# retinal-information-processing-lab/gaussian_processes

Measured on AMD Instinct MI355X. Metric: GP fits/sec (kernel+chol+solve+grad loglik) at N=8192 d=256, higher is better.
Workload: dtype f64; 1 GPU; N=8192 d=256 single cell f64, one M-step closure evaluation with 6 gradients (BASELINE configs[2], headline); N=8192, d=256, parallelism=independent units over 1 GPU(s), one process per GPU, no data-path collective

## Files before the change

### gaussian_processes_amd/csrc/elementwise.hip

```cpp
#include "kernels.h"

namespace gpfit {

__device__ __forceinline__ double wave_sum(double v) {
#pragma unroll
  for (int o = 32; o > 0; o >>= 1) v += __shfl_down(v, o);
  return v;
}

__device__ __forceinline__ double block_sum(double v, double* sh) {
  const int lane = threadIdx.x & 63, wave = threadIdx.x >> 6;
  const int nw = (blockDim.x + 63) >> 6;
  v = wave_sum(v);
  __syncthreads();
  if (lane == 0) sh[wave] = v;
  __syncthreads();
  if (wave == 0) {
    double t = (lane < nw) ? sh[lane] : 0.0;
    t = wave_sum(t);
    if (lane == 0) sh[16] = t;
  }
  __syncthreads();
  return sh[16];
}

__device__ __forceinline__ double lin_pm1(int i, int n) {
  if (n <= 1) return -1.0;
  const double step = 2.0 / (double)(n - 1);
  return (i < n / 2) ? fma(step, (double)i, -1.0) : fma(-step, (double)(n - 1 - i), 1.0);
}

template <typename R>
__global__ void localker_kernel(Theta th, const int* __restrict__ pix, int d, int dp, int n_rows, int n_cols,
                                R* __restrict__ C, int64_t ldc, R* __restrict__ dC) {
  const int j = blockIdx.x * blockDim.x + threadIdx.x;
  const int i = blockIdx.y * blockDim.y + threadIdx.y;
  if (i >= dp || j >= dp) return;
  if (i >= d || j >= d) {
    C[(int64_t)i * ldc + j] = (R)0;
    return;
  }
  const int pi = pix[i], pj = pix[j];
  const double xi = lin_pm1(pi % n_cols, n_cols), yi = lin_pm1(pi / n_cols, n_rows);
  const double xj = lin_pm1(pj % n_cols, n_cols), yj = lin_pm1(pj / n_cols, n_rows);
  const double dxi = xi - th.eps0x, dyi = yi - th.eps0y, dxj = xj - th.eps0x, dyj = yj - th.eps0y;
  const double lai = -th.eb * (dxi * dxi + dyi * dyi);
  const double laj = -th.eb * (dxj * dxj + dyj * dyj);
  const double ai = exp(lai), aj = exp(laj);
  const double ex = xj - xi, ey = yj - yi;
  const double ls = -th.er * (ex * ex + ey * ey);
  const double es = exp(ls);
  const double cij = th.amp * ai * es * aj;
  const double cji = th.amp * aj * es * ai;
  const double c = (cij + cji) / 2.0;
  C[(int64_t)i * ldc + j] = (R)c;
  if (dC) {
    const int64_t dd = (int64_t)d * d, o = (int64_t)i * d + j;
    dC[o] = (R)(c / th.amp);
    dC[dd + o] = (R)(c * (lai + laj));
    dC[2 * dd + o] = (R)(c * ls);
    dC[3 * dd + o] = (R)(2.0 * th.eb * c * (xi + xj - 2.0 * th.eps0x));
    dC[4 * dd + o] = (R)(2.0 * th.eb * c * (yi + yj - 2.0 * th.eps0y));
  }
}

template <typename R>
int launch_localker(const Theta& th, const int* pix, int d, int dp, int n_rows, int n_cols, R* C, int64_t ldc,
                    R* dC, hipStream_t s) {
  dim3 block(32, 8), grid((dp + 31) / 32, (dp + 7) / 8);
  hipLaunchKernelGGL(localker_kernel<R>, grid, block, 0, s, th, pix, d, dp, n_rows, n_cols, C, ldc, dC);
  GP_HIP(hipGetLastError());
  return 0;
}

template <typename R>
__global__ void gather_kernel(const R* __restrict__ X, int64_t ldx, int n, const int* __restrict__ pix, int d,
                              R* __restrict__ Xt, int64_t ldt, R* __restrict__ Xm, int64_t ldm) {
  __shared__ R tile[32][33];
  const int k0 = blockIdx.x * 32, n0 = blockIdx.y * 32;
  const int tx = threadIdx.x, ty = threadIdx.y;
#pragma unroll
  for (int r = 0; r < 4; ++r) {
    const int nn = n0 + ty + 8 * r, k = k0 + tx;
    R v = 0;
    if (nn < n && k < d) v = X[(int64_t)nn * ldx + (pix ? pix[k] : k)];
    tile[ty + 8 * r][tx] = v;
    if (Xm) Xm[(int64_t)nn * ldm + k] = v;
  }
  __syncthreads();
#pragma unroll
  for (int r = 0; r < 4; ++r) {
    const int k = k0 + ty + 8 * r, nn = n0 + tx;
    Xt[(int64_t)k * ldt + nn] = tile[tx][ty + 8 * r];
  }
}

template <typename R>
int launch_gather(const R* X, int64_t ldx, int n, const int* pix, int d, int dp, int np, R* Xt, int64_t ldt, R* Xm,
                  int64_t ldm, hipStream_t s) {
  if (dp % 32 || np % 32) {
    set_error("launch_gather: padded extents must be multiples of 32");
    return -3;
  }
  hipLaunchKernelGGL(gather_kernel<R>, dim3(dp / 32, np / 32), dim3(32, 8), 0, s, X, ldx, n, pix, d, Xt, ldt, Xm,
                     ldm);
  GP_HIP(hipGetLastError());
  return 0;
}

template <typename R>
__global__ __launch_bounds__(256) void qvec_kernel(const R* __restrict__ Xt, const R* __restrict__ XCt, int64_t ld, int dp,
                                                   int n, int np, double s0sq, R* __restrict__ Kvec, R* __restrict__ q) {
  __shared__ double part[8][33];
  const int li = threadIdx.x & 31, sl = threadIdx.x >> 5;
  const int i = blockIdx.x * 32 + li;
  double h = 0.0;
  if (i < n) {
#pragma unroll 4
    for (int k = sl; k < dp; k += 8) h += (double)Xt[(int64_t)k * ld + i] * (double)XCt[(int64_t)k * ld + i];
  }
  part[sl][li] = h;
  __syncthreads();
  if (sl != 0 || i >= np) return;
  if (i >= n) {
    Kvec[i] = (R)1;
    q[i] = (R)1;
    return;
  }
  double t = part[0][li];
#pragma unroll
  for (int z = 1; z < 8; ++z) t += part[z][li];
  const double kv = t + s0sq;
  Kvec[i] = (R)kv;
  q[i] = (R)sqrt(kv);
}

template <typename R>
int launch_qvec(const R* Xt, const R* XCt, int64_t ld, int dp, int n, int np, double s0sq, R* Kvec, R* q,
                hipStream_t s) {
  hipLaunchKernelGGL(qvec_kernel<R>, dim3((np + 31) / 32), dim3(256), 0, s, Xt, XCt, ld, dp, n, np, s0sq, Kvec, q);
  GP_HIP(hipGetLastError());
  return 0;
}

template <typename R>
__global__ __launch_bounds__(256) void group_prepare_kernel(GroupPrepT<R> g) {
  const int u = blockIdx.y;
  const int i = blockIdx.x * 256 + threadIdx.x;
  if (i < g.np) g.mpad[u][i] = (i < g.n) ? g.m[u][i] : (R)0;
  if (blockIdx.x == 0) {
    for (int k = threadIdx.x; k < g.d[u]; k += 256) g.pix[u][k] = g.pix_host[u][k];
    if (threadIdx.x < 4) g.info[u][threadIdx.x] = 0;
  }
}

template <typename R>
int launch_group_prepare(const GroupPrepT<R>& g, hipStream_t s) {
  hipLaunchKernelGGL(group_prepare_kernel<R>, dim3((g.np + 255) / 256, g.n_units), dim3(256), 0, s, g);
  GP_HIP(hipGetLastError());
  return 0;
}

__global__ void group_collect_kernel(GroupCollectT g) {
  const int u = blockIdx.x, t = threadIdx.x;
  if (t < 64) g.scal_host[u][t] = g.scal[u][t];
  else if (t < 68) g.info_host[u][t - 64] = g.info[u][t - 64];
  __threadfence_system();
}

int launch_group_collect(const GroupCollectT& g, hipStream_t s) {
  hipLaunchKernelGGL(group_collect_kernel, dim3(g.n_units), dim3(128), 0, s, g);
  GP_HIP(hipGetLastError());
  return 0;
}

template <typename R>
__global__ __launch_bounds__(256) void pack_lower_kernel(const R* __restrict__ src, int64_t lds, int n, R* __restrict__ dst,
                                                         int64_t ldd) {
  const int tj = blockIdx.x, ti = blockIdx.y;
  if (tj > ti) return;
  const int r0 = ti * TILE + 16 * blockIdx.z, c0 = tj * TILE;
#pragma unroll
  for (int it = 0; it < 8; ++it) {
    const int e = threadIdx.x + 256 * it;
    const int i = r0 + (e >> 7), j = c0 + (e & 127);
    R v;
    if (i < n && j < n) v = src[(int64_t)i * lds + j];
    else v = (i == j) ? (R)1 : (R)0;
    dst[(int64_t)i * ldd + j] = v;
  }
}

template <typename R>
int launch_pack_lower(const R* src, int64_t lds, int n, R* dst, int64_t ldd, int np, hipStream_t s) {
  hipLaunchKernelGGL(pack_lower_kernel<R>, dim3(np / TILE, np / TILE, TILE / 16), dim3(256), 0, s, src, lds, n, dst, ldd);
  GP_HIP(hipGetLastError());
  return 0;
}

template <typename R>
__global__ void symmetrize_kernel(R* __restrict__ A, int64_t lda, int n) {
  __shared__ R tile[32][33];
  const int tj = blockIdx.x, ti = blockIdx.y;
  if (tj > ti) return;
  const int tx = threadIdx.x, ty = threadIdx.y;
#pragma unroll
  for (int r = 0; r < 4; ++r) {
    const int i = ti * 32 + ty + 8 * r, j = tj * 32 + tx;
    tile[ty + 8 * r][tx] = (i < n && j < n) ? A[(int64_t)i * lda + j] : (R)0;
  }
  __syncthreads();
#pragma unroll
  for (int r = 0; r < 4; ++r) {
    const int jj = tj * 32 + ty + 8 * r, ii = ti * 32 + tx;
    if (ii < n && jj < n && ii > jj) A[(int64_t)jj * lda + ii] = tile[tx][ty + 8 * r];
  }
}

template <typename R>
int launch_symmetrize(R* A, int64_t lda, int n, hipStream_t s) {
  const int t = (n + 31) / 32;
  hipLaunchKernelGGL(symmetrize_kernel<R>, dim3(t, t), dim3(32, 8), 0, s, A, lda, n);
  GP_HIP(hipGetLastError());
  return 0;
}

template <typename R>
__global__ void logdet_kernel(const R* __restrict__ L0, double* __restrict__ out0, const R* __restrict__ L1,
                              double* __restrict__ out1, int64_t ldl, int n) {
  __shared__ double sh[17];
  const R* __restrict__ L = blockIdx.x == 0 ? L0 : L1;
  double v = 0.0;
  for (int i = threadIdx.x; i < n; i += blockDim.x) v += log((double)L[(int64_t)i * ldl + i]);
  v = block_sum(v, sh);
  if (threadIdx.x == 0) (blockIdx.x == 0 ? out0 : out1)[0] = 2.0 * v;
}

template <typename R>
int launch_logdet(const R* L, int64_t ldl, int n, double* out, hipStream_t s) {
  hipLaunchKernelGGL(logdet_kernel<R>, dim3(1), dim3(1024), 0, s, L, out, L, out, ldl, n);
  GP_HIP(hipGetLastError());
  return 0;
}

template <typename R>
int launch_logdet_pair(const R* L0, double* out0, const R* L1, double* out1, int64_t ldl, int n, hipStream_t s) {
  hipLaunchKernelGGL(logdet_kernel<R>, dim3(2), dim3(1024), 0, s, L0, out0, L1, out1, ldl, n);
  GP_HIP(hipGetLastError());
  return 0;
}

template <typename R>
__global__ void sum_kernel(const R* __restrict__ x, int n, double scale, double* __restrict__ out) {
  __shared__ double sh[17];
  double v = 0.0;
  for (int i = threadIdx.x; i < n; i += blockDim.x) v += (double)x[i];
  v = block_sum(v, sh);
  if (threadIdx.x == 0) out[0] = scale * v;
}

template <typename R>
__global__ void frob_tile_kernel(const R* __restrict__ T, int64_t ldt, double* __restrict__ partial) {
  __shared__ double sh[17];
  int ti, tj;
  {
    const int t = blockIdx.x;
    int i = (int)((sqrt(8.0 * (double)t + 1.0) - 1.0) * 0.5);
    while ((i + 1) * (i + 2) / 2 <= t) ++i;
    while (i * (i + 1) / 2 > t) --i;
    ti = i;
    tj = t - i * (i + 1) / 2;
  }
  const R* base = T + (int64_t)ti * TILE * ldt + tj * TILE;
  double v = 0.0;
#pragma unroll 8
  for (int e = threadIdx.x; e < TILE * TILE; e += 256) {
    const double x = (double)base[(int64_t)(e >> 7) * ldt + (e & 127)];
    v += x * x;
  }
  v = block_sum(v, sh);
  if (threadIdx.x == 0) partial[blockIdx.x] = v;
}

template <typename R>
int launch_frob_lower(const R* T, int64_t ldt, int np, double* out, double* partial, hipStream_t s) {
  const int t = np / TILE, nt = t * (t + 1) / 2;
  hipLaunchKernelGGL(frob_tile_kernel<R>, dim3(nt), dim3(256), 0, s, T, ldt, partial);
  hipLaunchKernelGGL(sum_kernel<double>, dim3(1), dim3(1024), 0, s, partial, nt, 1.0, out);
  GP_HIP(hipGetLastError());
  return 0;
}

int launch_frob_finish(const double* partial, int nt, double* out, hipStream_t s) {
  hipLaunchKernelGGL(sum_kernel<double>, dim3(1), dim3(1024), 0, s, partial, nt, 1.0, out);
  GP_HIP(hipGetLastError());
  return 0;
}

template <typename R>
__global__ void trmv_lower_kernel(const R* __restrict__ L, int64_t ldl, int np, const R* __restrict__ x,
                                  R* __restrict__ y) {
  const int lane = threadIdx.x & 63;
  const int i = blockIdx.x * (blockDim.x >> 6) + (threadIdx.x >> 6);
  if (i >= np) return;
  const R* row = L + (int64_t)i * ldl;
  double v = 0.0;
#pragma unroll 8
  for (int j = lane; j <= i; j += 64) v += (double)row[j] * (double)x[j];
  v = wave_sum(v);
  if (lane == 0) y[i] = (R)v;
}

template <typename R>
int launch_trmv_lower(const R* L, int64_t ldl, int np, const R* x, R* y, hipStream_t s) {
  hipLaunchKernelGGL(trmv_lower_kernel<R>, dim3((np + 3) / 4), dim3(256), 0, s, L, ldl, np, x, y);
  GP_HIP(hipGetLastError());
  return 0;
}

template <typename R>
__global__ void trmv_lower_t_kernel(const R* __restrict__ L, int64_t ldl, int np, const R* __restrict__ x,
                                    double* __restrict__ partial) {
  __shared__ double sh[4][64];
  const int c = threadIdx.x & 63, rl = threadIdx.x >> 6;
  const int j = blockIdx.x * 64 + c;
  const int i0 = blockIdx.y * TRMV_ROWS, i1 = min(np, i0 + TRMV_ROWS);
  double v = 0.0;
  if (i1 > blockIdx.x * 64) {
#pragma unroll 8
    for (int i = i0 + rl; i < i1; i += 4)
      if (i >= j) v += (double)L[(int64_t)i * ldl + j] * (double)x[i];
  }
  sh[rl][c] = v;
  __syncthreads();
  if (rl == 0) partial[(int64_t)blockIdx.y * np + j] = sh[0][c] + sh[1][c] + sh[2][c] + sh[3][c];
}

template <typename RI, typename RO>
__global__ void reduce_slices_kernel(const RI* __restrict__ src, int64_t stride, int nslice, RO* __restrict__ dst,
                                     int64_t count) {
  const int64_t i = (int64_t)blockIdx.x * blockDim.x + threadIdx.x;
  if (i >= count) return;
  double v = 0.0;
  for (int z = 0; z < nslice; ++z) v += (double)src[(int64_t)z * stride + i];
  dst[i] = (RO)v;
}

template <typename RI, typename RO>
int launch_reduce_slices(const RI* src, int64_t slice_stride, int nslice, RO* dst, int64_t count, hipStream_t s) {
  hipLaunchKernelGGL((reduce_slices_kernel<RI, RO>), dim3((unsigned)((count + 255) / 256)), dim3(256), 0, s, src,
                     slice_stride, nslice, dst, count);
  GP_HIP(hipGetLastError());
  return 0;
}

template <typename R>
int launch_trmv_lower_t(const R* L, int64_t ldl, int np, const R* x, R* z, double* partial, hipStream_t s) {
  const int chunks = (np + TRMV_ROWS - 1) / TRMV_ROWS;
  hipLaunchKernelGGL(trmv_lower_t_kernel<R>, dim3(np / 64, chunks), dim3(256), 0, s, L, ldl, np, x, partial);
  GP_HIP(hipGetLastError());
  return launch_reduce_slices(partial, np, chunks, z, np, s);
}

template <typename R>
__global__ void dot_kernel(const R* __restrict__ x, const R* __restrict__ y, int n, double* __restrict__ out) {
  __shared__ double sh[17];
  double v = 0.0;
  for (int i = threadIdx.x; i < n; i += blockDim.x) v += (double)x[i] * (double)y[i];
  v = block_sum(v, sh);
  if (threadIdx.x == 0) out[0] = v;
}

template <typename R>
int launch_dot(const R* x, const R* y, int n, double* out, hipStream_t s) {
  hipLaunchKernelGGL(dot_kernel<R>, dim3(1), dim3(1024), 0, s, x, y, n, out);
  GP_HIP(hipGetLastError());
  return 0;
}

template <typename R>
__global__ __launch_bounds__(256) void moments_kernel(const R* __restrict__ Kvec, const R* __restrict__ q,
                                                      const R* __restrict__ Cos, int64_t ldc, const R* __restrict__ V,
                                                      int64_t ldv, const R* __restrict__ m, const R* __restrict__ r, int n,
                                                      double A, double lambda0, R* __restrict__ lam_m,
                                                      R* __restrict__ lam_var, R* __restrict__ f, R* __restrict__ wl,
                                                      double* __restrict__ scal, double* __restrict__ part,
                                                      int* __restrict__ ticket) {
  __shared__ double sh[17];
  __shared__ bool last;
  double s_rm = 0.0, s_r = 0.0, s_f = 0.0;
  const int i = blockIdx.x * 256 + threadIdx.x;
  if (i < n) {
    const double c = (double)Cos[(int64_t)i * ldc + i];
    const double delta = acos(c);
    const double J = (sqrt(1.0 - c * c) + PI32 * c - delta * c) / PI32;
    const double qi = (double)q[i];
    const double kii = qi * qi * J;
    const double lv = (double)Kvec[i] - kii + (double)V[(int64_t)i * ldv + i];
    const double lm = (double)m[i];
    const double fi = exp(A * lm + 0.5 * A * A * lv + lambda0);
    const double g = 1.0 - J - (PI32 - delta) * (1.0 - c) / PI32;
    lam_m[i] = (R)lm;
    lam_var[i] = (R)lv;
    f[i] = (R)fi;
    wl[i] = (R)(-0.5 * A * A * fi * g);
    s_rm = (double)r[i] * lm;
    s_r = (double)r[i];
    s_f = fi;
  }
  s_rm = block_sum(s_rm, sh);
  s_r = block_sum(s_r, sh);
  s_f = block_sum(s_f, sh);
  if (threadIdx.x == 0) {
    part[blockIdx.x * 3 + 0] = s_rm;
    part[blockIdx.x * 3 + 1] = s_r;
    part[blockIdx.x * 3 + 2] = s_f;
    __threadfence();
    last = (atomicAdd(ticket, 1) == (int)gridDim.x - 1);
  }
  __syncthreads();
  if (!last) return;
  __threadfence();
  if (threadIdx.x < 3) {
    double v = 0.0;
    for (int b = 0; b < (int)gridDim.x; ++b)
      v += __hip_atomic_load(&part[b * 3 + threadIdx.x], __ATOMIC_RELAXED, __HIP_MEMORY_SCOPE_AGENT);
    scal[threadIdx.x] = v;
  }
  if (threadIdx.x == 0) *ticket = 0;
}

template <typename R>
int launch_moments(const R* Kvec, const R* q, const R* Cos, int64_t ldc, const R* V, int64_t ldv, const R* m,
                   const R* r, int n, double A, double lambda0, R* lam_m, R* lam_var, R* f, R* wl, double* scal,
                   double* part, int* ticket, hipStream_t s) {
  hipLaunchKernelGGL(moments_kernel<R>, dim3((n + 255) / 256), dim3(256), 0, s, Kvec, q, Cos, ldc, V, ldv, m, r, n, A,
                     lambda0, lam_m, lam_var, f, wl, scal, part, ticket);
  GP_HIP(hipGetLastError());
  return 0;
}

template <typename R>
__global__ __launch_bounds__(256) void adjoint_kernel(const R* __restrict__ W, const R* __restrict__ Cos, int64_t ld,
                                                      const R* __restrict__ b, const R* __restrict__ q, int n,
                                                      int np, R* __restrict__ Aout, double* __restrict__ upart,
                                                      double* __restrict__ vpart, double* __restrict__ sumA_part) {
  __shared__ R tA[64][65];
  __shared__ double colsum[4][64];
  __shared__ double sh[17];
  int ti, tj;
  {
    const int t = blockIdx.x;
    int i = (int)((sqrt(8.0 * (double)t + 1.0) - 1.0) * 0.5);
    while ((i + 1) * (i + 2) / 2 <= t) ++i;
    while (i * (i + 1) / 2 > t) --i;
    ti = i;
    tj = t - i * (i + 1) / 2;
  }
  const bool diag = (ti == tj);
  const int tx = threadIdx.x & 63, ty = threadIdx.x >> 6;
  const int j = tj * 64 + tx;
  const double qj = (double)q[j], bj = (double)b[j];
  double csum = 0.0, asum = 0.0;
  for (int rr = ty; rr < 64; rr += 4) {
    const int i = ti * 64 + rr;
    double aw = 0.0, bm = 0.0;
    if (i < n && j < n) {
      const int64_t o = (diag && i < j) ? ((int64_t)j * ld + i) : ((int64_t)i * ld + j);
      const double w = (double)W[o] - 0.5 * (double)b[i] * bj;
      const double c = (double)Cos[o];
      aw = w * (PI32 - acos(c)) / PI32;
      bm = w * sqrt(1.0 - c * c) / PI32;
    }
    tA[rr][tx] = (R)aw;
    Aout[(int64_t)i * ld + j] = (R)aw;
    asum += aw;
    const double rs = wave_sum(bm * qj);
    if (tx == 0) upart[(int64_t)tj * np + i] = rs;
    csum += bm * (double)q[i];
  }
  colsum[ty][tx] = csum;
  __syncthreads();
  if (!diag) {
    if (ty == 0) vpart[(int64_t)ti * np + j] = colsum[0][tx] + colsum[1][tx] + colsum[2][tx] + colsum[3][tx];
    for (int rr = ty; rr < 64; rr += 4) {
      const int jj = tj * 64 + rr, ii = ti * 64 + tx;
      Aout[(int64_t)jj * ld + ii] = tA[tx][rr];
    }
  }
  asum = block_sum(asum, sh);
  if (threadIdx.x == 0) sumA_part[blockIdx.x] = diag ? asum : 2.0 * asum;
}

template <typename R>
__global__ __launch_bounds__(256) void adjoint_u_kernel(const double* __restrict__ upart, const double* __restrict__ vpart,
                                                        int nt64, const R* __restrict__ q, const R* __restrict__ wl, int n,
                                                        int np, R* __restrict__ tvec, double* __restrict__ uq) {
  __shared__ double sl[8][33];
  const int li = threadIdx.x & 31, z = threadIdx.x >> 5;
  const int i = blockIdx.x * 32 + li;
  double u = 0.0;
  if (i < n) {
    const int T = i >> 6;
#pragma unroll 4
    for (int t = z; t < nt64; t += 8) u += (t <= T ? upart : vpart)[(int64_t)t * np + i];
  }
  sl[z][li] = u;
  __syncthreads();
  if (z != 0 || i >= np) return;
  if (i >= n) {
    tvec[i] = (R)0;
    uq[i] = 0.0;
    return;
  }
  u = sl[0][li];
#pragma unroll
  for (int k = 1; k < 8; ++k) u += sl[k][li];
  const double v = u / (double)q[i];
  uq[i] = v;
  tvec[i] = (R)(v - (double)wl[i]);
}

template <typename R>
__global__ void adjoint_sums_kernel(const double* __restrict__ uq, const R* __restrict__ wl, int n,
                                    const double* __restrict__ sumA_part, int ntile_tri, double* __restrict__ out) {
  __shared__ double sh[17];
  const int b = blockIdx.x;
  double v = 0.0;
  if (b == 0) for (int i = threadIdx.x; i < n; i += blockDim.x) v += uq[i];
  else if (b == 1) for (int i = threadIdx.x; i < n; i += blockDim.x) v += (double)wl[i];
  else for (int i = threadIdx.x; i < ntile_tri; i += blockDim.x) v += sumA_part[i];
  v = block_sum(v, sh);
  if (threadIdx.x == 0) out[b] = v;
}

__global__ __launch_bounds__(256) void adjoint_rect_kernel(const double* __restrict__ W, int64_t ldw,
                                                           const double* __restrict__ Cos, int64_t ldc,
                                                           const double* __restrict__ q1,
                                                           const double* __restrict__ q2, int n1, int n2, int np1,
                                                           int np2, double* __restrict__ Aout, int64_t lda,
                                                           double* __restrict__ upart, double* __restrict__ vpart,
                                                           double* __restrict__ tile_sum) {
  __shared__ double colsum[4][64];
  __shared__ double sh[17];
  const int tj = blockIdx.x, ti = blockIdx.y;
  const int tx = threadIdx.x & 63, ty = threadIdx.x >> 6;
  const int j = tj * 64 + tx;
  const double qj = (j < n2) ? q2[j] : 0.0;
  double csum = 0.0, asum = 0.0;
  for (int rr = ty; rr < 64; rr += 4) {
    const int i = ti * 64 + rr;
    double aw = 0.0, bm = 0.0;
    if (i < n1 && j < n2) {
      const double w = W[(int64_t)i * ldw + j];
      const double c = Cos[(int64_t)i * ldc + j];
      aw = w * (PI32 - acos(c)) / PI32;
      bm = w * sqrt(1.0 - c * c) / PI32;
    }
    Aout[(int64_t)i * lda + j] = aw;
    asum += aw;
    const double rs = wave_sum(bm * qj);
    if (tx == 0) upart[(int64_t)tj * np1 + i] = rs;
    csum += (i < n1) ? bm * q1[i] : 0.0;
  }
  colsum[ty][tx] = csum;
  __syncthreads();
  if (ty == 0) vpart[(int64_t)ti * np2 + j] = colsum[0][tx] + colsum[1][tx] + colsum[2][tx] + colsum[3][tx];
  asum = block_sum(asum, sh);
  if (threadIdx.x == 0) tile_sum[ti * gridDim.x + tj] = asum;
}

__global__ __launch_bounds__(256) void adjoint_rect_reduce_kernel(const double* __restrict__ part, int nt,
                                                                  const double* __restrict__ q,
                                                                  const double* __restrict__ extra, int n, int np,
                                                                  double* __restrict__ tvec, double* __restrict__ uq) {
  __shared__ double sl[8][33];
  const int li = threadIdx.x & 31, z = threadIdx.x >> 5;
  const int i = blockIdx.x * 32 + li;
  double u = 0.0;
  if (i < n) {
#pragma unroll 4
    for (int t = z; t < nt; t += 8) u += part[(int64_t)t * np + i];
  }
  sl[z][li] = u;
  __syncthreads();
  if (z != 0 || i >= np) return;
  if (i >= n) {
    tvec[i] = 0.0;
    uq[i] = 0.0;
    return;
  }
  u = sl[0][li];
#pragma unroll
  for (int k = 1; k < 8; ++k) u += sl[k][li];
  const double v = u / q[i];
  uq[i] = v;
  tvec[i] = 0.5 * v + (extra ? extra[i] : 0.0);
}

struct SumList {
  const double* x[4];
  int n[4];
  double scale[4];
  double* out[4];
};
__global__ void sum_list_kernel(SumList l) {
  __shared__ double sh[17];
  const int b = blockIdx.x;
  double v = 0.0;
  for (int i = threadIdx.x; i < l.n[b]; i += blockDim.x) v += l.x[b][i];
  v = block_sum(v, sh);
  if (threadIdx.x == 0) l.out[b][0] = l.scale[b] * v;
}

int launch_adjoint_rect(const double* W, int64_t ldw, const double* Cos, int64_t ldc, const double* q1,
                        const double* q2, int n1, int n2, int np1, int np2, double* Aout, int64_t lda, double* upart,
                        double* vpart, double* tile_sum, const double* extra1, double* t1, double* t2, double* uq1,
                        double* uq2, double* scal3, hipStream_t s) {
  const int g1 = np1 / 64, g2 = np2 / 64;
  hipLaunchKernelGGL(adjoint_rect_kernel, dim3(g2, g1), dim3(256), 0, s, W, ldw, Cos, ldc, q1, q2, n1, n2, np1, np2,
                     Aout, lda, upart, vpart, tile_sum);
  hipLaunchKernelGGL(adjoint_rect_reduce_kernel, dim3((np1 + 31) / 32), dim3(256), 0, s, upart, g2, q1, extra1, n1,
                     np1, t1, uq1);
  hipLaunchKernelGGL(adjoint_rect_reduce_kernel, dim3((np2 + 31) / 32), dim3(256), 0, s, vpart, g1, q2,
                     (const double*)nullptr, n2, np2, t2, uq2);
  SumList l{};
  l.x[0] = tile_sum; l.n[0] = g1 * g2; l.scale[0] = 1.0; l.out[0] = scal3 + 0;
  l.x[1] = uq1; l.n[1] = n1; l.scale[1] = 1.0; l.out[1] = scal3 + 1;
  l.x[2] = uq2; l.n[2] = n2; l.scale[2] = 1.0; l.out[2] = scal3 + 2;
  hipLaunchKernelGGL(sum_list_kernel, dim3(3), dim3(1024), 0, s, l);
  GP_HIP(hipGetLastError());
  return 0;
}

template <typename R>
int launch_adjoint(const R* W, const R* Cos, int64_t ld, const R* b, const R* q, int n, int np, R* Aout,
                   double* upart, double* vpart, double* sumA_part, hipStream_t s) {
  const int t = np / 64, nt = t * (t + 1) / 2;
  hipLaunchKernelGGL(adjoint_kernel<R>, dim3(nt), dim3(256), 0, s, W, Cos, ld, b, q, n, np, Aout, upart, vpart,
                     sumA_part);
  GP_HIP(hipGetLastError());
  return 0;
}

template <typename R>
int launch_adjoint_reduce(const double* upart, const double* vpart, const double* sumA_part, int ntile,
                          int ntile_tri, const R* q, const R* wl, int n, int np, R* tvec, double* uq,
                          double* scal_out, hipStream_t s) {
  hipLaunchKernelGGL(adjoint_u_kernel<R>, dim3((np + 31) / 32), dim3(256), 0, s, upart, vpart, ntile, q, wl, n,
                     np, tvec, uq);
  hipLaunchKernelGGL(adjoint_sums_kernel<R>, dim3(3), dim3(1024), 0, s, uq, wl, n, sumA_part, ntile_tri, scal_out);
  GP_HIP(hipGetLastError());
  return 0;
}

template <typename R>
__global__ void rowscale_add_kernel(R* __restrict__ Y, int64_t ldy, const R* __restrict__ Xm, int64_t ldm,
                                    const R* __restrict__ t, int dp) {
  const int i = blockIdx.y;
  const R ti = t[i];
  for (int k = blockIdx.x * blockDim.x + threadIdx.x; k < dp; k += gridDim.x * blockDim.x)
    Y[(int64_t)i * ldy + k] += ti * Xm[(int64_t)i * ldm + k];
}

template <typename R>
int launch_rowscale_add(R* Y, int64_t ldy, const R* Xm, int64_t ldm, const R* t, int np, int dp, hipStream_t s) {
  hipLaunchKernelGGL(rowscale_add_kernel<R>, dim3((dp + 255) / 256, np), dim3(256), 0, s, Y, ldy, Xm, ldm, t, dp);
  GP_HIP(hipGetLastError());
  return 0;
}

constexpr int METRIC_BLOCKS = 32;
template <typename R>
__global__ __launch_bounds__(256) void metric_contract_kernel(Theta th, const int* __restrict__ pix, int d, int n_rows,
                                                              int n_cols, const R* __restrict__ C, int64_t ldc,
                                                              const R* __restrict__ M, int64_t ldm,
                                                              double* __restrict__ grad5, double* __restrict__ part,
                                                              int* __restrict__ ticket) {
  __shared__ double sh[17];
  __shared__ int last;
  double g[5] = {0, 0, 0, 0, 0};
  for (int i = blockIdx.x; i < d; i += gridDim.x) {
    const int pi = pix[i];
    const double xi = lin_pm1(pi % n_cols, n_cols), yi = lin_pm1(pi / n_cols, n_rows);
    const double dxi = xi - th.eps0x, dyi = yi - th.eps0y;
    const double lai = -th.eb * (dxi * dxi + dyi * dyi);
    for (int j = threadIdx.x; j < d; j += blockDim.x) {
      const int pj = pix[j];
      const double xj = lin_pm1(pj % n_cols, n_cols), yj = lin_pm1(pj / n_cols, n_rows);
      const double dxj = xj - th.eps0x, dyj = yj - th.eps0y;
      const double laj = -th.eb * (dxj * dxj + dyj * dyj);
      const double ex = xj - xi, ey = yj - yi;
      const double ls = -th.er * (ex * ex + ey * ey);
      const double c = (double)C[(int64_t)i * ldc + j];
      const double mm = (double)M[(int64_t)i * ldm + j];
      g[0] += (c / th.amp) * mm;
      g[1] += (c * (lai + laj)) * mm;
      g[2] += (c * ls) * mm;
      g[3] += (2.0 * th.eb * c * (xi + xj - 2.0 * th.eps0x)) * mm;
      g[4] += (2.0 * th.eb * c * (yi + yj - 2.0 * th.eps0y)) * mm;
    }
  }
#pragma unroll
  for (int p = 0; p < 5; ++p) {
    const double v = block_sum(g[p], sh);
    if (threadIdx.x == 0) part[blockIdx.x * 5 + p] = v;
  }
  if (threadIdx.x == 0) {
    __threadfence();
    last = (atomicAdd(ticket, 1) == (int)gridDim.x - 1);
  }
  __syncthreads();
  if (!last) return;
  __threadfence();
  if (threadIdx.x < 5) {
    double v = 0.0;
    for (int b = 0; b < (int)gridDim.x; ++b) v += __hip_atomic_load(&part[b * 5 + threadIdx.x], __ATOMIC_RELAXED, __HIP_MEMORY_SCOPE_AGENT);
    grad5[threadIdx.x] = v;
  }
  if (threadIdx.x == 0) *ticket = 0;
}

template <typename R>
int launch_metric_contract(const Theta& th, const int* pix, int d, int n_rows, int n_cols, const R* C, int64_t ldc,
                           const R* M, int64_t ldm, double* grad5, double* part, int* ticket, hipStream_t s) {
  hipLaunchKernelGGL(metric_contract_kernel<R>, dim3(METRIC_BLOCKS), dim3(256), 0, s, th, pix, d, n_rows, n_cols, C,
                     ldc, M, ldm, grad5, part, ticket);
  GP_HIP(hipGetLastError());
  return 0;
}

__global__ void pad_copy_kernel(const double* __restrict__ src, int64_t lds, int rows, int cols,
                                double* __restrict__ dst, int64_t ldd, int prow, int pcol) {
  const int j = blockIdx.x * blockDim.x + threadIdx.x, i = blockIdx.y;
  if (j >= pcol || i >= prow) return;
  dst[(int64_t)i * ldd + j] = (i < rows && j < cols) ? src[(int64_t)i * lds + j] : 0.0;
}

int launch_pad_copy(const double* src, int64_t lds, int rows, int cols, double* dst, int64_t ldd, int prow,
                    int pcol, hipStream_t s) {
  hipLaunchKernelGGL(pad_copy_kernel, dim3((pcol + 255) / 256, prow), dim3(256), 0, s, src, lds, rows, cols, dst,
                     ldd, prow, pcol);
  GP_HIP(hipGetLastError());
  return 0;
}

__global__ void symmetrize_avg_kernel(double* __restrict__ A, int64_t lda, int n) {
  const int j = blockIdx.x * blockDim.x + threadIdx.x, i = blockIdx.y;
  if (i >= n || j >= i) return;
  const double a = A[(int64_t)i * lda + j], b = A[(int64_t)j * lda + i];
  const double v = (a + b) / 2.0;
  A[(int64_t)i * lda + j] = v;
  A[(int64_t)j * lda + i] = v;
}

int launch_symmetrize_avg(double* A, int64_t lda, int n, hipStream_t s) {
  hipLaunchKernelGGL(symmetrize_avg_kernel, dim3((n + 255) / 256, n), dim3(256), 0, s, A, lda, n);
  GP_HIP(hipGetLastError());
  return 0;
}

__global__ void dk_sigma0_kernel(const double* __restrict__ Cos, int64_t ldc, const double* __restrict__ q1,
                                 const double* __restrict__ q2, int n1, int n2, double s0,
                                 double* __restrict__ dK, int64_t ldk) {
  const int j = blockIdx.x * blockDim.x + threadIdx.x, i = blockIdx.y;
  if (i >= n1 || j >= n2) return;
  const double c = Cos[(int64_t)i * ldc + j];
  const double a = q1[i], b = q2[j], qq = a * b;
  const double delta = acos(c);
  const double J = (sqrt(1.0 - c * c) + PI32 * c - delta * c) / PI32;
  const double dqq = s0 * s0 * (b / a + a / b);
  const double dcos = (2.0 * s0 * s0 - c * dqq) / qq;
  const double dJ = -(delta - PI32) * dcos / PI32;
  dK[(int64_t)i * ldk + j] = (qq * dJ + dqq * J) / s0;
}

int launch_dk_sigma0(const double* Cos, int64_t ldc, const double* q1, const double* q2, int n1, int n2,
                     double s0, double* dK, int64_t ldk, hipStream_t s) {
  hipLaunchKernelGGL(dk_sigma0_kernel, dim3((n2 + 255) / 256, n1), dim3(256), 0, s, Cos, ldc, q1, q2, n1, n2, s0,
                     dK, ldk);
  GP_HIP(hipGetLastError());
  return 0;
}

__global__ void dq_kernel(const double* __restrict__ Xt, const double* __restrict__ XDt, int64_t ld, int dp,
                          int n, const double* __restrict__ q, double* __restrict__ dq, double* __restrict__ h) {
  const int i = blockIdx.x * blockDim.x + threadIdx.x;
  if (i >= n) return;
  double v = 0.0;
  for (int k = 0; k < dp; ++k) v += Xt[(int64_t)k * ld + i] * XDt[(int64_t)k * ld + i];
  if (h) h[i] = v;
  if (dq) dq[i] = 0.5 * v / q[i];
}

int launch_dq(const double* Xt, const double* XDt, int64_t ld, int dp, int n, const double* q, double* dq,
              double* h, hipStream_t s) {
  hipLaunchKernelGGL(dq_kernel, dim3((n + 255) / 256), dim3(256), 0, s, Xt, XDt, ld, dp, n, q, dq, h);
  GP_HIP(hipGetLastError());
  return 0;
}

__global__ void dk_metric_kernel(double* __restrict__ H, int64_t ldh, const double* __restrict__ Cos, int64_t ldc,
                                 const double* __restrict__ q1, const double* __restrict__ q2,
                                 const double* __restrict__ dq1, const double* __restrict__ dq2, int n1, int n2) {
  const int j = blockIdx.x * blockDim.x + threadIdx.x, i = blockIdx.y;
  if (i >= n1 || j >= n2) return;
  const double c = Cos[(int64_t)i * ldc + j];
  const double a = q1[i], b = q2[j], qq = a * b;
  const double delta = acos(c);
  const double J = (sqrt(1.0 - c * c) + PI32 * c - delta * c) / PI32;
  const double dqq = dq1[i] * b + a * dq2[j];
  const double dcos = (H[(int64_t)i * ldh + j] - c * dqq) / qq;
  const double dJ = -(delta - PI32) * dcos / PI32;
  H[(int64_t)i * ldh + j] = qq * dJ + dqq * J;
}

int launch_dk_metric(double* H, int64_t ldh, const double* Cos, int64_t ldc, const double* q1, const double* q2,
                     const double* dq1, const double* dq2, int n1, int n2, hipStream_t s) {
  hipLaunchKernelGGL(dk_metric_kernel, dim3((n2 + 255) / 256, n1), dim3(256), 0, s, H, ldh, Cos, ldc, q1, q2, dq1,
                     dq2, n1, n2);
  GP_HIP(hipGetLastError());
  return 0;
}

template <typename R>
__global__ void add_diag_kernel(R* __restrict__ A, int64_t lda, int n, double v) {
  const int i = blockIdx.x * blockDim.x + threadIdx.x;
  if (i < n) A[(int64_t)i * lda + i] += (R)v;
}

template <typename R>
int launch_add_diag(R* A, int64_t lda, int n, double v, hipStream_t s) {
  hipLaunchKernelGGL(add_diag_kernel<R>, dim3((n + 255) / 256), dim3(256), 0, s, A, lda, n, v);
  GP_HIP(hipGetLastError());
  return 0;
}

template <typename R>
__global__ void scale_copy_kernel(R* __restrict__ dst, const R* __restrict__ src, int n, R alpha) {
  const int i = blockIdx.x * blockDim.x + threadIdx.x;
  if (i < n) dst[i] = alpha * src[i];
}

template <typename R>
int launch_scale_copy(R* dst, const R* src, int n, double alpha, hipStream_t s) {
  hipLaunchKernelGGL(scale_copy_kernel<R>, dim3((n + 255) / 256), dim3(256), 0, s, dst, src, n, (R)alpha);
  GP_HIP(hipGetLastError());
  return 0;
}

template <typename R>
__global__ void axpby_block_kernel(R* __restrict__ dst, int64_t ldd, const R* __restrict__ src, int64_t lds, int rows,
                                   int cols, R a, R b) {
  const int c = (blockIdx.x * blockDim.x + threadIdx.x) * 2;
  const int r = blockIdx.y;
  if (c >= cols || r >= rows) return;
  R* d = dst + (int64_t)r * ldd + c;
  const R* q = src + (int64_t)r * lds + c;
  d[0] = a * d[0] + b * q[0];
  d[1] = a * d[1] + b * q[1];
}

template <typename R>
int launch_axpby_block(R* dst, int64_t ldd, const R* src, int64_t lds, int rows, int cols, double a, double b,
                       hipStream_t s) {
  hipLaunchKernelGGL(axpby_block_kernel<R>, dim3((cols / 2 + 255) / 256, rows), dim3(256), 0, s, dst, ldd, src, lds,
                     rows, cols, (R)a, (R)b);
  GP_HIP(hipGetLastError());
  return 0;
}

__global__ void fill_kernel(double* __restrict__ x, int64_t n, double v) {
  const int64_t i = (int64_t)blockIdx.x * blockDim.x + threadIdx.x;
  if (i < n) x[i] = v;
}

int launch_fill(double* x, int64_t n, double v, hipStream_t s) {
  hipLaunchKernelGGL(fill_kernel, dim3((unsigned)((n + 255) / 256)), dim3(256), 0, s, x, n, v);
  GP_HIP(hipGetLastError());
  return 0;
}

__global__ void estep_prep_kernel(const double* __restrict__ f, const double* __restrict__ r,
                                  const double* __restrict__ m, int n, int np, double A, double* __restrict__ sv,
                                  double* __restrict__ rhs) {
  const int i = blockIdx.x * blockDim.x + threadIdx.x;
  if (i >= np) return;
  if (i >= n) {
    sv[i] = 0.0;
    rhs[i] = 0.0;
    return;
  }
  sv[i] = A * sqrt(f[i]);
  rhs[i] = A * A * f[i] * m[i] + A * (r[i] - f[i]);
}

int launch_estep_prep(const double* f, const double* r, const double* m, int n, int np, double A, double* sv,
                      double* rhs, hipStream_t s) {
  hipLaunchKernelGGL(estep_prep_kernel, dim3((np + 255) / 256), dim3(256), 0, s, f, r, m, n, np, A, sv, rhs);
  GP_HIP(hipGetLastError());
  return 0;
}

__global__ void estep_build_kernel(const double* __restrict__ K, int64_t ldk, int n, const double* __restrict__ sv,
                                   double* __restrict__ Mb, double* __restrict__ SK, double* __restrict__ Kl,
                                   int64_t ld) {
  const int tj = blockIdx.x, ti = blockIdx.y;
  const int r0 = ti * TILE, c0 = tj * TILE;
  for (int e = threadIdx.x; e < TILE * TILE; e += blockDim.x) {
    const int i = r0 + (e >> 7), j = c0 + (e & 127);
    const bool in = (i < n && j < n);
    const double k = in ? K[(int64_t)i * ldk + j] : 0.0;
    const double si = sv[i];
    SK[(int64_t)i * ld + j] = si * k;
    if (tj <= ti) {
      Mb[(int64_t)i * ld + j] = si * k * sv[j] + ((i == j) ? 1.0 : 0.0);
      Kl[(int64_t)i * ld + j] = k;
    }
  }
}

int launch_estep_build(const double* K, int64_t ldk, int n, int np, const double* sv, double* Mb, double* SK,
                       double* Kl, int64_t ld, hipStream_t s) {
  hipLaunchKernelGGL(estep_build_kernel, dim3(np / TILE, np / TILE), dim3(256), 0, s, K, ldk, n, sv, Mb, SK, Kl, ld);
  GP_HIP(hipGetLastError());
  return 0;
}

__global__ void symv_lower_kernel(const double* __restrict__ A, int64_t lda, int n, const double* __restrict__ x,
                                  double* __restrict__ y) {
  const int lane = threadIdx.x & 63;
  const int i = blockIdx.x * (blockDim.x >> 6) + (threadIdx.x >> 6);
  if (i >= n) return;
  double v = 0.0;
  for (int j = lane; j <= i; j += 64) v += A[(int64_t)i * lda + j] * x[j];
  for (int j = i + 1 + lane; j < n; j += 64) v += A[(int64_t)j * lda + i] * x[j];
  v = wave_sum(v);
  if (lane == 0) y[i] = v;
}

int launch_symv_lower(const double* A, int64_t lda, int n, const double* x, double* y, hipStream_t s) {
  hipLaunchKernelGGL(symv_lower_kernel, dim3((n + 3) / 4), dim3(256), 0, s, A, lda, n, x, y);
  GP_HIP(hipGetLastError());
  return 0;
}

__global__ void unpack_sym_kernel(const double* __restrict__ src, int64_t lds, int n, double* __restrict__ dst,
                                  int64_t ldd) {
  const int j = blockIdx.x * blockDim.x + threadIdx.x, i = blockIdx.y;
  if (i >= n || j >= n) return;
  dst[(int64_t)i * ldd + j] = (j <= i) ? src[(int64_t)i * lds + j] : src[(int64_t)j * lds + i];
}

int launch_unpack_sym(const double* src, int64_t lds, int n, double* dst, int64_t ldd, hipStream_t s) {
  hipLaunchKernelGGL(unpack_sym_kernel, dim3((n + 255) / 256, n), dim3(256), 0, s, src, lds, n, dst, ldd);
  GP_HIP(hipGetLastError());
  return 0;
}

__global__ void unpack_tri_kernel(const double* __restrict__ src, int64_t lds, int n, double* __restrict__ dst,
                                  int64_t ldd) {
  const int j = blockIdx.x * blockDim.x + threadIdx.x, i = blockIdx.y;
  if (i >= n || j >= n) return;
  dst[(int64_t)i * ldd + j] = (j <= i) ? src[(int64_t)i * lds + j] : 0.0;
}

int launch_unpack_tri(const double* src, int64_t lds, int n, double* dst, int64_t ldd, hipStream_t s) {
  hipLaunchKernelGGL(unpack_tri_kernel, dim3((n + 255) / 256, n), dim3(256), 0, s, src, lds, n, dst, ldd);
  GP_HIP(hipGetLastError());
  return 0;
}


__device__ __forceinline__ void fparam_sums_A(const double* __restrict__ lam_m, const double* __restrict__ lam_var,
                                              int n, double A, double* sh, double& se, double& sg) {
  double e_sum = 0.0, g_sum = 0.0;
  for (int i = threadIdx.x; i < n; i += blockDim.x) {
    const double e = exp(A * lam_m[i] + 0.5 * A * A * lam_var[i]);
    e_sum += e;
    g_sum += (lam_m[i] + A * lam_var[i]) * e;
  }
  se = block_sum(e_sum, sh);
  sg = block_sum(g_sum, sh);
}

__device__ __forceinline__ void fparam_sums_r(const double* __restrict__ lam_m, const double* __restrict__ r, int n,
                                              double* sh, double& sr, double& srm) {
  double r_sum = 0.0, rm_sum = 0.0;
  for (int i = threadIdx.x; i < n; i += blockDim.x) {
    r_sum += r[i];
    rm_sum += r[i] * lam_m[i];
  }
  sr = block_sum(r_sum, sh);
  srm = block_sum(rm_sum, sh);
}

__device__ __forceinline__ void fparam_rate(const double* __restrict__ lam_m, const double* __restrict__ lam_var, int n,
                                            double A, double lambda0, double* __restrict__ f) {
  for (int i = threadIdx.x; i < n; i += blockDim.x) f[i] = exp(A * lam_m[i] + 0.5 * A * A * lam_var[i] + lambda0);
}

struct FparamScalars {
  double lambda0, loglik, dloglik, sum_f, lambda0_closed;
};
__device__ __forceinline__ FparamScalars fparam_scalars(double A, double se, double sg, double sr, double srm,
                                                        int closed_form, double lambda0_in) {
  FparamScalars v;
  v.lambda0 = closed_form ? (log(sr) - log(se)) : lambda0_in;
  const double el0 = exp(v.lambda0);
  v.sum_f = se * el0;
  v.loglik = A * srm + v.lambda0 * sr - v.sum_f;
  v.dloglik = A * (srm - sg * el0);
  v.lambda0_closed = log(sr) - log(se);
  return v;
}

__global__ void fparam_kernel(const double* __restrict__ lam_m, const double* __restrict__ lam_var,
                              const double* __restrict__ r, int n, double A, int closed_form, double lambda0_in,
                              double* __restrict__ f, double* __restrict__ out) {
  __shared__ double sh[17];
  double se, sg, sr, srm;
  fparam_sums_A(lam_m, lam_var, n, A, sh, se, sg);
  fparam_sums_r(lam_m, r, n, sh, sr, srm);
  const FparamScalars v = fparam_scalars(A, se, sg, sr, srm, closed_form, lambda0_in);
  if (f) fparam_rate(lam_m, lam_var, n, A, v.lambda0, f);
  if (threadIdx.x == 0) {
    out[0] = v.lambda0;
    out[1] = v.loglik;
    out[2] = v.dloglik;
    out[3] = v.sum_f;
    out[4] = sr;
    out[5] = srm;
    out[6] = v.lambda0_closed;
  }
}

int launch_fparam(const double* lam_m, const double* lam_var, const double* r, int n, double A, int closed_form,
                  double lambda0_in, double* f, double* out, hipStream_t s) {
  hipLaunchKernelGGL(fparam_kernel, dim3(1), dim3(1024), 0, s, lam_m, lam_var, r, n, A, closed_form, lambda0_in, f,
                     out);
  GP_HIP(hipGetLastError());
  return 0;
}

struct FparamDevicePass {
  const double* lam_m;
  const double* lam_var;
  int n;
  double* sh;
  double sr, srm;
  double A, se, sg;
  __device__ void pass(double logA) {
    const double A_new = exp(logA);
    if (!(A_new == A)) {
      fparam_sums_A(lam_m, lam_var, n, A_new, sh, se, sg);
      A = A_new;
    }
  }
  __device__ double lambda0_closed() const { return log(sr) - log(se); }
  __device__ FparamValues values(double lambda0_used) const {
    const FparamScalars v = fparam_scalars(A, se, sg, sr, srm, 0, lambda0_used);
    return FparamValues{v.loglik, v.dloglik, v.sum_f};
  }
};

struct Lbfgs1dLdsSlots {
  __device__ static void put(double* p, int i, double v) {
    if (threadIdx.x == 0) p[i] = v;
  }
  __device__ static void publish() { __syncthreads(); }
};

__global__ __launch_bounds__(1024) void fparam_lbfgs_kernel(const double* __restrict__ lam_m,
                                                            const double* __restrict__ lam_var,
                                                            const double* __restrict__ r, int n, double logA0,
                                                            int lambda0_mode, double lambda0_fixed, Lbfgs1dConfig cfg,
                                                            double* __restrict__ f, double* __restrict__ out) {
  __shared__ double sh[17];
  extern __shared__ double hist[];
  const int hs = cfg.history_size;
  FparamClosure<FparamDevicePass> obj;
  obj.ev.lam_m = lam_m;
  obj.ev.lam_var = lam_var;
  obj.ev.n = n;
  obj.ev.sh = sh;
  obj.ev.A = __builtin_nan("");
  obj.ev.se = obj.ev.sg = 0.0;
  fparam_sums_r(lam_m, r, n, sh, obj.ev.sr, obj.ev.srm);
  obj.fixed = lambda0_mode;
  obj.lambda0_fixed = lambda0_fixed;
  obj.lambda0 = 0.0;
  obj.calls = 0;
  obj.fail_x = obj.fail_lambda0 = 0.0;
  const Lbfgs1dResult res =
      lbfgs1d_step<Lbfgs1dLdsSlots>(obj, logA0, cfg, Lbfgs1dStorage{hist, hist + hs, hist + 2 * hs, hist + 3 * hs});
  double lambda0 = __builtin_nan("");
  if (res.status == 0) {
    obj.ev.pass(res.x);
    lambda0 = obj.ev.lambda0_closed();
    if (f) fparam_rate(lam_m, lam_var, n, obj.ev.A, lambda0, f);
  }
  if (threadIdx.x == 0) {
    out[0] = res.x;
    out[1] = lambda0;
    out[2] = res.first_loss;
    out[3] = res.last_loss;
    out[4] = res.n_evals;
    out[5] = res.n_iter;
    out[6] = res.status;
    out[7] = res.status ? obj.fail_x : 0.0;
    out[8] = res.status ? obj.fail_lambda0 : 0.0;
  }
}

int launch_fparam_lbfgs(const double* lam_m, const double* lam_var, const double* r, int n, double logA0,
                        int lambda0_mode, double lambda0_fixed, const Lbfgs1dConfig& cfg, double* f, double* out,
                        hipStream_t s) {
  const size_t lds = 4 * (size_t)cfg.history_size * sizeof(double);
  hipLaunchKernelGGL(fparam_lbfgs_kernel, dim3(1), dim3(1024), lds, s, lam_m, lam_var, r, n, logA0, lambda0_mode,
                     lambda0_fixed, cfg, f, out);
  GP_HIP(hipGetLastError());
  return 0;
}

#define GP_INST(R)                                                                                                  \
  template int launch_localker<R>(const Theta&, const int*, int, int, int, int, R*, int64_t, R*, hipStream_t);      \
  template int launch_gather<R>(const R*, int64_t, int, const int*, int, int, int, R*, int64_t, R*, int64_t,        \
                                hipStream_t);                                                                       \
  template int launch_qvec<R>(const R*, const R*, int64_t, int, int, int, double, R*, R*, hipStream_t);             \
  template int launch_pack_lower<R>(const R*, int64_t, int, R*, int64_t, int, hipStream_t);                         \
  template int launch_symmetrize<R>(R*, int64_t, int, hipStream_t);                                                 \
  template int launch_logdet<R>(const R*, int64_t, int, double*, hipStream_t);                                      \
  template int launch_logdet_pair<R>(const R*, double*, const R*, double*, int64_t, int, hipStream_t);              \
  template int launch_frob_lower<R>(const R*, int64_t, int, double*, double*, hipStream_t);                         \
  template int launch_trmv_lower<R>(const R*, int64_t, int, const R*, R*, hipStream_t);                             \
  template int launch_trmv_lower_t<R>(const R*, int64_t, int, const R*, R*, double*, hipStream_t);                  \
  template int launch_group_prepare<R>(const GroupPrepT<R>&, hipStream_t);                                          \
  template int launch_dot<R>(const R*, const R*, int, double*, hipStream_t);                                        \
  template int launch_moments<R>(const R*, const R*, const R*, int64_t, const R*, int64_t, const R*, const R*, int, \
                                 double, double, R*, R*, R*, R*, double*, double*, int*, hipStream_t);              \
  template int launch_adjoint<R>(const R*, const R*, int64_t, const R*, const R*, int, int, R*, double*, double*,   \
                                 double*, hipStream_t);                                                             \
  template int launch_adjoint_reduce<R>(const double*, const double*, const double*, int, int, const R*, const R*,  \
                                        int, int, R*, double*, double*, hipStream_t);                               \
  template int launch_rowscale_add<R>(R*, int64_t, const R*, int64_t, const R*, int, int, hipStream_t);             \
  template int launch_reduce_slices<R, R>(const R*, int64_t, int, R*, int64_t, hipStream_t);                        \
  template int launch_metric_contract<R>(const Theta&, const int*, int, int, int, const R*, int64_t, const R*,      \
                                         int64_t, double*, double*, int*, hipStream_t);                             \
  template int launch_add_diag<R>(R*, int64_t, int, double, hipStream_t);                                           \
  template int launch_axpby_block<R>(R*, int64_t, const R*, int64_t, int, int, double, double, hipStream_t);          \
  template int launch_scale_copy<R>(R*, const R*, int, double, hipStream_t);
GP_INST(double)
GP_INST(float)
#undef GP_INST
template int launch_reduce_slices<double, float>(const double*, int64_t, int, float*, int64_t, hipStream_t);

}
```

### gaussian_processes_amd/csrc/fit.hip

```cpp
#include "context.h"
#include "gpfit_mi355x.h"

#include <algorithm>
#include <chrono>
#include <cmath>
#include <cstdlib>
#include <cstring>
#include <limits>

namespace gpfit {

static thread_local gpfit_ctx* g_prof = nullptr;
static thread_local void* g_main_sk_ws = nullptr;

static const int* walks() {
  static int w[7] = {3, 2, 1, 9, 9, 2, 2};
  static bool init = false;
  if (!init) {
    init = true;
    if (const char* e = getenv("GPFIT_WALKS")) {
      int v[7];
      if (sscanf(e, "%d,%d,%d,%d,%d,%d,%d", &v[0], &v[1], &v[2], &v[3], &v[4], &v[5], &v[6]) == 7)
        for (int i = 0; i < 7; ++i) w[i] = v[i];
    }
  }
  return w;
}

static hipEvent_t prof_event(gpfit_ctx* c) {
  hipEvent_t e;
  if (!c->ev_pool.empty()) {
    e = c->ev_pool.back();
    c->ev_pool.pop_back();
    return e;
  }
  (void)hipEventCreate(&e);
  return e;
}

void prof_begin(gpfit_ctx* c) {
  if (c->profile == 1) {
    g_prof = c;
    c->prof.clear();
  }
}

void prof_end(gpfit_ctx* c) {
  if (g_prof != c) return;
  g_prof = nullptr;
  (void)hipDeviceSynchronize();
  double ms[4] = {0, 0, 0, 0}, fl[4] = {0, 0, 0, 0}, cnt[4] = {0, 0, 0, 0};
  double big_ms = 0, big_fl = 0;
  for (auto& r : c->prof) {
    float t = 0.f;
    (void)hipEventElapsedTime(&t, r.a, r.b);
    if (r.kind == 0 && r.flops > big_fl) { big_fl = r.flops; big_ms = t; }
    ms[r.kind] += t;
    fl[r.kind] += r.flops;
    cnt[r.kind] += 1;
    c->ev_pool.push_back(r.a);
    c->ev_pool.push_back(r.b);
  }
  c->prof.clear();
  c->prof_out[0] = ms[0]; c->prof_out[1] = fl[0]; c->prof_out[2] = cnt[0];
  c->prof_out[3] = ms[1]; c->prof_out[4] = cnt[1];
  c->prof_out[5] = ms[2]; c->prof_out[6] = fl[2]; c->prof_out[7] = cnt[2];
  c->prof_out[8] = ms[3]; c->prof_out[9] = fl[3]; c->prof_out[10] = cnt[3];
  c->prof_out[11] = big_ms; c->prof_out[12] = big_fl;
}

ProfScope::ProfScope(hipStream_t s_, double flops_, int kind_) : s(s_), flops(flops_), kind(kind_) {
  if (g_prof) {
    a = prof_event(g_prof);
    (void)hipEventRecord(a, s);
  }
}
ProfScope::~ProfScope() {
  if (g_prof && a) {
    hipEvent_t b = prof_event(g_prof);
    (void)hipEventRecord(b, s);
    g_prof->prof.push_back({a, b, flops, kind});
  }
}

template <typename R>
double gemm_flops(const GemmArgsT<R>& g) {
  const int T = gemm_pick_tile(g);
  const int tm = (g.M + T - 1) / T, tn = (g.N + T - 1) / T, r = TILE / T;
  double steps = 0;
  for (int ti = 0; ti < tm; ++ti)
    for (int tj = 0; tj < tn; ++tj) {
      if (g.out_lower && tj / r > ti / r) continue;
      int kb = 0, ke = g.K;
      if (g.a_tri == 1) ke = std::min(ke, ti * T + T);
      if (g.a_tri == 2) kb = std::max(kb, ti * T);
      if (g.b_tri == 1) kb = std::max(kb, tj * T);
      if (g.b_tri == 2) ke = std::min(ke, tj * T + T);
      if (ke > kb) steps += (ke - kb);
    }
  return 2.0 * T * T * steps * (g.nptr > 0 ? g.nptr : (g.batch > 0 ? g.batch : 1));
}

template <typename R>
static GemmArgsT<R> gemm_args(int a_kmajor, int b_kmajor, int M, int N, int K, double alpha, const R* A, int64_t lda,
                              const R* B, int64_t ldb, double beta, R* C, int64_t ldc, int out_lower, int a_tri,
                              int b_tri, int reverse = 0, int ws = 0, void* sk_ws = nullptr) {
  GemmArgsT<R> g{};
  g.A = A; g.B = B; g.C = C;
  g.lda = lda; g.ldb = ldb; g.ldc = ldc;
  g.M = M; g.N = N; g.K = K;
  g.alpha = alpha; g.beta = beta;
  g.a_kmajor = a_kmajor; g.b_kmajor = b_kmajor;
  g.out_lower = out_lower; g.a_tri = a_tri; g.b_tri = b_tri;
  g.batch = 1; g.split_k = 1; g.reverse = reverse; g.workspace = ws; g.sk_ws = sk_ws ? sk_ws : g_main_sk_ws;
  return g;
}

static int g_eval_count = 0;
static int gemm_log_eval() {
  static const int v = getenv("GPFIT_GEMM_LOG") ? atoi(getenv("GPFIT_GEMM_LOG")) : -1;
  return v;
}

template <typename R>
static int run_gemm(hipStream_t s, const GemmArgsT<R>& g) {
  if (gemm_log_eval() >= 0 && g_eval_count == gemm_log_eval())
    fprintf(stderr, "[gpfit gemm] M %d N %d K %d atri %d btri %d lower %d nb %d tile %d ak %d bk %d epi %d flops %.6e\n", g.M, g.N, g.K,
            g.a_tri, g.b_tri, g.out_lower, g.nptr > 0 ? g.nptr : 1, gemm_pick_tile(g), g.a_kmajor, g.b_kmajor, g.epi, gemm_flops(g));
  ProfScope ps(s, g_prof ? gemm_flops(g) : 0.0, (g_prof && gemm_pick_tile(g) != TILE) ? 3 : 0);
  return launch_gemm(g, s);
}

template <typename R>
static int gemm(hipStream_t s, int a_kmajor, int b_kmajor, int M, int N, int K, double alpha, const R* A,
                int64_t lda, const R* B, int64_t ldb, double beta, R* C, int64_t ldc, int out_lower, int a_tri,
                int b_tri, int reverse = 0, int ws = 0, void* sk_ws = nullptr) {
  return run_gemm(s, gemm_args<R>(a_kmajor, b_kmajor, M, N, K, alpha, A, lda, B, ldb, beta, C, ldc, out_lower, a_tri, b_tri,
                                  reverse, ws, sk_ws));
}

template <typename R>
static int gemm_splitk(hipStream_t s, int a_kmajor, int b_kmajor, int M, int N, int K, double alpha, const R* A, int64_t lda,
                       const R* B, int64_t ldb, R* C, int64_t ldc, int splits, R* partial, int64_t partial_elems) {
  static const bool off = getenv("GPFIT_NO_SPLITK") != nullptr;
  splits = (int)std::min<int64_t>(splits, partial_elems / std::max<int64_t>(1, (int64_t)M * ldc));
  if (splits <= 1 || off || partial == nullptr)
    return gemm<R>(s, a_kmajor, b_kmajor, M, N, K, alpha, A, lda, B, ldb, 0.0, C, ldc, 0, 0, 0);
  GemmArgsT<R> g = gemm_args<R>(a_kmajor, b_kmajor, M, N, K, alpha, A, lda, B, ldb, 0.0, partial, ldc, 0, 0, 0);
  g.split_k = splits;
  g.sC = (int64_t)M * ldc;
  g.tile = TILE;
  GP_TRY(run_gemm(s, g));
  return launch_reduce_slices(partial, (int64_t)M * ldc, splits, C, (int64_t)M * ldc, s);
}
static int splitk_for(int M, int N, int K) {
  const long tiles = (long)((M + TILE - 1) / TILE) * ((N + TILE - 1) / TILE);
  if (tiles >= 384) return 1;
  long sp = (768 + tiles - 1) / tiles;
  sp = std::min<long>(sp, std::max(1, K / 256));
  return (int)std::max<long>(1, sp);
}

static int fused_epilogues() {
  static const int v = getenv("GPFIT_FUSED_EPI") ? atoi(getenv("GPFIT_FUSED_EPI")) : 7;
  return v;
}


template <typename R>
static int gemm_list(hipStream_t s, int cnt, const R* const* Ap, const R* const* Bp, R* const* Cp, int a_kmajor,
                     int b_kmajor, int M, int N, int K, double alpha, int64_t lda, int64_t ldb, double beta, int64_t ldc,
                     int out_lower, int a_tri, int b_tri, int reverse = 0, int ws_id = 0, void* sk_ws = nullptr,
                     int epi = 0, R* const* auxp = nullptr, double* const* sumsqp = nullptr, bool* epi_done = nullptr,
                     int* sumsq_entries = nullptr) {
  if (epi_done) *epi_done = false;
  if (sumsq_entries) *sumsq_entries = 0;
  if (cnt <= 0) return 0;
  if (cnt > GEMM_MAXB) {
    set_error("gemm_list: more problems than a pointer batch holds");
    return -3;
  }
  GemmArgsT<R> g = gemm_args<R>(a_kmajor, b_kmajor, M, N, K, alpha, Ap[0], lda, Bp[0], ldb, beta, Cp[0], ldc, out_lower,
                                a_tri, b_tri, reverse, ws_id, sk_ws);
  static const bool no_batch = getenv("GPFIT_NO_BATCH") != nullptr;
  static const int list_t128 = getenv("GPFIT_LIST_T128") ? atoi(getenv("GPFIT_LIST_T128")) : 0;
  static const int list_t128_dim = getenv("GPFIT_LIST_T128_DIM") ? atoi(getenv("GPFIT_LIST_T128_DIM")) : 4096;
  const bool share_t128 = epi != 0 && list_t128 > 0 && cnt >= list_t128 && M <= list_t128_dim && N <= list_t128_dim;
  if (cnt == 1 || (gemm_pick_tile(g) == TILE && !share_t128) || no_batch) {
    bool fused = epi != 0;
    for (int i = 0; i < cnt && fused; ++i) {
      g.A = Ap[i]; g.B = Bp[i]; g.C = Cp[i];
      g.epi = epi; g.aux = auxp ? auxp[i] : nullptr; g.sumsq = sumsqp ? sumsqp[i] : nullptr;
      fused = gemm_epilogue_ok(g);
    }
    for (int i = 0; i < cnt; ++i) {
      g.A = Ap[i]; g.B = Bp[i]; g.C = Cp[i];
      g.epi = fused ? epi : 0; g.aux = (fused && auxp) ? auxp[i] : nullptr; g.sumsq = (fused && sumsqp) ? sumsqp[i] : nullptr;
      GP_TRY(run_gemm(s, g));
    }
    if (epi_done) *epi_done = fused;
    if (fused && sumsq_entries) {
      g.A = Ap[0]; g.B = Bp[0]; g.C = Cp[0];
      g.epi = epi; g.aux = auxp ? auxp[0] : nullptr; g.sumsq = sumsqp ? sumsqp[0] : nullptr;
      *sumsq_entries = gemm_sumsq_entries(g);
    }
    return 0;
  }
  g.nptr = cnt;
  g.batch = cnt;
  for (int i = 0; i < cnt; ++i) {
    g.Ap[i] = Ap[i]; g.Bp[i] = Bp[i]; g.Cp[i] = Cp[i];
    g.auxp[i] = auxp ? auxp[i] : nullptr; g.sumsqp[i] = sumsqp ? sumsqp[i] : nullptr;
  }
  g.epi = epi;
  if (epi && !gemm_epilogue_ok(g)) g.epi = 0;
  if (epi_done) *epi_done = g.epi != 0;
  if (g.epi && sumsq_entries) *sumsq_entries = gemm_sumsq_entries(g);
  return run_gemm(s, g);
}

template <typename R>
static int bgemm(const CholBatchT<R>& B, hipStream_t s, uint32_t mask, int a_kmajor, int b_kmajor, int M, int N, int K,
                 double alpha, R* const* Ab, int64_t offA, R* const* Bb, int64_t offB, double beta, R* const* Cb,
                 int64_t offC, int out_lower, int a_tri, int b_tri, int reverse, int ws_id, void* sk_ws) {
  const R* Ap[GEMM_MAXB];
  const R* Bp[GEMM_MAXB];
  R* Cp[GEMM_MAXB];
  int cnt = 0;
  for (int b = 0; b < B.nb; ++b)
    if (mask & (1u << b)) {
      Ap[cnt] = Ab[b] + offA; Bp[cnt] = Bb[b] + offB; Cp[cnt] = Cb[b] + offC;
      ++cnt;
    }
  return gemm_list<R>(s, cnt, Ap, Bp, Cp, a_kmajor, b_kmajor, M, N, K, alpha, B.ld, B.ld, beta, B.ld, out_lower, a_tri,
                      b_tri, reverse, ws_id, sk_ws);
}

template <typename R>
static GemmArgsT<R> batch_args(const CholBatchT<R>& B, uint32_t mask, int a_kmajor, int b_kmajor, int M, int N, int K, double alpha,
                               R* const* Ab, int64_t offA, R* const* Bb, int64_t offB, double beta, R* const* Cb, int64_t offC,
                               int out_lower, int a_tri, int b_tri, int reverse) {
  GemmArgsT<R> g = gemm_args<R>(a_kmajor, b_kmajor, M, N, K, alpha, (const R*)nullptr, B.ld, (const R*)nullptr, B.ld, beta,
                                (R*)nullptr, B.ld, out_lower, a_tri, b_tri, reverse, B.ws, B.sk_ws);
  int cnt = 0;
  for (int b = 0; b < B.nb; ++b)
    if (mask & (1u << b)) {
      g.Ap[cnt] = Ab[b] + offA; g.Bp[cnt] = Bb[b] + offB; g.Cp[cnt] = Cb[b] + offC;
      ++cnt;
    }
  g.nptr = cnt;
  g.batch = cnt;
  if (cnt > 0) { g.A = g.Ap[0]; g.B = g.Bp[0]; g.C = g.Cp[0]; }
  return g;
}

template <typename R>
int potrf_lockstep(const CholBatchT<R>& B, int r0, int n, uint32_t need, hipStream_t s, uint32_t halves) {
  const int64_t ld = B.ld;
  const uint32_t all = (B.nb >= 32) ? 0xffffffffu : ((1u << B.nb) - 1u);
  auto off = [&](int r, int c) { return (int64_t)r * ld + c; };
  if (n == TILE) {
    ProfScope ps(s, 0.0, 1);
    LeafBatchT<R> bt{};
    bt.n = B.nb;
    for (int b = 0; b < B.nb; ++b) {
      bt.A[b] = B.A[b] + off(r0, r0); bt.L[b] = B.L[b] + off(r0, r0); bt.Li[b] = B.Li[b] + off(r0, r0);
      bt.info[b] = B.info[b];
    }
    bt.lda = bt.ldl = bt.ldi = ld;
    bt.info_base = r0;
    return launch_chol_leaf_batch(bt, s);
  }
  const int k = n / TILE;
  const int n1 = ((k + 1) / 2) * TILE, n2 = n - n1;
  const int r1 = r0 + n1;
  GP_TRY(potrf_lockstep<R>(B, r0, n1, all, s));
  GP_TRY(bgemm<R>(B, s, all, 0, 0, n2, n1, n1, 1.0, B.A, off(r1, r0), B.Li, off(r0, r0), 0.0, B.L, off(r1, r0), 0, 0, 2,
                  walks()[0], B.ws, B.sk_ws));
  hipEvent_t joined = nullptr;
  if (need && B.ctx && B.side_min > 0 && n >= B.side_min && B.ctx->side) {
    gpfit_ctx* c = B.ctx;
    auto next_event = [&]() {
      if (c->side_ev_next == (int)c->side_ev.size()) {
        hipEvent_t e = nullptr;
        (void)hipEventCreateWithFlags(&e, hipEventDisableTiming);
        c->side_ev.push_back(e);
      }
      return c->side_ev[c->side_ev_next++];
    };
    hipEvent_t fork = next_event();
    joined = next_event();
    GP_HIP(hipEventRecord(fork, s));
    GP_HIP(hipStreamWaitEvent(c->side, fork, 0));
    GP_TRY(bgemm<R>(B, c->side, need, 0, 1, n2, n1, n1, 1.0, B.L, off(r1, r0), B.Li, off(r0, r0), 0.0, B.Tmp, off(r1, r0), 0, 0,
                    1, walks()[1], 1, c->sk_ws[1]));
    GP_HIP(hipEventRecord(joined, c->side));
  }
  bool merged = false;
  if (need && !joined) {
    static const bool no_batch = getenv("GPFIT_NO_BATCH") != nullptr;
    const GemmArgsT<R> g2 = batch_args<R>(B, all, 0, 0, n2, n2, n1, -1.0, B.L, off(r1, r0), B.L, off(r1, r0), 1.0, B.A, off(r1, r1),
                                          1, 0, 0, 0);
    const GemmArgsT<R> g3 = batch_args<R>(B, need, 0, 1, n2, n1, n1, 1.0, B.L, off(r1, r0), B.Li, off(r0, r0), 0.0, B.Tmp,
                                          off(r1, r0), 0, 0, 1, walks()[1]);
    if (!no_batch && gemm_pair_ok(g2, g3)) {
      if (gemm_log_eval() >= 0 && g_eval_count == gemm_log_eval())
        fprintf(stderr, "[gpfit gemm] pair: M %d N %d K %d lower 1 nb %d + M %d N %d K %d btri 1 nb %d tile %d flops %.6e\n", g2.M, g2.N,
                g2.K, g2.nptr, g3.M, g3.N, g3.K, g3.nptr, gemm_pick_tile(g3), gemm_flops(g2) + gemm_flops(g3));
      ProfScope ps(s, g_prof ? gemm_flops(g2) + gemm_flops(g3) : 0.0, 3);
      GP_TRY(launch_gemm_pair(g2, g3, s));
      merged = true;
    }
  }
  if (!merged)
    GP_TRY(bgemm<R>(B, s, all, 0, 0, n2, n2, n1, -1.0, B.L, off(r1, r0), B.L, off(r1, r0), 1.0, B.A, off(r1, r1), 1, 0, 0, 0,
                    B.ws, B.sk_ws));
  GP_TRY(potrf_lockstep<R>(B, r1, n2, need | halves, s));
  if (need) {
    if (joined) GP_HIP(hipStreamWaitEvent(s, joined, 0));
    else if (!merged)
      GP_TRY(bgemm<R>(B, s, need, 0, 1, n2, n1, n1, 1.0, B.L, off(r1, r0), B.Li, off(r0, r0), 0.0, B.Tmp, off(r1, r0), 0, 0,
                      1, walks()[1], B.ws, B.sk_ws));
    GP_TRY(bgemm<R>(B, s, need, 0, 1, n2, n1, n2, -1.0, B.Li, off(r1, r1), B.Tmp, off(r1, r0), 0.0, B.Li, off(r1, r0), 0, 1, 0,
                    walks()[2], B.ws, B.sk_ws));
  }
  return 0;
}

template int potrf_lockstep<double>(const CholBatchT<double>&, int, int, uint32_t, hipStream_t, uint32_t);
template int potrf_lockstep<float>(const CholBatchT<float>&, int, int, uint32_t, hipStream_t, uint32_t);

template <typename R>
struct TwoSidedBufs {
  const R* Q; const R* Li; R* W; R* Z; R* H; int64_t ld; int min_split;
  void* sk_ws = nullptr;
};
template <typename R>
static int two_sided_list(int cnt, const TwoSidedBufs<R>* b, const int* r0, int n, hipStream_t s) {
  if (cnt <= 0) return 0;
  const int64_t ld = b[0].ld;
  auto at = [&](const R* base, int r, int c) { return const_cast<R*>(base) + (int64_t)r * ld + c; };
  const R* Ap[GEMM_MAXB];
  const R* Bp[GEMM_MAXB];
  R* Cp[GEMM_MAXB];
  const int k = n / TILE;
  if (n < b[0].min_split || k < 2) {
    static const int wbase_walk = getenv("GPFIT_WBASE_WALK") ? atoi(getenv("GPFIT_WBASE_WALK")) : 0;
    for (int i = 0; i < cnt; ++i) { Ap[i] = at(b[i].Q, r0[i], r0[i]); Bp[i] = at(b[i].Li, r0[i], r0[i]); Cp[i] = at(b[i].Z, r0[i], r0[i]); }
    GP_TRY(gemm_list<R>(s, cnt, Ap, Bp, Cp, 1, 1, n, n, n, 1.0, ld, ld, 0.0, ld, 0, 0, 1, walks()[5], 0, b[0].sk_ws));
    for (int i = 0; i < cnt; ++i) { Ap[i] = at(b[i].Li, r0[i], r0[i]); Bp[i] = at(b[i].Z, r0[i], r0[i]); Cp[i] = at(b[i].W, r0[i], r0[i]); }
    GP_TRY(gemm_list<R>(s, cnt, Ap, Bp, Cp, 1, 1, n, n, n, 0.5, ld, ld, 0.0, ld, 1, 2, 0, wbase_walk, 0, b[0].sk_ws));
    return 0;
  }
  const int n1 = ((k + 1) / 2) * TILE, n2 = n - n1;
  auto diagonal_blocks = [&]() -> int {
    TwoSidedBufs<R> bb[GEMM_MAXB];
    int rr[GEMM_MAXB];
    if (n1 == n2 && 2 * cnt <= GEMM_MAXB) {
      for (int i = 0; i < cnt; ++i) {
        bb[2 * i] = b[i]; rr[2 * i] = r0[i];
        bb[2 * i + 1] = b[i]; rr[2 * i + 1] = r0[i] + n1;
      }
      return two_sided_list<R>(2 * cnt, bb, rr, n1, s);
    }
    for (int i = 0; i < cnt; ++i) rr[i] = r0[i] + n1;
    GP_TRY(two_sided_list<R>(cnt, b, r0, n1, s));
    return two_sided_list<R>(cnt, b, rr, n2, s);
  };
  for (int i = 0; i < cnt; ++i) {
    const int r1 = r0[i] + n1;
    Ap[i] = at(b[i].Q, r1, r1); Bp[i] = at(b[i].Li, r1, r0[i]); Cp[i] = at(b[i].Z, r1, r0[i]);
  }
  GP_TRY(gemm_list<R>(s, cnt, Ap, Bp, Cp, 1, 1, n2, n1, n2, 0.5, ld, ld, 0.0, ld, 0, 0, 0, 0, 0, b[0].sk_ws));
  {
    R* Zp[GEMM_MAXB];
    for (int i = 0; i < cnt; ++i) {
      const int r1 = r0[i] + n1;
      Ap[i] = at(b[i].Q, r1, r0[i]); Bp[i] = at(b[i].Li, r0[i], r0[i]); Cp[i] = at(b[i].H, r1, r0[i]); Zp[i] = at(b[i].Z, r1, r0[i]);
    }
    bool fused = false;
    if (fused_epilogues() & 4) {
      GemmArgsT<R> g = gemm_args<R>(0, 1, n2, n1, n1, 1.0, Ap[0], ld, Bp[0], ld, 0.0, Cp[0], ld, 0, 0, 1, walks()[6], 0, b[0].sk_ws);
      g.epi = 4; g.aux = Zp[0];
      static const bool no_batch = getenv("GPFIT_NO_BATCH") != nullptr;
      if (cnt > 1 && gemm_pick_tile(g) != TILE && !no_batch) { g.nptr = cnt; g.batch = cnt; }
      fused = gemm_epilogue_ok(g);
    }
    if (fused) {
      bool done = false;
      GP_TRY(gemm_list<R>(s, cnt, Ap, Bp, Cp, 0, 1, n2, n1, n1, 1.0, ld, ld, 0.0, ld, 0, 0, 1, walks()[6], 0, b[0].sk_ws, 4, Zp, nullptr,
                          &done));
      if (!done) {
        set_error("two_sided: the dual-update epilogue was announced but not carried");
        return -100;
      }
    } else {
      for (int i = 0; i < cnt; ++i)
        GP_HIP(hipMemcpy2DAsync(Cp[i], (size_t)ld * sizeof(R), Zp[i], (size_t)ld * sizeof(R), (size_t)n1 * sizeof(R), (size_t)n2,
                                hipMemcpyDeviceToDevice, s));
      GP_TRY(gemm_list<R>(s, cnt, Ap, Bp, Cp, 0, 1, n2, n1, n1, 1.0, ld, ld, 1.0, ld, 0, 0, 1, walks()[6], 0, b[0].sk_ws));
      for (int i = 0; i < cnt; ++i) GP_TRY(launch_axpby_block<R>(Zp[i], ld, Cp[i], ld, n2, n1, 1.0, 1.0, s));
    }
  }
  static const int w21_walk = getenv("GPFIT_W21_WALK") ? atoi(getenv("GPFIT_W21_WALK")) : 0;
  for (int i = 0; i < cnt; ++i) {
    const int r1 = r0[i] + n1;
    Ap[i] = at(b[i].Li, r1, r1); Bp[i] = at(b[i].Z, r1, r0[i]); Cp[i] = at(b[i].W, r1, r0[i]);
  }
  GP_TRY(gemm_list<R>(s, cnt, Ap, Bp, Cp, 1, 1, n2, n1, n2, 0.5, ld, ld, 0.0, ld, 0, 2, 0, w21_walk, 0, b[0].sk_ws));
  GP_TRY(diagonal_blocks());
  for (int i = 0; i < cnt; ++i) {
    const int r1 = r0[i] + n1;
    Ap[i] = at(b[i].Li, r1, r0[i]); Bp[i] = at(b[i].H, r1, r0[i]); Cp[i] = at(b[i].W, r0[i], r0[i]);
  }
  GP_TRY(gemm_list<R>(s, cnt, Ap, Bp, Cp, 1, 1, n1, n1, n2, 0.5, ld, ld, 1.0, ld, 1, 0, 0, 0, 0, b[0].sk_ws));
  for (int i = 0; i < cnt; ++i) {
    const int r1 = r0[i] + n1;
    Ap[i] = at(b[i].H, r1, r0[i]); Bp[i] = at(b[i].Li, r1, r0[i]);
  }
  GP_TRY(gemm_list<R>(s, cnt, Ap, Bp, Cp, 1, 1, n1, n1, n2, 0.5, ld, ld, 1.0, ld, 1, 0, 0, 0, 0, b[0].sk_ws));
  return 0;
}

static double lin_pm1_host(int i, int n) {
  if (n <= 1) return -1.0;
  const double step = 2.0 / (double)(n - 1);
  return (i < n / 2) ? std::fma(step, (double)i, -1.0) : std::fma(-step, (double)(n - 1 - i), 1.0);
}

static int compute_mask(const double* theta, int n_rows, int n_cols, uint8_t* mask, int* pix) {
  const double eb = std::exp(theta[3]);
  int d = 0;
  for (int p = 0; p < n_rows * n_cols; ++p) {
    const double x = lin_pm1_host(p % n_cols, n_cols), y = lin_pm1_host(p / n_cols, n_rows);
    const double dx = x - theta[1], dy = y - theta[2];
    const double alpha = std::exp(-eb * (dx * dx + dy * dy));
    const bool keep = alpha >= 0.001;
    if (mask) mask[p] = keep ? 1 : 0;
    if (keep) {
      if (pix) pix[d] = p;
      ++d;
    }
  }
  return d;
}

static Theta make_theta(const double* t) {
  Theta th;
  th.sigma0 = t[0]; th.eps0x = t[1]; th.eps0y = t[2]; th.logbeta = t[3]; th.logrho = t[4]; th.amp = t[5];
  th.eb = std::exp(t[3]);
  th.er = std::exp(t[4]);
  return th;
}

static int check_limits(const double* theta, const double* lower, const double* upper) {
  static const char* names[6] = {"sigma_0", "eps_0x", "eps_0y", "-2log2beta", "-log2rho2", "Amp"};
  for (int i = 0; i < 6; ++i) {
    if (!(lower[i] <= theta[i] && theta[i] <= upper[i])) {
      char buf[256];
      snprintf(buf, sizeof buf, "%s = %.4f is not within the limits of %g and %g", names[i], theta[i], lower[i],
               upper[i]);
      set_error(buf);
      return -2;
    }
  }
  return 0;
}

static int ensure_side_stream(gpfit_ctx* c) {
  if (c->side) return 0;
  int least = 0, greatest = 0;
  GP_HIP(hipDeviceGetStreamPriorityRange(&least, &greatest));
  GP_HIP(hipStreamCreateWithPriority(&c->side, hipStreamNonBlocking, least));
  return 0;
}

template <typename T>
static int dev_alloc(gpfit_ctx* c, T** p, size_t count) {
  void* q = nullptr;
  GP_HIP(hipMalloc(&q, count * sizeof(T)));
  c->allocs.push_back(q);
  *p = (T*)q;
  return 0;
}

template <typename R>
static R* ws_as(double* b) { return reinterpret_cast<R*>(b); }

static void fill_out_of_box(double* out) {
  const double inf = std::numeric_limits<double>::infinity();
  out[0] = inf;
  out[1] = out[2] = std::numeric_limits<double>::quiet_NaN();
  for (int i = 0; i < 6; ++i) out[3 + i] = inf;
}

struct Admitted { int d, dp; Theta th; };
static int admit(gpfit_ctx* c, const char* name, const char* whose, const double* theta, const double* lower,
                 const double* upper, int n_rows, int n_cols, int np, double* out, Admitted* a) {
  if (lower && upper && check_limits(theta, lower, upper) != 0) {
    fill_out_of_box(out);
    return -2;
  }
  if (np > c->np_cap || n_rows * n_cols > c->dfull_cap) {
    set_error(std::string(name) + ": problem larger than " + whose + " capacity");
    return -3;
  }
  a->d = compute_mask(theta, n_rows, n_cols, nullptr, c->pix_host);
  a->dp = (int)round_up(a->d, 32);
  if (a->d <= 0 || a->dp > c->dp_cap) {
    set_error(std::string(name) + ": masked pixel count is zero or exceeds " + whose + " capacity");
    return -3;
  }
  a->th = make_theta(theta);
  return 0;
}

template <typename R>
static int build_metric(gpfit_ctx* c, hipStream_t s, const Theta& th, int d, int dp, int n_rows, int n_cols) {
  return launch_localker<R>(th, c->pix, d, dp, n_rows, n_cols, ws_as<R>(c->Cmat), dp, nullptr, s);
}
template <typename R>
static int kernel_side(gpfit_ctx* c, hipStream_t s, const R* X, int64_t ldx, int n, int np, int d, int dp, double s0sq,
                       R* Xt, R* XCt, R* Xm, R* Kvec, R* q) {
  const int64_t ld = np;
  GP_TRY(launch_gather(X, ldx, n, c->pix, d, dp, np, Xt, ld, Xm, dp, s));
  GP_TRY(gemm<R>(s, 1, 1, dp, np, dp, 1.0, ws_as<R>(c->Cmat), dp, Xt, ld, 0.0, XCt, ld, 0, 0, 0));
  return launch_qvec(Xt, XCt, ld, dp, n, np, s0sq, Kvec, q, s);
}
template <typename R>
static int gram_square(hipStream_t s, const R* XCt, const R* Xt, const R* q, R* Kout, R* Cos, int n, int np, int dp,
                       double s0sq, int mirror) {
  GramArgsT<R> g{};
  g.XCt = XCt; g.Xt = Xt; g.q1 = q; g.q2 = q; g.Kout = Kout; g.Cos = Cos;
  g.ld1 = np; g.ld2 = np; g.ldk = np; g.np1 = np; g.np2 = np; g.nv1 = n; g.nv2 = n; g.Kd = dp;
  g.s0sq = s0sq; g.lower = 1; g.pad_identity = 1;
  g.mirror = mirror;
  ProfScope ps(s, (double)np * (np + TILE) * dp, 2);
  return launch_gram(g, s);
}
template <typename R>
static int build_kernel(gpfit_ctx* c, hipStream_t s, const Theta& th, int d, int dp, int n_rows, int n_cols, const R* X,
                        int64_t ldx, int n, int np, int mirror) {
  const double s0sq = th.sigma0 * th.sigma0;
  GP_TRY(build_metric<R>(c, s, th, d, dp, n_rows, n_cols));
  GP_TRY(kernel_side<R>(c, s, X, ldx, n, np, d, dp, s0sq, ws_as<R>(c->Xt), ws_as<R>(c->XCt), ws_as<R>(c->Xm),
                        ws_as<R>(c->Kvec), ws_as<R>(c->q)));
  return gram_square<R>(s, ws_as<R>(c->XCt), ws_as<R>(c->Xt), ws_as<R>(c->q), ws_as<R>(c->Kbuf), ws_as<R>(c->Cos), n, np,
                        dp, s0sq, mirror);
}

template <typename R>
static int solve_mean(gpfit_ctx* c, int np, hipStream_t s) {
  const int64_t ld = np;
  GP_TRY(launch_trmv_lower(ws_as<R>(c->Libuf), ld, np, ws_as<R>(c->mpad), ws_as<R>(c->yv), s));
  GP_TRY(launch_dot(ws_as<R>(c->yv), ws_as<R>(c->yv), np, c->scal + 6, s));
  return launch_trmv_lower_t(ws_as<R>(c->Libuf), ld, np, ws_as<R>(c->yv), ws_as<R>(c->bv), c->trmv_part, s);
}

template <typename R>
static int adjoint_pass(gpfit_ctx* c, hipStream_t s, const R* W, const R* Cos, const R* bv, const R* q, const R* wl, int n,
                        int np, R* A, R* tvec) {
  GP_TRY(launch_adjoint(W, Cos, (int64_t)np, bv, q, n, np, A, c->upart, c->vpart, c->sumA_part, s));
  const int t64 = np / 64;
  return launch_adjoint_reduce(c->upart, c->vpart, c->sumA_part, t64, t64 * (t64 + 1) / 2, q, wl, n, np, tvec, c->rpad,
                               c->scal + 7, s);
}
template <typename R>
static int xty(gpfit_ctx* c, hipStream_t s, const R* Xa, const R* Yb, int np, int dp, R* out, bool prof) {
  GemmArgsT<R> g{};
  g.A = Xa; g.B = Yb; g.C = ws_as<R>(c->Mpart);
  g.lda = dp; g.ldb = dp; g.ldc = dp;
  g.M = dp; g.N = dp; g.K = np;
  g.alpha = 1.0; g.beta = 0.0; g.a_kmajor = 1; g.b_kmajor = 1;
  g.batch = 1; g.split_k = c->split_k_M; g.sC = (int64_t)dp * dp;
  if (prof) {
    ProfScope ps(s, g_prof ? gemm_flops(g) : 0.0, (g_prof && gemm_pick_tile(g) != TILE) ? 3 : 0);
    GP_TRY(launch_gemm(g, s));
  } else {
    GP_TRY(launch_gemm(g, s));
  }
  return launch_reduce_slices(ws_as<R>(c->Mpart), (int64_t)dp * dp, c->split_k_M, out, (int64_t)dp * dp, s);
}
static int pullback_to_metric(gpfit_ctx* c, hipStream_t s, const double* W, const double* Cos, const double* q, int n,
                              int np, int dp, double* A, const double* Xm) {
  GP_TRY(adjoint_pass<double>(c, s, W, Cos, c->bv, q, c->wl, n, np, A, c->tvec));
  GP_TRY(gemm<double>(s, 1, 1, np, dp, np, 1.0, A, np, Xm, dp, 0.0, c->Ybuf, dp, 0, 0, 0));
  GP_TRY(launch_rowscale_add(c->Ybuf, dp, Xm, dp, c->tvec, np, dp, s));
  return xty<double>(c, s, Xm, c->Ybuf, np, dp, c->Mmat, false);
}

static int projected_factor(gpfit_ctx* c, hipStream_t s, const double* V_b, int64_t ldvb, int nk, int nb, double* Va,
                            double* Vl, double* Vli, double* Vt) {
  double *S1 = c->Vbuf, *S2 = c->LVbuf, *S3 = c->LiVbuf, *S4 = c->TmpV;
  const int64_t lb = nb;
  CholBatchT<double> cb;
  cb.nb = 2;
  cb.A[0] = S1; cb.L[0] = S2; cb.Li[0] = S3; cb.Tmp[0] = S4; cb.info[0] = c->info + 0;
  cb.A[1] = Va; cb.L[1] = Vl; cb.Li[1] = Vli; cb.Tmp[1] = Vt; cb.info[1] = c->info + 1;
  cb.ld = lb; cb.ws = 0; cb.sk_ws = c->sk_ws[0]; cb.ctx = nullptr; cb.side_min = 0;
  GP_TRY(potrf_lockstep<double>(cb, 0, nb, 1u, s));
  GP_TRY(launch_logdet(Vl, lb, nk, c->scal + 40, s));
  GP_TRY(launch_logdet(S2, lb, nk, c->scal + 3, s));
  GP_TRY(gemm<double>(s, 1, 1, nb, nb, nb, 1.0, S3, lb, S3, lb, 0.0, S1, lb, 1, 2, 1));
  GP_TRY(launch_symmetrize(S1, lb, nb, s));
  GP_TRY(launch_pack_lower(V_b, ldvb, nk, S2, lb, nb, s));
  return launch_symmetrize(S2, lb, nb, s);
}
static int projected_kl_products(gpfit_ctx* c, hipStream_t s, int nk, int nb) {
  double *Ki = c->Vbuf, *S2 = c->LVbuf, *S3 = c->LiVbuf, *S4 = c->TmpV;
  const int64_t lb = nb;
  GP_TRY(gemm<double>(s, 0, 1, nb, nb, nb, 1.0, Ki, lb, S2, lb, 0.0, S3, lb, 0, 0, 0));
  GP_TRY(launch_proj_trace(S3, lb, nk, c->scal + 5, s));
  return gemm<double>(s, 0, 1, nb, nb, nb, 1.0, S3, lb, Ki, lb, 0.0, S4, lb, 0, 0, 0);
}

static double sigma0_row_metric(const double* sc, double sigma0) { return sigma0 * (2.0 * sc[9] + 2.0 * sc[7]); }
static void grad_rows(const double* sc, double sigma0_row, double* g6) {
  g6[0] = sigma0_row;
  g6[1] = sc[13];
  g6[2] = sc[14];
  g6[3] = sc[11];
  g6[4] = sc[12];
  g6[5] = sc[10];
}
static int assemble_out(gpfit_ctx* c, double A, double lambda0, double sigma0_row, int pad, int d, int want_grad,
                        const char* err_K, const char* err_V, double* out_host) {
  const double* sc = c->scal_host;
  const double loglik = A * sc[0] + lambda0 * sc[1] - sc[2];
  const double trKinvV = sc[5] - (double)pad;
  const double logdetV = sc[40];
  const double KL = -0.5 * logdetV + 0.5 * sc[3] + 0.5 * sc[6] + 0.5 * trKinvV;
  out_host[0] = -(loglik - KL);
  out_host[1] = loglik;
  out_host[2] = KL;
  if (want_grad) grad_rows(sc, sigma0_row, out_host + 3);
  else
    for (int i = 0; i < 6; ++i) out_host[3 + i] = 0.0;
  out_host[9] = sc[3];
  out_host[10] = logdetV;
  out_host[11] = trKinvV;
  out_host[12] = sc[6];
  out_host[13] = (double)d;
  out_host[14] = (double)c->info_host[0];
  out_host[15] = (double)c->info_host[1];
  if (c->info_host[0] != 0) {
    set_error(err_K);
    return c->info_host[0];
  }
  if (c->info_host[1] != 0) {
    set_error(err_V);
    return c->info_host[1];
  }
  return 0;
}

template <typename R>
struct PostJoin {
  const R *Li, *LV, *Cos, *bv, *q, *wl, *Xm, *Cmat;
  R *T, *W, *Z, *H, *A, *Y, *tvec, *Mpart, *Mmat;
};
template <typename R>
static PostJoin<R> post_join_args(gpfit_ctx* c) {
  auto RP = ws_as<R>;
  return PostJoin<R>{RP(c->Libuf), RP(c->LVbuf), RP(c->Cos), RP(c->bv), RP(c->q), RP(c->wl), RP(c->Xm), RP(c->Cmat),
                     RP(c->Tbuf), RP(c->Wbuf), RP(c->Zbuf), RP(c->Tmp), RP(c->Abuf), RP(c->Ybuf), RP(c->tvec),
                     RP(c->Mpart), RP(c->Mmat)};
}
static int demote_for_mixed(gpfit_ctx* c, bool reuse_V, int np, int dp, hipStream_t s, PostJoin<float>* pf) {
  auto F = ws_as<float>;
  const int64_t nn = (int64_t)np * np;
  GP_TRY((launch_reduce_slices<double, float>(c->Libuf, nn, 1, F(c->Kbuf), nn, s)));
  if (!(reuse_V && c->lv32_valid)) GP_TRY((launch_reduce_slices<double, float>(c->LVbuf, nn, 1, F(c->Vbuf), nn, s)));
  c->lv32_valid = true;
  GP_TRY((launch_reduce_slices<double, float>(c->Cos, nn, 1, F(c->TmpV), nn, s)));
  GP_TRY((launch_reduce_slices<double, float>(c->bv, np, 1, F(c->q2), np, s)));
  GP_TRY((launch_reduce_slices<double, float>(c->q, np, 1, F(c->dq1), np, s)));
  GP_TRY((launch_reduce_slices<double, float>(c->wl, np, 1, F(c->dq2), np, s)));
  GP_TRY((launch_reduce_slices<double, float>(c->Xm, (int64_t)np * dp, 1, F(c->Xt2), (int64_t)np * dp, s)));
  GP_TRY((launch_reduce_slices<double, float>(c->Cmat, (int64_t)dp * dp, 1, F(c->dCpad), (int64_t)dp * dp, s)));
  *pf = PostJoin<float>{F(c->Kbuf), F(c->Vbuf), F(c->TmpV), F(c->q2), F(c->dq1), F(c->dq2), F(c->Xt2), F(c->dCpad),
                        F(c->Tbuf), F(c->Wbuf), F(c->Zbuf), F(c->Tmp), F(c->Abuf), F(c->Ybuf), F(c->tvec),
                        F(c->Mpart), F(c->Mmat)};
  return 0;
}
template <typename R, typename PhaseFn>
static int post_join_list(int cnt, gpfit_ctx* const* cs, const PostJoin<R>* a, const Theta* th, int n, int np, const int* d,
                          const int* dp, int n_rows, int n_cols, int want_grad, hipStream_t s, PhaseFn&& phase) {
  const int64_t ld = np;
  const R* Ap[GEMM_MAXB];
  const R* Bp[GEMM_MAXB];
  R* Cp[GEMM_MAXB];
  double* Sp[GEMM_MAXB];
  if (cnt <= 0 || cnt > GEMM_MAXB) return cnt == 0 ? 0 : -3;
  {
    for (int i = 0; i < cnt; ++i) { Ap[i] = a[i].Li; Bp[i] = a[i].LV; Cp[i] = a[i].T; Sp[i] = cs[i]->frob_part; }
    bool normed = false;
    int norm_entries = 0;
    GP_TRY(gemm_list<R>(s, cnt, Ap, Bp, Cp, 0, 1, np, np, np, 1.0, ld, ld, 0.0, ld, 1, 1, 1, walks()[3], 0, cs[0]->sk_ws[0],
                        (fused_epilogues() & 2) ? 2 : 0, nullptr, Sp, &normed, &norm_entries));
    for (int i = 0; i < cnt; ++i) {
      if (normed) GP_TRY(launch_frob_finish(cs[i]->frob_part, norm_entries, cs[i]->scal + 5, s));
      else GP_TRY(launch_frob_lower(a[i].T, ld, np, cs[i]->scal + 5, cs[i]->frob_part, s));
    }
  }
  phase(4, s);
  if (!want_grad) return 0;
  {
    for (int i = 0; i < cnt; ++i) { Ap[i] = a[i].T; Bp[i] = a[i].T; Cp[i] = a[i].W; }
    bool mirrored = false;
    GP_TRY(gemm_list<R>(s, cnt, Ap, Bp, Cp, 0, 0, np, np, np, -1.0, ld, ld, 0.0, ld, 1, 1, 2, walks()[4], 0, cs[0]->sk_ws[0],
                        (fused_epilogues() & 1) ? 1 : 0, nullptr, nullptr, &mirrored));
    for (int i = 0; i < cnt; ++i) {
      GP_TRY(launch_add_diag(a[i].W, ld, np, 1.0, s));
      if (!mirrored) GP_TRY(launch_symmetrize(a[i].W, ld, np, s));
    }
  }
  phase(5, s);
  {
    static const int ts_min = getenv("GPFIT_TS_MIN") ? atoi(getenv("GPFIT_TS_MIN")) : 4096;
    TwoSidedBufs<R> tb[GEMM_MAXB];
    int r0[GEMM_MAXB];
    for (int i = 0; i < cnt; ++i) {
      tb[i] = TwoSidedBufs<R>{a[i].W, a[i].Li, a[i].T, a[i].Z, a[i].H, ld, ts_min > 0 ? ts_min : (1 << 30)};
      tb[i].sk_ws = cs[0]->sk_ws[0];
      r0[i] = 0;
    }
    GP_TRY(two_sided_list<R>(cnt, tb, r0, np, s));
  }
  phase(6, s);
  for (int i = 0; i < cnt; ++i)
    GP_TRY(adjoint_pass<R>(cs[i], s, a[i].T, a[i].Cos, a[i].bv, a[i].q, a[i].wl, n, np, a[i].A, a[i].tvec));
  {
    bool same_dp = true;
    for (int i = 1; i < cnt; ++i) same_dp = same_dp && dp[i] == dp[0];
    for (int i = 0; i < cnt; ++i) { Ap[i] = a[i].A; Bp[i] = a[i].Xm; Cp[i] = a[i].Y; }
    if (same_dp) GP_TRY(gemm_list<R>(s, cnt, Ap, Bp, Cp, 1, 1, np, dp[0], np, 1.0, ld, dp[0], 0.0, dp[0], 0, 0, 0, 0, 0, cs[0]->sk_ws[0]));
    else
      for (int i = 0; i < cnt; ++i) GP_TRY(gemm<R>(s, 1, 1, np, dp[i], np, 1.0, a[i].A, ld, a[i].Xm, dp[i], 0.0, a[i].Y, dp[i], 0, 0, 0));
  }
  for (int i = 0; i < cnt; ++i) {
    gpfit_ctx* c = cs[i];
    GP_TRY(launch_rowscale_add(a[i].Y, dp[i], a[i].Xm, dp[i], a[i].tvec, np, dp[i], s));
    GP_TRY(xty<R>(c, s, a[i].Xm, a[i].Y, np, dp[i], a[i].Mmat, true));
    GP_TRY(launch_metric_contract(th[i], c->pix, d[i], n_rows, n_cols, a[i].Cmat, dp[i], a[i].Mmat, dp[i], c->scal + 10, c->upart,
                                  c->info + 3, s));
  }
  return 0;
}

static void set_pending(gpfit_ctx* c, hipStream_t s, double A, double lambda0, double sigma0, int n, int np, int d,
                        int want_grad, int elem_bytes, bool use_done) {
  c->pend.active = true; c->pend.stream = s; c->pend.A = A; c->pend.lambda0 = lambda0; c->pend.sigma0 = sigma0;
  c->pend.n = n; c->pend.np = np; c->pend.d = d; c->pend.want_grad = want_grad; c->pend.elem_bytes = elem_bytes;
  c->pend.use_done = use_done;
}

int fit_eval_finish(gpfit_ctx* c, double* out_host);

template <typename R>
static int fit_eval_impl(gpfit_ctx* c, void* stream, const double* theta, const double* lower, const double* upper,
                         int n_rows, int n_cols, const R* X, int64_t ldx, int64_t N, const R* r, const R* m,
                         const R* V, int64_t ldv, double logA, double lambda0, int want_grad, double* out_host,
                         R* lam_m_out, R* lam_var_out, R* f_out) {
  auto RP = ws_as<R>;
  if (!c || !theta || !X || !r || !m || !V || !out_host || N <= 0) {
    set_error("gpfit_fit_eval: bad argument");
    return -3;
  }
  GP_CTX_ENTER(c, "gpfit_fit_eval");
  hipStream_t s = (hipStream_t)stream;
  const int n = (int)N, np = (int)round_up(N, TILE);
  Admitted ad;
  GP_TRY(admit(c, "gpfit_fit_eval", "the context", theta, lower, upper, n_rows, n_cols, np, out_host, &ad));
  const int d = ad.d, dp = ad.dp;
  const Theta th = ad.th;
  const double A = std::exp(logA);
  const int64_t ld = np;
  c->cur_n = n; c->cur_np = np; c->cur_d = d; c->cur_dp = dp;

  ++g_eval_count;
  const auto t_host0 = std::chrono::steady_clock::now();
  auto phase = [&](int i, hipStream_t st) {
    if (c->profile != 2) return;
    if (!c->phase_ev[i]) (void)hipEventCreate(&c->phase_ev[i]);
    (void)hipEventRecord(c->phase_ev[i], st);
  };
  c->phase_valid = false;
  phase(0, s);
  g_main_sk_ws = c->sk_ws[0];
  prof_begin(c);
  struct ProfGuard { gpfit_ctx* c; ~ProfGuard() { prof_end(c); } } prof_guard{c};
  GP_HIP(hipMemsetAsync(c->info, 0, 4 * sizeof(int), s));
  GP_HIP(hipMemcpyAsync(c->pix, c->pix_host, (size_t)d * sizeof(int), hipMemcpyHostToDevice, s));
  GP_HIP(hipMemsetAsync(RP(c->mpad), 0, (size_t)np * sizeof(R), s));
  GP_HIP(hipMemcpyAsync(RP(c->mpad), m, (size_t)n * sizeof(R), hipMemcpyDeviceToDevice, s));

  const bool reuse_V = (want_grad & 2) && c->lv_valid && c->lv_n == n && c->lv_bytes == (int)sizeof(R);
  const bool async_call = (want_grad & 4) != 0;
  const bool mixed_grad = (want_grad & 8) != 0 && sizeof(R) == 8 && (want_grad & 1);
  want_grad &= 1;
  static const int side_min_env = getenv("GPFIT_SIDE_MIN") ? atoi(getenv("GPFIT_SIDE_MIN")) : 1024;
  const int side_min = async_call ? 0 : side_min_env;
  if (!async_call) GP_TRY(ensure_side_stream(c));
  c->side_ev_next = 0;
  if (!reuse_V) {
    c->lv_valid = false; c->lv32_valid = false;
    GP_HIP(hipEventRecord(c->ev_fork, s));
    GP_HIP(hipStreamWaitEvent(c->aux, c->ev_fork, 0));
    GP_TRY(launch_pack_lower(V, ldv, n, RP(c->Vbuf), ld, np, c->aux));
    GP_HIP(hipEventRecord(c->ev_join, c->aux));
  }

  GP_TRY(build_kernel<R>(c, s, th, d, dp, n_rows, n_cols, X, ldx, n, np, 0));
  GP_TRY(launch_moments(RP(c->Kvec), RP(c->q), RP(c->Cos), ld, V, ldv, m, r, n, A, lambda0, RP(c->lam_m), RP(c->lam_var), RP(c->fvec),
                        RP(c->wl), c->scal, c->sumA_part, c->info + 2, s));
  phase(1, s);
  {
    CholBatchT<R> cb;
    cb.nb = reuse_V ? 1 : 2;
    cb.A[0] = RP(c->Kbuf); cb.L[0] = RP(c->Lbuf); cb.Li[0] = RP(c->Libuf); cb.Tmp[0] = RP(c->Tmp); cb.info[0] = c->info + 0;
    cb.A[1] = RP(c->Vbuf); cb.L[1] = RP(c->LVbuf); cb.Li[1] = RP(c->LiVbuf); cb.Tmp[1] = RP(c->TmpV); cb.info[1] = c->info + 1;
    cb.ld = ld; cb.ws = 0; cb.sk_ws = c->sk_ws[0]; cb.ctx = c; cb.side_min = side_min;
    if (!reuse_V) GP_HIP(hipStreamWaitEvent(s, c->ev_join, 0));
    GP_TRY(potrf_lockstep<R>(cb, 0, np, 1u, s));
    if (!reuse_V) GP_TRY(launch_logdet(RP(c->LVbuf), ld, n, c->scal + 40, s));
    phase(3, s);
  }
  GP_TRY(launch_logdet(RP(c->Lbuf), ld, n, c->scal + 3, s));
  GP_TRY(solve_mean<R>(c, np, s));

  phase(2, s);
  if (mixed_grad) {
    PostJoin<float> pf;
    GP_TRY(demote_for_mixed(c, reuse_V, np, dp, s, &pf));
    GP_TRY(post_join_list<float>(1, &c, &pf, &th, n, np, &d, &dp, n_rows, n_cols, want_grad, s, phase));
  } else {
    const PostJoin<R> pj = post_join_args<R>(c);
    GP_TRY(post_join_list<R>(1, &c, &pj, &th, n, np, &d, &dp, n_rows, n_cols, want_grad, s, phase));
  }

  if (lam_m_out) GP_HIP(hipMemcpyAsync(lam_m_out, RP(c->lam_m), (size_t)n * sizeof(R), hipMemcpyDeviceToDevice, s));
  if (lam_var_out) GP_HIP(hipMemcpyAsync(lam_var_out, RP(c->lam_var), (size_t)n * sizeof(R), hipMemcpyDeviceToDevice, s));
  if (f_out) GP_HIP(hipMemcpyAsync(f_out, RP(c->fvec), (size_t)n * sizeof(R), hipMemcpyDeviceToDevice, s));
  GP_HIP(hipMemcpyAsync(c->scal_host, c->scal, 64 * sizeof(double), hipMemcpyDeviceToHost, s));
  GP_HIP(hipMemcpyAsync(c->info_host, c->info, 4 * sizeof(int), hipMemcpyDeviceToHost, s));
  phase(7, s);
  c->phase_valid = (c->profile == 2 && want_grad && !reuse_V);
  c->last_enqueue_ms = std::chrono::duration<double, std::milli>(std::chrono::steady_clock::now() - t_host0).count();
  set_pending(c, s, A, lambda0, th.sigma0, n, np, d, want_grad, (int)sizeof(R), false);
  if (async_call) return 0;
  return fit_eval_finish(c, out_host);
}

template <typename R>
static int fit_eval_batch_impl(gpfit_ctx* const* cs, int nu, void* stream, const double* theta6, const double* lower,
                               const double* upper, int n_rows, int n_cols, const R* const* X, int64_t ldx, int64_t N,
                               const R* const* r, const R* const* m, const R* const* V, int64_t ldv, const double* logA,
                               const double* lambda0, int want_grad, double* out_host, int* rc_out) {
  auto RP = ws_as<R>;
  if (!cs || nu <= 0 || 2 * nu > GEMM_MAXB || !theta6 || !X || !r || !m || !V || !logA || !lambda0 || !out_host || !rc_out ||
      N <= 0) {
    set_error("gpfit_fit_eval_batch: bad argument (1 .. 16 units per call)");
    return -3;
  }
  for (int u = 0; u < nu; ++u) {
    if (!cs[u] || !X[u] || !r[u] || !m[u] || !V[u]) {
      set_error("gpfit_fit_eval_batch: null context or operand");
      return -3;
    }
    if (cs[u]->device != cs[0]->device) {
      set_error("gpfit_fit_eval_batch: the contexts of one call must live on one device");
      return -3;
    }
    for (int v = 0; v < u; ++v)
      if (cs[v] == cs[u]) {
        set_error("gpfit_fit_eval_batch: every unit needs a context of its own");
        return -3;
      }
    if (cs[u]->pend.active) {
      set_error("gpfit_fit_eval_batch: an asynchronous evaluation is pending on one of the contexts");
      return -3;
    }
  }
  DeviceGuard device_guard(cs[0]->device);
  hipStream_t s = (hipStream_t)stream;
  const int n = (int)N, np = (int)round_up(N, TILE);
  const int64_t ld = np;
  const bool mixed_grad = (want_grad & 8) != 0 && sizeof(R) == 8 && (want_grad & 1);
  const bool want_reuse = (want_grad & 2) != 0;
  want_grad &= 1;
  const auto t_host0 = std::chrono::steady_clock::now();

  struct Unit { gpfit_ctx* c; int u, d, dp; Theta th; double A; bool reuse_V; };
  Unit un[GEMM_MAXB];
  int na = 0;
  for (int u = 0; u < nu; ++u) {
    gpfit_ctx* c = cs[u];
    Admitted ad;
    const int rc = admit(c, "gpfit_fit_eval_batch", "a context's", theta6 + 6 * u, lower, upper, n_rows, n_cols, np,
                         out_host + 16 * u, &ad);
    rc_out[u] = rc == -2 ? -2 : 0;
    if (rc == -2) continue;
    if (rc != 0) return rc;
    Unit& q = un[na++];
    q.c = c; q.u = u; q.d = ad.d; q.dp = ad.dp; q.th = ad.th; q.A = std::exp(logA[u]);
    q.reuse_V = want_reuse && c->lv_valid && c->lv_n == n && c->lv_bytes == (int)sizeof(R);
    c->cur_n = n; c->cur_np = np; c->cur_d = q.d; c->cur_dp = q.dp;
    c->phase_valid = false;
    c->side_ev_next = 0;
  }
  if (na == 0) return 0;
  gpfit_ctx* c0 = un[0].c;
  static const bool batch_times = getenv("GPFIT_BATCH_TIMES") != nullptr;
  hipEvent_t tev[4] = {nullptr, nullptr, nullptr, nullptr};
  if (batch_times) {
    for (auto& e : tev) (void)hipEventCreate(&e);
    (void)hipEventRecord(tev[0], s);
  }
  {
    GroupPrepT<R> gp{};
    gp.n_units = na; gp.n = n; gp.np = np;
    for (int i = 0; i < na; ++i) {
      gpfit_ctx* c = un[i].c;
      gp.pix_host[i] = c->pix_host; gp.pix[i] = c->pix; gp.d[i] = un[i].d; gp.info[i] = c->info;
      gp.m[i] = m[un[i].u]; gp.mpad[i] = RP(c->mpad);
    }
    GP_TRY(launch_group_prepare(gp, s));
  }
  for (int i = 0; i < na; ++i) {
    Unit& q = un[i];
    gpfit_ctx* c = q.c;
    g_main_sk_ws = c0->sk_ws[0];
    GP_TRY(build_kernel<R>(c, s, q.th, q.d, q.dp, n_rows, n_cols, X[q.u], ldx, n, np, 0));
    GP_TRY(launch_moments(RP(c->Kvec), RP(c->q), RP(c->Cos), ld, V[q.u], ldv, m[q.u], r[q.u], n, q.A, lambda0[q.u], RP(c->lam_m),
                          RP(c->lam_var), RP(c->fvec), RP(c->wl), c->scal, c->sumA_part, c->info + 2, s));
    if (!q.reuse_V) {
      c->lv_valid = false; c->lv32_valid = false;
      GP_TRY(launch_pack_lower(V[q.u], ldv, n, RP(c->Vbuf), ld, np, s));
    }
  }
  if (batch_times) (void)hipEventRecord(tev[1], s);
  {
    CholBatchT<R> cb;
    uint32_t need = 0;
    for (int i = 0; i < na; ++i) {
      gpfit_ctx* c = un[i].c;
      int b = cb.nb++;
      cb.A[b] = RP(c->Kbuf); cb.L[b] = RP(c->Lbuf); cb.Li[b] = RP(c->Libuf); cb.Tmp[b] = RP(c->Tmp); cb.info[b] = c->info + 0;
      need |= 1u << b;
      if (un[i].reuse_V) continue;
      b = cb.nb++;
      cb.A[b] = RP(c->Vbuf); cb.L[b] = RP(c->LVbuf); cb.Li[b] = RP(c->LiVbuf); cb.Tmp[b] = RP(c->TmpV); cb.info[b] = c->info + 1;
    }
    cb.ld = ld; cb.ws = 0; cb.sk_ws = c0->sk_ws[0]; cb.ctx = nullptr; cb.side_min = 0;
    GP_TRY(potrf_lockstep<R>(cb, 0, np, need, s));
  }
  if (batch_times) (void)hipEventRecord(tev[2], s);
  auto no_phase = [](int, hipStream_t) {};
  gpfit_ctx* cl[GEMM_MAXB];
  Theta thl[GEMM_MAXB];
  int dl[GEMM_MAXB], dpl[GEMM_MAXB];
  PostJoin<R> pjl[GEMM_MAXB];
  PostJoin<float> pfl[GEMM_MAXB];
  for (int i = 0; i < na; ++i) {
    Unit& q = un[i];
    gpfit_ctx* c = q.c;
    cl[i] = c; thl[i] = q.th; dl[i] = q.d; dpl[i] = q.dp;
    if (!q.reuse_V) GP_TRY(launch_logdet_pair(RP(c->Lbuf), c->scal + 3, RP(c->LVbuf), c->scal + 40, ld, n, s));
    else GP_TRY(launch_logdet(RP(c->Lbuf), ld, n, c->scal + 3, s));
    GP_TRY(solve_mean<R>(c, np, s));
    if (mixed_grad) GP_TRY(demote_for_mixed(c, q.reuse_V, np, q.dp, s, &pfl[i]));
    else pjl[i] = post_join_args<R>(c);
  }
  if (mixed_grad) GP_TRY(post_join_list<float>(na, cl, pfl, thl, n, np, dl, dpl, n_rows, n_cols, want_grad, s, no_phase));
  else GP_TRY(post_join_list<R>(na, cl, pjl, thl, n, np, dl, dpl, n_rows, n_cols, want_grad, s, no_phase));
  {
    GroupCollectT gc{};
    gc.n_units = na;
    for (int i = 0; i < na; ++i) {
      gpfit_ctx* c = un[i].c;
      gc.scal[i] = c->scal; gc.info[i] = c->info; gc.scal_host[i] = c->scal_host; gc.info_host[i] = c->info_host;
    }
    GP_TRY(launch_group_collect(gc, s));
  }
  if (!c0->pend.done) GP_HIP(hipEventCreateWithFlags(&c0->pend.done, hipEventDisableTiming));
  GP_HIP(hipEventRecord(c0->pend.done, s));
  for (int i = 0; i < na; ++i) {
    Unit& q = un[i];
    gpfit_ctx* c = q.c;
    if (c != c0) {
      if (!c->pend.done) GP_HIP(hipEventCreateWithFlags(&c->pend.done, hipEventDisableTiming));
      GP_HIP(hipEventRecord(c->pend.done, s));
    }
    set_pending(c, s, q.A, lambda0[q.u], q.th.sigma0, n, np, q.d, want_grad, (int)sizeof(R), true);
  }
  c0->last_enqueue_ms = std::chrono::duration<double, std::milli>(std::chrono::steady_clock::now() - t_host0).count();
  if (batch_times) {
    (void)hipEventRecord(tev[3], s);
    (void)hipEventSynchronize(tev[3]);
    float a = 0, b = 0, d3 = 0;
    (void)hipEventElapsedTime(&a, tev[0], tev[1]);
    (void)hipEventElapsedTime(&b, tev[1], tev[2]);
    (void)hipEventElapsedTime(&d3, tev[2], tev[3]);
    fprintf(stderr, "[gpfit batch] %d units: build %.3f ms, lock-step factorisations %.3f ms, post %.3f ms (enqueue %.2f ms)\n", na, a,
            b, d3, c0->last_enqueue_ms);
    for (auto& e : tev) (void)hipEventDestroy(e);
  }
  return 0;
}

static int grad_pullback_impl(gpfit_ctx* c, void* stream, const double* theta, int n_rows, int n_cols, const double* X,
                              int64_t ldx, int64_t N, const double* W, int64_t ldw, const double* gvec,
                              double* out6) {
  using R = double;
  if (!c || !theta || !X || !W || !gvec || !out6 || N <= 0) {
    set_error("gpfit_grad_pullback: bad argument");
    return -3;
  }
  GP_CTX_ENTER(c, "gpfit_grad_pullback");
  hipStream_t s = (hipStream_t)stream;
  const int n = (int)N, np = (int)round_up(N, TILE);
  Admitted ad;
  GP_TRY(admit(c, "gpfit_grad_pullback", "the context", theta, nullptr, nullptr, n_rows, n_cols, np, nullptr, &ad));
  const int d = ad.d, dp = ad.dp;
  const Theta th = ad.th;
  c->lv_valid = false; c->lv32_valid = false;
  g_main_sk_ws = c->sk_ws[0];
  GP_HIP(hipMemcpyAsync(c->pix, c->pix_host, (size_t)d * sizeof(int), hipMemcpyHostToDevice, s));
  GP_TRY(build_kernel<R>(c, s, th, d, dp, n_rows, n_cols, X, ldx, n, np, 0));
  GP_TRY(launch_pack_lower(W, ldw, n, c->Wbuf, (int64_t)np, np, s));
  GP_HIP(hipMemsetAsync(c->bv, 0, (size_t)np * sizeof(R), s));
  GP_HIP(hipMemsetAsync(c->wl, 0, (size_t)np * sizeof(R), s));
  GP_TRY(launch_scale_copy<R>(c->wl, gvec, n, -1.0, s));
  GP_TRY(pullback_to_metric(c, s, c->Wbuf, c->Cos, c->q, n, np, dp, c->Abuf, c->Xm));
  GP_TRY(launch_metric_contract(th, c->pix, d, n_rows, n_cols, c->Cmat, dp, c->Mmat, dp, c->scal + 10, c->upart, c->info + 3, s));
  GP_HIP(hipMemcpyAsync(c->scal_host, c->scal, 64 * sizeof(double), hipMemcpyDeviceToHost, s));
  GP_HIP(hipStreamSynchronize(s));
  const double* sc = c->scal_host;
  grad_rows(sc, sigma0_row_metric(sc, th.sigma0) - 2.0 * th.sigma0 * sc[8], out6);
  return 0;
}

static int fit_eval_projected_impl(gpfit_ctx* c, void* stream, const double* theta, const double* lower,
                                   const double* upper, int n_rows, int n_cols, const double* X, int64_t ldx, int64_t N,
                                   const double* r, const double* B, int64_t ldb, int64_t n_kept, const double* m_b,
                                   const double* V_b, int64_t ldvb, double logA, double lambda0, double* out_host) {
  using R = double;
  if (!c || !theta || !X || !r || !B || !m_b || !V_b || !out_host || N <= 0 || n_kept <= 0 || n_kept > N) {
    set_error("gpfit_fit_eval_projected: bad argument");
    return -3;
  }
  GP_CTX_ENTER(c, "gpfit_fit_eval_projected");
  hipStream_t s = (hipStream_t)stream;
  const int n = (int)N, np = (int)round_up(N, TILE), nk = (int)n_kept, nb = (int)round_up(n_kept, TILE);
  Admitted ad;
  GP_TRY(admit(c, "gpfit_fit_eval_projected", "the context", theta, lower, upper, n_rows, n_cols, np, out_host, &ad));
  const int d = ad.d, dp = ad.dp;
  const Theta th = ad.th;
  const double A = std::exp(logA);
  const int64_t ld = np, lb = nb;
  c->lv_valid = false; c->lv32_valid = false;
  c->side_ev_next = 0;
  g_main_sk_ws = c->sk_ws[0];
  ++g_eval_count;
  prof_begin(c);
  struct ProfGuard { gpfit_ctx* c; ~ProfGuard() { prof_end(c); } } prof_guard{c};
  double *Kt = c->Kbuf, *Bp = c->Lbuf, *Kb = c->Libuf, *aV = c->Tbuf, *Ga = c->Zbuf, *GaKi = c->Tmp, *W = c->Wbuf;
  double *S1 = c->Vbuf, *S2 = c->LVbuf, *S3 = c->LiVbuf, *S4 = c->TmpV;
  double *mbp = c->mpad, *bvec = c->yv, *gm = c->dq1, *gv = c->dq2;
  GP_HIP(hipMemsetAsync(c->info, 0, 4 * sizeof(int), s));
  GP_HIP(hipMemcpyAsync(c->pix, c->pix_host, (size_t)d * sizeof(int), hipMemcpyHostToDevice, s));
  GP_TRY(build_kernel<R>(c, s, th, d, dp, n_rows, n_cols, X, ldx, n, np, 1));
  GP_TRY(launch_pad_copy(B, ldb, n, nk, Bp, lb, np, nb, s));
  GP_HIP(hipMemsetAsync(mbp, 0, (size_t)np * sizeof(double), s));
  GP_HIP(hipMemcpyAsync(mbp, m_b, (size_t)nk * sizeof(double), hipMemcpyDeviceToDevice, s));
  GP_TRY(gemm_splitk<R>(s, 0, 1, np, nb, np, 1.0, Kt, ld, Bp, lb, Kb, lb, splitk_for(np, nb, np), c->Wbuf, (int64_t)c->np_cap * c->np_cap));
  GP_TRY(gemm_splitk<R>(s, 1, 1, nb, nb, np, 1.0, Bp, lb, Kb, lb, S4, lb, splitk_for(nb, nb, np), c->Wbuf, (int64_t)c->np_cap * c->np_cap));
  GP_TRY(launch_symmetrize_avg(S4, lb, nk, s));
  GP_TRY(launch_pack_lower(S4, lb, nk, S1, lb, nb, s));
  GP_TRY(launch_pack_lower(V_b, ldvb, nk, c->Abuf, lb, nb, s));
  GP_TRY(projected_factor(c, s, V_b, ldvb, nk, nb, c->Abuf, c->Wbuf, c->Zbuf, c->Tmp));
  double* Ki = S1;
  GP_TRY(gemm<R>(s, 0, 1, np, nb, nb, 1.0, Bp, lb, S2, lb, 0.0, aV, lb, 0, 0, 0));
  GP_TRY(projected_kl_products(c, s, nk, nb));
  GP_TRY(launch_symv_lower(Ki, lb, nb, mbp, bvec, s));
  GP_TRY(launch_dot(mbp, bvec, nb, c->scal + 6, s));
  GP_TRY(launch_proj_moments(Bp, Kb, aV, lb, nb, mbp, c->Kvec, r, n, A, lambda0, c->lam_m, c->lam_var, c->fvec, gm, gv,
                             c->upart, c->scal + 0, s));
  GP_TRY(launch_proj_ga(Kb, aV, lb, nb, n, np, gm, gv, mbp, Ga, s));
  GP_TRY(gemm<R>(s, 0, 1, np, nb, nb, 1.0, Ga, lb, Ki, lb, 0.0, GaKi, lb, 0, 0, 0));
  GP_TRY(gemm_splitk<R>(s, 1, 1, nb, nb, np, 1.0, Bp, lb, GaKi, lb, c->Abuf, lb, splitk_for(nb, nb, np), c->Wbuf, (int64_t)c->np_cap * c->np_cap));
  GP_TRY(launch_proj_gktb(Ki, S4, c->Abuf, lb, nb, bvec, S3, s));
  GP_TRY(launch_proj_gkb(Bp, lb, nb, n, np, gv, GaKi, s));
  GP_TRY(gemm<R>(s, 0, 1, np, nb, nb, 1.0, Bp, lb, S3, lb, 1.0, GaKi, lb, 0, 0, 0));
  if (2 * (int64_t)nb * np <= (int64_t)c->np_cap * c->np_cap) {
    double *Cat1 = Ga, *Cat2 = aV;
    const int64_t l2b = 2 * lb;
    GP_TRY(launch_pad_copy(GaKi, lb, np, nb, Cat1, l2b, np, nb, s));
    GP_TRY(launch_pad_copy(Bp, lb, np, nb, Cat1 + nb, l2b, np, nb, s));
    GP_TRY(launch_pad_copy(Bp, lb, np, nb, Cat2, l2b, np, nb, s));
    GP_TRY(launch_pad_copy(GaKi, lb, np, nb, Cat2 + nb, l2b, np, nb, s));
    GP_TRY(gemm<R>(s, 0, 0, np, np, 2 * nb, 0.5, Cat1, l2b, Cat2, l2b, 0.0, W, ld, 1, 0, 0));
  } else {
    GP_TRY(gemm<R>(s, 0, 0, np, np, nb, 1.0, GaKi, lb, Bp, lb, 0.0, W, ld, 0, 0, 0));
    GP_TRY(launch_symmetrize_avg(W, ld, np, s));
  }
  GP_HIP(hipMemsetAsync(c->bv, 0, (size_t)np * sizeof(R), s));
  GP_HIP(hipMemsetAsync(c->wl, 0, (size_t)np * sizeof(R), s));
  GP_TRY(launch_scale_copy<R>(c->wl, gv, n, 1.0, s));
  GP_TRY(pullback_to_metric(c, s, W, c->Cos, c->q, n, np, dp, c->Abuf, c->Xm));
  GP_TRY(launch_metric_contract(th, c->pix, d, n_rows, n_cols, c->Cmat, dp, c->Mmat, dp, c->scal + 10, c->upart, c->info + 3, s));
  GP_HIP(hipMemcpyAsync(c->scal_host, c->scal, 64 * sizeof(double), hipMemcpyDeviceToHost, s));
  GP_HIP(hipMemcpyAsync(c->info_host, c->info, 4 * sizeof(int), hipMemcpyDeviceToHost, s));
  GP_HIP(hipStreamSynchronize(s));
  const double* sc = c->scal_host;
  return assemble_out(c, A, lambda0, sigma0_row_metric(sc, th.sigma0) - 2.0 * th.sigma0 * sc[8], 0, d, 1,
                      "gpfit_fit_eval_projected: Cholesky of the projected K_tilde failed (non-positive pivot)",
                      "gpfit_fit_eval_projected: Cholesky of V_b failed (non-positive pivot)", out_host);
}

static int fit_eval_sparse_impl(gpfit_ctx* c, void* stream, const double* theta, const double* lower,
                                const double* upper, int n_rows, int n_cols, const double* X, int64_t ldx, int64_t N,
                                const double* Xtilde, int64_t ldxt, int64_t Ntilde, const double* r, const double* B,
                                int64_t ldb, int64_t n_kept, const double* m_b, const double* V_b, int64_t ldvb,
                                double logA, double lambda0, double* out_host) {
  using R = double;
  if (!c || !theta || !X || !Xtilde || !r || !B || !m_b || !V_b || !out_host || N <= 0 || Ntilde <= 0 || n_kept <= 0 ||
      n_kept > Ntilde) {
    set_error("gpfit_fit_eval_sparse: bad argument");
    return -3;
  }
  GP_CTX_ENTER(c, "gpfit_fit_eval_sparse");
  hipStream_t s = (hipStream_t)stream;
  const int n1 = (int)N, n2 = (int)Ntilde, nk = (int)n_kept;
  const int np1 = (int)round_up(N, TILE), np2 = (int)round_up(Ntilde, TILE), nb = (int)round_up(n_kept, TILE);
  Admitted ad;
  GP_TRY(admit(c, "gpfit_fit_eval_sparse", "the context", theta, lower, upper, n_rows, n_cols, std::max(np1, np2),
               out_host, &ad));
  const int d = ad.d, dp = ad.dp;
  const Theta th = ad.th;
  const double s0sq = th.sigma0 * th.sigma0, A = std::exp(logA);
  const int64_t l2 = np2, lb = nb;
  c->lv_valid = false; c->lv32_valid = false;
  c->side_ev_next = 0;
  g_main_sk_ws = c->sk_ws[0];
  ++g_eval_count;
  prof_begin(c);
  struct ProfGuard { gpfit_ctx* c; ~ProfGuard() { prof_end(c); } } prof_guard{c};
  double *X1m = c->Xm, *X2m = c->XDt, *Zm = c->XDt2;
  double *Kt = c->Kbuf, *CosT = c->Cos, *Kr = c->Lbuf, *CosR = c->Libuf, *Bp = c->Tbuf, *Kb = c->Zbuf, *am = c->Tmp,
         *aV = c->Abuf;
  double *S1 = c->Vbuf, *S2 = c->LVbuf, *S3 = c->LiVbuf, *S4 = c->TmpV;
  double *mbp = c->mpad, *bvec = c->yv, *gm = c->dq1, *gv = c->dq2, *gvec = c->hvec;
  GP_HIP(hipMemsetAsync(c->info, 0, 4 * sizeof(int), s));
  GP_HIP(hipMemcpyAsync(c->pix, c->pix_host, (size_t)d * sizeof(int), hipMemcpyHostToDevice, s));
  GP_TRY(build_metric<R>(c, s, th, d, dp, n_rows, n_cols));
  GP_TRY(kernel_side<R>(c, s, X, ldx, n1, np1, d, dp, s0sq, c->Xt, c->XCt, X1m, c->Kvec, c->q));
  GP_TRY(kernel_side<R>(c, s, Xtilde, ldxt, n2, np2, d, dp, s0sq, c->Xt2, c->XCt2, X2m, c->hvec, c->q2));
  GP_TRY(gram_square<R>(s, c->XCt2, c->Xt2, c->q2, Kt, CosT, n2, np2, dp, s0sq, 1));
  {
    GramArgsT<R> g{};
    g.XCt = c->XCt; g.Xt = c->Xt2; g.q1 = c->q; g.q2 = c->q2; g.Kout = Kr; g.Cos = CosR;
    g.ld1 = np1; g.ld2 = l2; g.ldk = l2; g.np1 = np1; g.np2 = np2; g.nv1 = n1; g.nv2 = n2; g.Kd = dp;
    g.s0sq = s0sq; g.lower = 0; g.pad_identity = 0;
    g.ldcos = l2;
    ProfScope ps(s, 2.0 * np1 * np2 * dp, 2);
    GP_TRY(launch_gram(g, s));
  }
  GP_TRY(launch_pad_copy(B, ldb, n2, nk, Bp, lb, np2, nb, s));
  GP_HIP(hipMemsetAsync(mbp, 0, (size_t)c->np_cap * sizeof(double), s));
  GP_HIP(hipMemcpyAsync(mbp, m_b, (size_t)nk * sizeof(double), hipMemcpyDeviceToDevice, s));
  GP_TRY(gemm_splitk<R>(s, 0, 1, np1, nb, np2, 1.0, Kr, l2, Bp, lb, Kb, lb, splitk_for(np1, nb, np2), c->Wbuf, (int64_t)c->np_cap * c->np_cap));
  GP_TRY(gemm_splitk<R>(s, 0, 1, np2, nb, np2, 1.0, Kt, l2, Bp, lb, am, lb, splitk_for(np2, nb, np2), c->Wbuf, (int64_t)c->np_cap * c->np_cap));
  GP_TRY(gemm_splitk<R>(s, 1, 1, nb, nb, np2, 1.0, Bp, lb, am, lb, S4, lb, splitk_for(nb, nb, np2), c->Wbuf, (int64_t)c->np_cap * c->np_cap));
  GP_TRY(launch_symmetrize_avg(S4, lb, nk, s));
  GP_TRY(launch_pack_lower(S4, lb, nk, S1, lb, nb, s));
  {
    double *Va = c->Wbuf, *Vl = c->Kbuf, *Vli = c->Lbuf, *Vt = c->Abuf;
    GP_TRY(launch_pack_lower(V_b, ldvb, nk, Va, lb, nb, s));
    for (double* p : {Vl, Vli, Vt})
      GP_HIP(hipMemsetAsync(p, 0, (size_t)nb * nb * sizeof(double), s));
    GP_TRY(projected_factor(c, s, V_b, ldvb, nk, nb, Va, Vl, Vli, Vt));
  }
  double* Ki = S1;
  GP_TRY(projected_kl_products(c, s, nk, nb));
  GP_TRY(gemm<R>(s, 0, 1, np1, nb, nb, 1.0, Kb, lb, Ki, lb, 0.0, am, lb, 0, 0, 0));
  GP_TRY(gemm<R>(s, 0, 1, np1, nb, nb, 1.0, am, lb, S2, lb, 0.0, aV, lb, 0, 0, 0));
  GP_TRY(launch_symv_lower(Ki, lb, nb, mbp, bvec, s));
  GP_TRY(launch_dot(mbp, bvec, nb, c->scal + 6, s));
  GP_TRY(launch_proj_moments(am, Kb, aV, lb, nb, mbp, c->Kvec, r, n1, A, lambda0, c->lam_m, c->lam_var, c->fvec, gm, gv,
                             c->upart, c->scal + 0, s));
  double* Ga = Kt;
  double* GaKi = Kr;
  GP_TRY(launch_proj_ga(Kb, aV, lb, nb, n1, np1, gm, gv, mbp, Ga, s));
  GP_TRY(gemm<R>(s, 0, 1, np1, nb, nb, 1.0, Ga, lb, Ki, lb, 0.0, GaKi, lb, 0, 0, 0));
  GP_TRY(gemm_splitk<R>(s, 1, 1, nb, nb, np1, 1.0, am, lb, GaKi, lb, c->Wbuf, lb, splitk_for(nb, nb, np1), c->TmpV + (int64_t)nb * nb,
                        (int64_t)c->np_cap * c->np_cap - (int64_t)nb * nb));
  GP_TRY(launch_proj_gktb(Ki, S4, c->Wbuf, lb, nb, bvec, S3, s));
  GP_TRY(launch_proj_gkb(am, lb, nb, n1, np1, gv, GaKi, s));
  GP_TRY(gemm<R>(s, 0, 1, np2, nb, nb, 1.0, Bp, lb, S3, lb, 0.0, Kt, lb, 0, 0, 0));
  GP_TRY(gemm<R>(s, 0, 0, np2, np2, nb, 1.0, Kt, lb, Bp, lb, 0.0, c->Wbuf, l2, 0, 0, 0));
  GP_TRY(launch_symmetrize_avg(c->Wbuf, l2, np2, s));
  GP_TRY(gemm<R>(s, 0, 0, np1, np2, nb, 1.0, GaKi, lb, Bp, lb, 0.0, aV, l2, 0, 0, 0));
  double* WK = aV;
  GP_HIP(hipMemsetAsync(c->bv, 0, (size_t)c->np_cap * sizeof(R), s));
  GP_HIP(hipMemsetAsync(c->wl, 0, (size_t)c->np_cap * sizeof(R), s));
  GP_TRY(pullback_to_metric(c, s, c->Wbuf, CosT, c->q2, n2, np2, dp, Kb, X2m));
  GP_TRY(launch_scale_copy<R>(gvec, gv, n1, -1.0, s));
  double* t1 = c->tvec;
  double* t2 = c->tvec + c->np_cap;
  GP_TRY(launch_adjoint_rect(WK, l2, CosR, l2, c->q, c->q2, n1, n2, np1, np2, Kt, l2, c->upart, c->vpart, c->rect_part,
                             gvec, t1, t2, c->rpad, c->mpad, c->scal + 20, s));
  GP_TRY(gemm<R>(s, 0, 1, np1, dp, np2, 1.0, Kt, l2, X2m, dp, 0.0, c->Ybuf, dp, 0, 0, 0));
  GP_TRY(launch_rowscale_add(c->Ybuf, dp, X1m, dp, t1, np1, dp, s));
  GP_HIP(hipMemsetAsync(Zm, 0, (size_t)np2 * dp * sizeof(double), s));
  GP_TRY(launch_rowscale_add(Zm, dp, X2m, dp, t2, np2, dp, s));
  GP_TRY(xty<R>(c, s, X1m, c->Ybuf, np1, dp, c->dCpad, false));
  GP_TRY(launch_axpby_block<double>(c->Mmat, dp, c->dCpad, dp, dp, dp, 1.0, 1.0, s));
  GP_TRY(xty<R>(c, s, X2m, Zm, np2, dp, c->dCpad, false));
  GP_TRY(launch_axpby_block<double>(c->Mmat, dp, c->dCpad, dp, dp, dp, 1.0, 1.0, s));
  GP_TRY(launch_symmetrize_avg(c->Mmat, dp, dp, s));
  GP_TRY(launch_metric_contract(th, c->pix, d, n_rows, n_cols, c->Cmat, dp, c->Mmat, dp, c->scal + 10, c->upart, c->info + 3, s));
  GP_HIP(hipMemcpyAsync(c->scal_host, c->scal, 64 * sizeof(double), hipMemcpyDeviceToHost, s));
  GP_HIP(hipMemcpyAsync(c->info_host, c->info, 4 * sizeof(int), hipMemcpyDeviceToHost, s));
  GP_HIP(hipStreamSynchronize(s));
  const double* sc = c->scal_host;
  const double sum_gvec = 0.5 * A * A * sc[2];
  return assemble_out(c, A, lambda0,
                      sigma0_row_metric(sc, th.sigma0) + th.sigma0 * (2.0 * sc[20] + sc[21] + sc[22]) +
                          2.0 * th.sigma0 * sum_gvec,
                      0, d, 1, "gpfit_fit_eval_sparse: Cholesky of the projected K_tilde failed (non-positive pivot)",
                      "gpfit_fit_eval_sparse: Cholesky of V_b failed (non-positive pivot)", out_host);
}

int fit_eval_finish(gpfit_ctx* c, double* out_host) {
  if (!c || !out_host || !c->pend.active) {
    set_error("gpfit_fit_eval_finish: nothing pending on this context");
    return -3;
  }
  c->pend.active = false;
  DeviceGuard device_guard(c->device);
  if (c->pend.use_done && c->pend.done) GP_HIP(hipEventSynchronize(c->pend.done));
  else GP_HIP(hipStreamSynchronize(c->pend.stream));
  const double* sc = c->scal_host;
  const double sigma0 = c->pend.sigma0;
  GP_TRY(assemble_out(c, c->pend.A, c->pend.lambda0, sigma0_row_metric(sc, sigma0) - 2.0 * sigma0 * sc[8],
                      c->pend.np - c->pend.n, c->pend.d, c->pend.want_grad, "Cholesky of K_tilde failed: non-positive pivot",
                      "Cholesky of V failed: non-positive pivot", out_host));
  c->lv_valid = true;
  c->lv_n = c->pend.n;
  c->lv_bytes = c->pend.elem_bytes;
  return 0;
}

}

using namespace gpfit;

extern "C" {

int gpfit_fit_eval(gpfit_ctx* c, void* stream, const double* theta, const double* lower, const double* upper,
                   int n_rows, int n_cols, const double* X, int64_t ldx, int64_t N, const double* r,
                   const double* m, const double* V, int64_t ldv, double logA, double lambda0, int want_grad,
                   double* out_host, double* lam_m_out, double* lam_var_out, double* f_out) {
  return fit_eval_impl<double>(c, stream, theta, lower, upper, n_rows, n_cols, X, ldx, N, r, m, V, ldv, logA, lambda0,
                               want_grad, out_host, lam_m_out, lam_var_out, f_out);
}

int gpfit_fit_eval_f32(gpfit_ctx* c, void* stream, const double* theta, const double* lower, const double* upper,
                       int n_rows, int n_cols, const float* X, int64_t ldx, int64_t N, const float* r,
                       const float* m, const float* V, int64_t ldv, double logA, double lambda0, int want_grad,
                       double* out_host, float* lam_m_out, float* lam_var_out, float* f_out) {
  return fit_eval_impl<float>(c, stream, theta, lower, upper, n_rows, n_cols, X, ldx, N, r, m, V, ldv, logA, lambda0,
                              want_grad, out_host, lam_m_out, lam_var_out, f_out);
}

int gpfit_fit_eval_finish(gpfit_ctx* c, double* out_host) { return fit_eval_finish(c, out_host); }

int gpfit_fit_eval_batch(gpfit_ctx* const* ctxs, int n_units, void* stream, const double* theta, const double* lower,
                         const double* upper, int n_rows, int n_cols, const double* const* X, int64_t ldx, int64_t N,
                         const double* const* r, const double* const* m, const double* const* V, int64_t ldv,
                         const double* logA, const double* lambda0, int want_grad, double* out_host, int* rc_out) {
  return fit_eval_batch_impl<double>(ctxs, n_units, stream, theta, lower, upper, n_rows, n_cols, X, ldx, N, r, m, V, ldv,
                                     logA, lambda0, want_grad, out_host, rc_out);
}

int gpfit_fit_eval_batch_f32(gpfit_ctx* const* ctxs, int n_units, void* stream, const double* theta, const double* lower,
                             const double* upper, int n_rows, int n_cols, const float* const* X, int64_t ldx, int64_t N,
                             const float* const* r, const float* const* m, const float* const* V, int64_t ldv,
                             const double* logA, const double* lambda0, int want_grad, double* out_host, int* rc_out) {
  return fit_eval_batch_impl<float>(ctxs, n_units, stream, theta, lower, upper, n_rows, n_cols, X, ldx, N, r, m, V, ldv,
                                    logA, lambda0, want_grad, out_host, rc_out);
}

int gpfit_fit_eval_projected(gpfit_ctx* c, void* stream, const double* theta, const double* lower, const double* upper,
                             int n_rows, int n_cols, const double* X, int64_t ldx, int64_t N, const double* r,
                             const double* B, int64_t ldb, int64_t n_kept, const double* m_b, const double* V_b,
                             int64_t ldvb, double logA, double lambda0, double* out_host) {
  return fit_eval_projected_impl(c, stream, theta, lower, upper, n_rows, n_cols, X, ldx, N, r, B, ldb, n_kept, m_b, V_b,
                                 ldvb, logA, lambda0, out_host);
}

int gpfit_fit_eval_sparse(gpfit_ctx* c, void* stream, const double* theta, const double* lower, const double* upper,
                          int n_rows, int n_cols, const double* X, int64_t ldx, int64_t N, const double* Xtilde,
                          int64_t ldxt, int64_t Ntilde, const double* r, const double* B, int64_t ldb, int64_t n_kept,
                          const double* m_b, const double* V_b, int64_t ldvb, double logA, double lambda0,
                          double* out_host) {
  return fit_eval_sparse_impl(c, stream, theta, lower, upper, n_rows, n_cols, X, ldx, N, Xtilde, ldxt, Ntilde, r, B, ldb,
                              n_kept, m_b, V_b, ldvb, logA, lambda0, out_host);
}

int gpfit_grad_pullback(gpfit_ctx* c, void* stream, const double* theta, int n_rows, int n_cols, const double* X,
                        int64_t ldx, int64_t N, const double* W, int64_t ldw, const double* gvec, double* out6) {
  return grad_pullback_impl(c, stream, theta, n_rows, n_cols, X, ldx, N, W, ldw, gvec, out6);
}

int gpfit_ctx_create(int device, int64_t n_max, int64_t d_max, int64_t d_full_max, gpfit_ctx** out) {
  if (!out || n_max <= 0 || d_max <= 0) {
    set_error("gpfit_ctx_create: bad argument");
    return -3;
  }
  DeviceGuard device_guard(device);
  {
    int cur = -1;
    GP_HIP(hipGetDevice(&cur));
    if (cur != device) {
      set_error("gpfit_ctx_create: cannot select the requested device");
      return -3;
    }
  }
  gpfit_ctx* c = new gpfit_ctx();
  c->device = device;
  c->np_cap = (int)round_up(n_max, TILE);
  c->dp_cap = (int)round_up(d_max, 32);
  c->dfull_cap = (int)std::max<int64_t>(d_full_max, d_max);
  const size_t np = c->np_cap, dp = c->dp_cap, nn = np * np;
  int rc = 0;
  auto A = [&](double** p, size_t cnt) { if (!rc) rc = dev_alloc(c, p, cnt); };
  A(&c->Kbuf, nn); A(&c->Cos, nn); A(&c->Lbuf, nn); A(&c->Libuf, nn); A(&c->Vbuf, nn); A(&c->LVbuf, nn);
  A(&c->LiVbuf, nn); A(&c->Tbuf, nn); A(&c->Zbuf, nn); A(&c->Wbuf, nn); A(&c->Abuf, nn); A(&c->Tmp, nn);
  A(&c->TmpV, nn);
  A(&c->Xt, dp * np); A(&c->Xm, np * dp); A(&c->XCt, dp * np); A(&c->Cmat, dp * dp); A(&c->Ybuf, np * dp);
  A(&c->Mpart, (size_t)c->split_k_M * dp * dp); A(&c->Mmat, dp * dp);
  A(&c->Xt2, dp * np); A(&c->XCt2, dp * np); A(&c->XDt, dp * np); A(&c->XDt2, dp * np); A(&c->dCpad, dp * dp);
  A(&c->q2, np); A(&c->dq1, np); A(&c->dq2, np); A(&c->hvec, np);
  A(&c->Kvec, np); A(&c->q, np); A(&c->lam_m, np); A(&c->lam_var, np); A(&c->fvec, np); A(&c->wl, np);
  A(&c->yv, np); A(&c->bv, np); A(&c->tvec, 2 * np); A(&c->mpad, np); A(&c->rpad, np);
  const size_t t64 = np / 64;
  A(&c->upart, t64 * np); A(&c->vpart, t64 * np); A(&c->sumA_part, t64 * (t64 + 1) / 2);
  A(&c->rect_part, t64 * t64);
  A(&c->frob_part, 33 * (np / TILE) * (np / TILE + 1) / 2); A(&c->trmv_part, (np / TRMV_ROWS + 1) * np);
  A(&c->scal, 64);
  for (int i = 0; i < 2 && !rc; ++i) {
    double* w = nullptr;
    rc = dev_alloc(c, &w, SK_WS_BYTES / sizeof(double));
    c->sk_ws[i] = w;
  }
  if (!rc) rc = dev_alloc(c, &c->pix, (size_t)c->dfull_cap);
  if (!rc) rc = dev_alloc(c, &c->info, 4);
  if (rc) {
    gpfit_ctx_destroy(c);
    return rc;
  }
  constexpr unsigned HOST_FLAGS = hipHostMallocMapped | hipHostMallocPortable;
  GP_HIP(hipHostMalloc((void**)&c->scal_host, 64 * sizeof(double), HOST_FLAGS));
  GP_HIP(hipHostMalloc((void**)&c->pix_host, (size_t)c->dfull_cap * sizeof(int), HOST_FLAGS));
  GP_HIP(hipHostMalloc((void**)&c->info_host, 4 * sizeof(int), HOST_FLAGS));
  {
    int least = 0, greatest = 0;
    GP_HIP(hipDeviceGetStreamPriorityRange(&least, &greatest));
    GP_HIP(hipStreamCreateWithPriority(&c->aux, hipStreamNonBlocking, least));
  }
  GP_HIP(hipEventCreateWithFlags(&c->ev_fork, hipEventDisableTiming));
  GP_HIP(hipEventCreateWithFlags(&c->ev_join, hipEventDisableTiming));
  for (double* p : {c->Kbuf, c->Cos, c->Lbuf, c->Libuf, c->Vbuf, c->LVbuf, c->LiVbuf, c->Tbuf, c->Zbuf, c->Wbuf,
                    c->Abuf, c->Tmp, c->TmpV})
    GP_HIP(hipMemset(p, 0, nn * sizeof(double)));
  GP_HIP(hipDeviceSynchronize());
  *out = c;
  return 0;
}

void gpfit_ctx_destroy(gpfit_ctx* c) {
  if (!c) return;
  DeviceGuard device_guard(c->device);
  (void)hipDeviceSynchronize();
  for (void* p : c->allocs) (void)hipFree(p);
  if (c->pend.done) (void)hipEventDestroy(c->pend.done);
  if (c->scal_host) (void)hipHostFree(c->scal_host);
  if (c->pix_host) (void)hipHostFree(c->pix_host);
  if (c->info_host) (void)hipHostFree(c->info_host);
  if (c->aux) (void)hipStreamDestroy(c->aux);
  if (c->side) (void)hipStreamDestroy(c->side);
  for (hipEvent_t e : c->side_ev) (void)hipEventDestroy(e);
  if (c->ev_fork) (void)hipEventDestroy(c->ev_fork);
  if (c->ev_join) (void)hipEventDestroy(c->ev_join);
  for (hipEvent_t e : c->phase_ev)
    if (e) (void)hipEventDestroy(e);
  delete c;
}

int gpfit_set_profile(gpfit_ctx* c, int on) {
  if (!c) return -3;
  c->profile = (on == 2) ? 2 : (on ? 1 : 0);
  return 0;
}

int gpfit_get_phases(gpfit_ctx* c, double* out8) {
  if (!c || !out8) return -3;
  if (!c->phase_valid) {
    set_error("gpfit_get_phases: no phase-timed evaluation (gpfit_set_profile(ctx, 2), then a synchronous gpfit_fit_eval with gradients)");
    return -3;
  }
  DeviceGuard device_guard(c->device);
  GP_HIP(hipDeviceSynchronize());
  for (int i = 0; i < 8; ++i) {
    float t = 0.f;
    GP_HIP(hipEventElapsedTime(&t, c->phase_ev[0], c->phase_ev[i]));
    out8[i] = t;
  }
  return 0;
}

double gpfit_last_enqueue_ms(gpfit_ctx* c) { return c ? c->last_enqueue_ms : -1.0; }

int gpfit_get_profile(gpfit_ctx* c, double* out16) {
  if (!c || !out16) return -3;
  for (int i = 0; i < 16; ++i) out16[i] = c->prof_out[i];
  return 0;
}

int gpfit_check_limits(const double* theta, const double* lower, const double* upper) {
  return check_limits(theta, lower, upper);
}

int gpfit_localker_mask(const double* theta, int n_rows, int n_cols, uint8_t* mask_host, int64_t* d_out) {
  if (!theta || n_rows <= 0 || n_cols <= 0) {
    set_error("gpfit_localker_mask: bad argument");
    return -3;
  }
  const int d = compute_mask(theta, n_rows, n_cols, mask_host, nullptr);
  if (d_out) *d_out = d;
  return 0;
}


}
```

### gaussian_processes_amd/csrc/gemm.hip

```cpp
#include "gemm_core.h"

#include <algorithm>
#include <cstdlib>
#include <mutex>
#include <set>
#include <utility>

namespace gpfit {

template <typename R, bool A_KMAJOR, bool B_KMAJOR, bool EDGE, int T, int NS>
__device__ __forceinline__ bool gemm_tile_compute(const GemmArgsT<R>& p, int tiles_n, int ntiles, R* smem,
                                                  typename Real<R>::acc_t (&acc)[T / 32][T / 32], int& ti, int& tj,
                                                  int& row0, int& col0, R*& C) {
  constexpr int KT = Real<R>::KT;

  const int bid = (p.reverse & 1) ? (ntiles - 1 - (int)blockIdx.x) : (int)blockIdx.x;
  if (p.sched != nullptr) {
    const int e = p.sched[blockIdx.x];
    if (e < 0) return false;
    ti = e >> 16;
    tj = e & 0xffff;
  } else if (p.out_lower && (p.reverse & 2) && T == TILE) {
    const int nt = tiles_n;
    int j = (int)((2.0 * nt + 1.0 - sqrt((2.0 * nt + 1.0) * (2.0 * nt + 1.0) - 8.0 * (double)bid)) * 0.5);
    while (j > 0 && (long)j * nt - (long)j * (j - 1) / 2 > bid) --j;
    while ((long)(j + 1) * nt - (long)(j + 1) * j / 2 <= bid) ++j;
    tj = j;
    ti = j + (bid - (j * nt - j * (j - 1) / 2));
  } else if (p.out_lower) {
    lower_tile(bid, TILE / T, ti, tj);
  } else if (p.reverse & 2) {
    const int tiles_m = ntiles / tiles_n;
    tj = bid / tiles_m;
    ti = bid % tiles_m;
  } else {
    ti = bid / tiles_n;
    tj = bid % tiles_n;
  }
  row0 = ti * T;
  col0 = tj * T;
  const int b = blockIdx.y, z = blockIdx.z;
  const R* A;
  const R* B;
  if (p.nptr > 0) {
    A = p.Ap[b];
    B = p.Bp[b];
    C = p.Cp[b];
  } else {
    A = p.A + (int64_t)b * p.sA;
    B = p.B + (int64_t)b * p.sB;
    C = p.C + (int64_t)b * p.sC;
  }

  int kbeg = 0, kend = p.K;
  if (p.a_tri == 1) kend = min(kend, row0 + T);
  if (p.a_tri == 2) kbeg = max(kbeg, row0);
  if (p.b_tri == 1) kbeg = max(kbeg, col0);
  if (p.b_tri == 2) kend = min(kend, col0 + T);
  if (p.split_k > 1) {
    const int steps = max(0, kend - kbeg) / KT;
    const int per = (steps + p.split_k - 1) / p.split_k;
    const int s0 = min(steps, z * per), s1 = min(steps, (z + 1) * per);
    kend = kbeg + s1 * KT;
    kbeg = kbeg + s0 * KT;
    C += (int64_t)z * p.sC;
  }

#pragma unroll
  for (int i = 0; i < T / 32; ++i)
#pragma unroll
    for (int j = 0; j < T / 32; ++j) acc[i][j] = acc_zero<R>();

  gemm_mainloop<R, A_KMAJOR, B_KMAJOR, EDGE, T, 0, NS>(A, p.lda, B, p.ldb, p.M, p.N, row0, col0, kbeg, kend, smem, acc,
                                                       (p.reverse & 4) != 0);
  return true;
}

template <typename R, bool A_KMAJOR, bool B_KMAJOR, bool EDGE, int T, int NS, int EPI = 0>
__device__ __forceinline__ void gemm_tile_body(const GemmArgsT<R>& p, int tiles_n, int ntiles, R* smem) {
  typename Real<R>::acc_t acc[T / 32][T / 32];
  int ti, tj, row0, col0;
  R* C;
  if (!gemm_tile_compute<R, A_KMAJOR, B_KMAJOR, EDGE, T, NS>(p, tiles_n, ntiles, smem, acc, ti, tj, row0, col0, C)) return;

  const R alpha = (R)p.alpha, beta = (p.split_k > 1) ? (R)0 : (R)p.beta;
  const int64_t ldc = p.ldc;
  const int M = p.M, N = p.N;
  if constexpr (EPI != 0) {
    constexpr int epi = EPI;
    R* __restrict__ D = p.nptr > 0 ? p.auxp[blockIdx.y] : p.aux;
    double* __restrict__ sumsq = p.nptr > 0 ? p.sumsqp[blockIdx.y] : p.sumsq;
    double ss = 0.0;
    for_each_acc<R, T>(acc, row0, col0, [&](int row, int col, R v) {
      if (EDGE && !(row < M && col < N)) return;
      R o = alpha * v;
      R* c = C + (int64_t)row * ldc + col;
      if (epi & 4) {
        R* dd = D + (int64_t)row * ldc + col;
        const R d0 = *dd;
        o += d0;
        *dd = o + d0;
      } else if (beta != (R)0) {
        o += beta * (*c);
      }
      if (epi & 1) {
        if (row >= col) *c = o;
        if (row > col) C[(int64_t)col * ldc + row] = o;
      } else {
        *c = o;
      }
      if (epi & 2) ss += (double)o * (double)o;
    });
    if (epi & 2) {
#pragma unroll
      for (int o = 32; o > 0; o >>= 1) ss += __shfl_down(ss, o);
      double* red = reinterpret_cast<double*>(smem);
      __syncthreads();
      if ((threadIdx.x & 63) == 0) red[threadIdx.x >> 6] = ss;
      __syncthreads();
      if (threadIdx.x == 0) sumsq[(int64_t)ti * (ti + 1) / 2 + tj] = (red[0] + red[1]) + (red[2] + red[3]);
    }
    return;
  }
  if (beta == (R)0) {
    for_each_acc<R, T>(acc, row0, col0, [&](int row, int col, R v) {
      if (!EDGE || (row < M && col < N)) C[(int64_t)row * ldc + col] = alpha * v;
    });
  } else {
    for_each_acc<R, T>(acc, row0, col0, [&](int row, int col, R v) {
      if (!EDGE || (row < M && col < N)) {
        R* c = C + (int64_t)row * ldc + col;
        *c = alpha * v + beta * (*c);
      }
    });
  }
}

template <typename R, bool A_KMAJOR, bool B_KMAJOR, bool EDGE, int T, int NS = 2>
__global__ __launch_bounds__(GEMM_THREADS, (T == 128 || NS > 2 ? 2 : 4)) void gemm_mfma_kernel(GemmArgsT<R> p,
                                                                                               int tiles_n,
                                                                                               int ntiles) {
  __shared__ __attribute__((aligned(16))) R smem[2 * NS * Real<R>::KT * T];
  gemm_tile_body<R, A_KMAJOR, B_KMAJOR, EDGE, T, NS>(p, tiles_n, ntiles, smem);
}

#ifdef GPFIT_CLOCK_STAMPS
__device__ long long g_gemm_clock[2][4096][2];
#endif

template <typename R, bool A_KMAJOR, bool B_KMAJOR>
__global__ __launch_bounds__(GEMM_THREADS, 2) void gemm_xcd_kernel(GemmArgsT<R> p, int tiles_n, int ntiles) {
  __shared__ __attribute__((aligned(16))) R smem[4 * Real<R>::KT * TILE];
#ifdef GPFIT_CLOCK_STAMPS
  const long long t0 = __builtin_amdgcn_s_memtime(), w0 = __builtin_amdgcn_s_memrealtime();
#endif
  gemm_tile_body<R, A_KMAJOR, B_KMAJOR, false, TILE, 2>(p, tiles_n, ntiles, smem);
#ifdef GPFIT_CLOCK_STAMPS
  if (threadIdx.x == 0 && blockIdx.x < 4096) {
    g_gemm_clock[B_KMAJOR ? 1 : 0][blockIdx.x][0] = (long long)__builtin_amdgcn_s_memtime() - t0;
    g_gemm_clock[B_KMAJOR ? 1 : 0][blockIdx.x][1] = (long long)__builtin_amdgcn_s_memrealtime() - w0;
  }
#endif
}

template <typename R, bool A_KMAJOR, bool B_KMAJOR, int EPI>
__global__ __launch_bounds__(GEMM_THREADS, 2) void gemm_epi_kernel(GemmArgsT<R> p, int tiles_n, int ntiles) {
  __shared__ __attribute__((aligned(16))) R smem[4 * Real<R>::KT * TILE];
#ifdef GPFIT_CLOCK_STAMPS
  const long long t0 = __builtin_amdgcn_s_memtime(), w0 = __builtin_amdgcn_s_memrealtime();
#endif
  gemm_tile_body<R, A_KMAJOR, B_KMAJOR, false, TILE, 2, EPI>(p, tiles_n, ntiles, smem);
#ifdef GPFIT_CLOCK_STAMPS
  if (threadIdx.x == 0 && blockIdx.x < 4096 && EPI != 4) {
    g_gemm_clock[B_KMAJOR ? 1 : 0][blockIdx.x][0] = (long long)__builtin_amdgcn_s_memtime() - t0;
    g_gemm_clock[B_KMAJOR ? 1 : 0][blockIdx.x][1] = (long long)__builtin_amdgcn_s_memrealtime() - w0;
  }
#endif
}

template <typename R>
int gemm_pick_tile(const GemmArgsT<R>& a) {
  if (a.tile == 128 || a.tile == 64 || a.tile == 32) return a.tile;
  auto ntiles = [&](int T) {
    const long tm = (a.M + T - 1) / T, tn = (a.N + T - 1) / T;
    const long nb = (a.M + TILE - 1) / TILE;
    return (a.out_lower ? (long)lower_tile_count((int)nb, TILE / T) : tm * tn) * (a.nptr > 0 ? a.nptr : (a.batch > 0 ? a.batch : 1)) *
           (a.split_k > 1 ? a.split_k : 1);
  };
  static const long t128_min = getenv("GPFIT_T128_MIN") ? atol(getenv("GPFIT_T128_MIN")) : 384;
  static const long t128_tri_min = getenv("GPFIT_T128_TRI_MIN") ? atol(getenv("GPFIT_T128_TRI_MIN")) : 1024;
  const bool batch_tri = a.nptr > 0 && (a.a_tri || a.b_tri);
  if (ntiles(128) >= (batch_tri ? t128_tri_min : t128_min)) return 128;
  static const long t64_min = getenv("GPFIT_T64_MIN") ? atol(getenv("GPFIT_T64_MIN")) : 256;
  static const long t32_dim = getenv("GPFIT_T32_DIM") ? atol(getenv("GPFIT_T32_DIM")) : 1024;
  if (ntiles(64) >= t64_min) return 64;
  return (a.M <= t32_dim && a.N <= t32_dim) ? 32 : 64;
}

constexpr int HALF_OCC_LDS = 17 * 1024;
static void allow_dynamic_lds(const void* fn) {
  static std::mutex mu;
  static std::set<std::pair<const void*, int>> done;
  int device = 0;
  (void)hipGetDevice(&device);
  std::lock_guard<std::mutex> lock(mu);
  if (done.insert({fn, device}).second)
    (void)hipFuncSetAttribute(fn, hipFuncAttributeMaxDynamicSharedMemorySize, HALF_OCC_LDS);
}

template <typename R, int T>
static void launch_T(const GemmArgsT<R>& p, hipStream_t s) {
  const int tm = (p.M + T - 1) / T, tn = (p.N + T - 1) / T;
  const int tiles = p.out_lower ? lower_tile_count((p.M + TILE - 1) / TILE, TILE / T) : tm * tn;
  const bool edge = (p.M % T) || (p.N % T) || (p.out_lower && (p.M % TILE));
  dim3 grid(p.sched ? p.sched_blocks : (p.tile_limit > 0 ? std::min(p.tile_limit, tiles) : tiles), p.batch,
            p.split_k > 1 ? p.split_k : 1);
  dim3 block(GEMM_THREADS);
  constexpr int DEEP = (T == 128) ? 2 : (T == 64 ? 4 : 8);
  static const int deep_max = getenv("GPFIT_DEEP_MAX") ? atoi(getenv("GPFIT_DEEP_MAX")) : 512;
  const bool deep = DEEP > 2 && !edge && (long)grid.x * grid.y * grid.z <= deep_max;
  const bool half = (T == TILE) && p.half_occ && !deep;
#define GP_LAUNCH(AK, BK, ED)                                                                          \
  do {                                                                                                 \
    if (deep) hipLaunchKernelGGL((gemm_mfma_kernel<R, AK, BK, ED, T, (ED ? 2 : DEEP)>), grid, block, 0, s, p, tn, tiles); \
    else if (half) {                                                                                   \
      allow_dynamic_lds(reinterpret_cast<const void*>(gemm_mfma_kernel<R, AK, BK, ED, T, 2>));          \
      hipLaunchKernelGGL((gemm_mfma_kernel<R, AK, BK, ED, T, 2>), grid, block, HALF_OCC_LDS, s, p, tn, tiles); \
    } else hipLaunchKernelGGL((gemm_mfma_kernel<R, AK, BK, ED, T, 2>), grid, block, 0, s, p, tn, tiles); \
  } while (0)
  if (p.epi) {
    if constexpr (T == TILE) {
      const int key = p.epi * 4 + (p.a_kmajor ? 2 : 0) + (p.b_kmajor ? 1 : 0);
      if (key == 2 * 4 + 1) hipLaunchKernelGGL((gemm_epi_kernel<R, false, true, 2>), grid, block, 0, s, p, tn, tiles);
      else if (key == 1 * 4 + 0) hipLaunchKernelGGL((gemm_epi_kernel<R, false, false, 1>), grid, block, 0, s, p, tn, tiles);
      else if (key == 4 * 4 + 1) hipLaunchKernelGGL((gemm_epi_kernel<R, false, true, 4>), grid, block, 0, s, p, tn, tiles);
    }
    return;
  }
  if (p.sched && T == TILE && !edge) {
    switch ((p.a_kmajor ? 2 : 0) | (p.b_kmajor ? 1 : 0)) {
      case 0: hipLaunchKernelGGL((gemm_xcd_kernel<R, false, false>), grid, block, 0, s, p, tn, tiles); break;
      case 1: hipLaunchKernelGGL((gemm_xcd_kernel<R, false, true>), grid, block, 0, s, p, tn, tiles); break;
      case 2: hipLaunchKernelGGL((gemm_xcd_kernel<R, true, false>), grid, block, 0, s, p, tn, tiles); break;
      default: hipLaunchKernelGGL((gemm_xcd_kernel<R, true, true>), grid, block, 0, s, p, tn, tiles); break;
    }
    return;
  }
  const int sel = (p.a_kmajor ? 4 : 0) | (p.b_kmajor ? 2 : 0) | (edge ? 1 : 0);
  switch (sel) {
    case 0: GP_LAUNCH(false, false, false); break;
    case 1: GP_LAUNCH(false, false, true); break;
    case 2: GP_LAUNCH(false, true, false); break;
    case 3: GP_LAUNCH(false, true, true); break;
    case 4: GP_LAUNCH(true, false, false); break;
    case 5: GP_LAUNCH(true, false, true); break;
    case 6: GP_LAUNCH(true, true, false); break;
    case 7: GP_LAUNCH(true, true, true); break;
  }
#undef GP_LAUNCH
}

template <typename R>
bool gemm_epilogue_ok(const GemmArgsT<R>& a) {
  if (a.split_k > 1 || (a.batch > 1 && a.nptr <= 0) || a.M <= 0 || a.N <= 0) return false;
  const int T = gemm_pick_tile(a);
  if ((a.M % T) || (a.N % T)) return false;
  if ((a.epi & 1) && (!a.out_lower || a.M != a.N)) return false;
  if ((a.epi & 2) && (T != TILE || !a.out_lower)) return false;
  if ((a.epi & 4) && a.nptr <= 0 && a.aux == nullptr) return false;
  if (T != TILE || a.a_kmajor || a.half_occ) return false;
  if (!((a.epi == 2 && a.b_kmajor) || (a.epi == 1 && !a.b_kmajor) || (a.epi == 4 && a.b_kmajor))) return false;
  if (a.nptr > 0) return true;
  if (T == TILE && a.tile_limit == 0) {
    if ((a.reverse & 8) && gemm_xcd_applies(a)) return true;
    if (gemm_streamk_applies(a)) return gemm_streamk_carries(a);
  }
  return true;
}

template <typename R>
int gemm_sumsq_entries(const GemmArgsT<R>& a) {
  if (!(a.epi & 2) || !gemm_epilogue_ok(a)) return 0;
  const int t = a.M / TILE, nt = t * (t + 1) / 2;
  if (a.nptr > 0 || a.half_occ || a.tile_limit != 0 || a.batch > 1) return nt;
  if ((a.reverse & 8) && gemm_xcd_applies(a)) return nt;
  return gemm_streamk_applies(a) ? 33 * nt : nt;
}
template int gemm_sumsq_entries<double>(const GemmArgsT<double>&);
template int gemm_sumsq_entries<float>(const GemmArgsT<float>&);
template bool gemm_epilogue_ok<double>(const GemmArgsT<double>&);
template bool gemm_epilogue_ok<float>(const GemmArgsT<float>&);

template <typename R>
int launch_gemm(const GemmArgsT<R>& a, hipStream_t s) {
  if (a.M <= 0 || a.N <= 0) return 0;
  if (a.epi && !gemm_epilogue_ok(a)) {
    set_error("launch_gemm: this launch cannot carry a fused epilogue (ask gemm_epilogue_ok first)");
    return -3;
  }
  if (a.nptr > 0) return launch_gemm_plain(a, s);
  if (a.half_occ) return launch_gemm_plain(a, s);
  if (a.tile_limit == 0 && gemm_pick_tile(a) == TILE && a.batch <= 1) {
    if (a.reverse & 8) {
      const int rc = launch_gemm_xcd(a, s);
      if (rc <= 0) return rc;
    }
    const int rc = launch_gemm_streamk(a, s);
    if (rc <= 0) return rc;
  }
  return launch_gemm_plain(a, s);
}

template <typename R>
int launch_gemm_plain(const GemmArgsT<R>& a, hipStream_t s) {
  if (a.M <= 0 || a.N <= 0) return 0;
  constexpr int EPC = 16 / (int)sizeof(R);
  if (a.K % ktile_of<R>() != 0 || (a.lda % EPC) || (a.ldb % EPC)) {
    set_error("launch_gemm: K must be a multiple of the K step and lda, ldb multiples of 16 bytes");
    return -3;
  }
  if (a.out_lower && a.M != a.N) {
    set_error("launch_gemm: out_lower needs a square output");
    return -3;
  }
  GemmArgsT<R> p = a;
  if (p.nptr > 0) {
    if (p.nptr > GEMM_MAXB || p.sched || p.split_k > 1) {
      set_error("launch_gemm: a pointer batch holds at most GEMM_MAXB plain problems");
      return -3;
    }
    p.batch = p.nptr;
  }
  if (p.batch <= 0) p.batch = 1;
  switch (gemm_pick_tile(p)) {
    case 128: launch_T<R, 128>(p, s); break;
    case 64: launch_T<R, 64>(p, s); break;
    default: launch_T<R, 32>(p, s); break;
  }
  GP_HIP(hipGetLastError());
  return 0;
}

template <typename R>
struct GemmPairT {
  GemmArgsT<R> g[2];
  int tiles[2], tiles_n[2];
};

template <typename R, int T, int NS>
__global__ __launch_bounds__(GEMM_THREADS, (NS > 2 ? 2 : 4)) void gemm_pair_kernel(GemmPairT<R> q) {
  __shared__ __attribute__((aligned(16))) R smem[2 * NS * Real<R>::KT * T];
  const int w = blockIdx.z;
  const GemmArgsT<R>& p = q.g[w];
  if ((int)blockIdx.x >= q.tiles[w] || (int)blockIdx.y >= p.batch) return;
  if (p.b_kmajor) gemm_tile_body<R, false, true, false, T, NS>(p, q.tiles_n[w], q.tiles[w], smem);
  else gemm_tile_body<R, false, false, false, T, NS>(p, q.tiles_n[w], q.tiles[w], smem);
}

template <typename R>
static int pair_member_tile(const GemmArgsT<R>& a) {
  constexpr int EPC = 16 / (int)sizeof(R);
  if (a.nptr <= 0 || a.nptr > GEMM_MAXB || a.epi || a.split_k > 1 || a.sched || a.half_occ || a.tile_limit || a.a_kmajor) return 0;
  if (a.M <= 0 || a.N <= 0 || (a.M % 64) || (a.N % 64) || (a.out_lower && ((a.M % TILE) || a.M != a.N))) return 0;
  if (a.K % ktile_of<R>() != 0 || (a.lda % EPC) || (a.ldb % EPC)) return 0;
  const int T = gemm_pick_tile(a);
  return (T == 32 || T == 64) ? T : 0;
}

template <typename R>
bool gemm_pair_ok(const GemmArgsT<R>& a, const GemmArgsT<R>& b) {
  static const bool off = getenv("GPFIT_NO_PAIR") != nullptr;
  static const bool no64 = getenv("GPFIT_NO_PAIR64") != nullptr;
  if (off) return false;
  const int ta = pair_member_tile(a), tb = pair_member_tile(b);
  return ta != 0 && ta == tb && !(no64 && ta == 64);
}
template bool gemm_pair_ok<double>(const GemmArgsT<double>&, const GemmArgsT<double>&);
template bool gemm_pair_ok<float>(const GemmArgsT<float>&, const GemmArgsT<float>&);

template <typename R>
int launch_gemm_pair(const GemmArgsT<R>& a, const GemmArgsT<R>& b, hipStream_t s) {
  if (!gemm_pair_ok(a, b)) {
    set_error("launch_gemm_pair: the two problems cannot share a launch (ask gemm_pair_ok first)");
    return -3;
  }
  static_assert(sizeof(GemmPairT<R>) <= 4096, "kernel arguments are limited to 4 KiB");
  const int T = pair_member_tile(a);
  GemmPairT<R> q;
  int gx = 0, gy = 0;
  long total = 0;
  for (int w = 0; w < 2; ++w) {
    q.g[w] = w == 0 ? a : b;
    GemmArgsT<R>& p = q.g[w];
    p.batch = p.nptr;
    const int tm = p.M / T, tn = p.N / T;
    q.tiles_n[w] = tn;
    q.tiles[w] = p.out_lower ? lower_tile_count(p.M / TILE, TILE / T) : tm * tn;
    gx = std::max(gx, q.tiles[w]);
    gy = std::max(gy, p.batch);
    total += (long)q.tiles[w] * p.batch;
  }
  const dim3 grid(gx, gy, 2), block(GEMM_THREADS);
  static const int deep_max = getenv("GPFIT_DEEP_MAX") ? atoi(getenv("GPFIT_DEEP_MAX")) : 512;
  if (T == 32 && total <= deep_max) hipLaunchKernelGGL((gemm_pair_kernel<R, 32, 8>), grid, block, 0, s, q);
  else if (T == 32) hipLaunchKernelGGL((gemm_pair_kernel<R, 32, 2>), grid, block, 0, s, q);
  else if (total <= deep_max) hipLaunchKernelGGL((gemm_pair_kernel<R, 64, 4>), grid, block, 0, s, q);
  else hipLaunchKernelGGL((gemm_pair_kernel<R, 64, 2>), grid, block, 0, s, q);
  GP_HIP(hipGetLastError());
  return 0;
}
template int launch_gemm_pair<double>(const GemmArgsT<double>&, const GemmArgsT<double>&, hipStream_t);
template int launch_gemm_pair<float>(const GemmArgsT<float>&, const GemmArgsT<float>&, hipStream_t);

template int launch_gemm<double>(const GemmArgsT<double>&, hipStream_t);
template int launch_gemm<float>(const GemmArgsT<float>&, hipStream_t);
template int launch_gemm_plain<double>(const GemmArgsT<double>&, hipStream_t);
template int launch_gemm_plain<float>(const GemmArgsT<float>&, hipStream_t);
template int gemm_pick_tile<double>(const GemmArgsT<double>&);
template int gemm_pick_tile<float>(const GemmArgsT<float>&);

}

#ifdef GPFIT_CLOCK_STAMPS
extern "C" int gpfit_dev_gemm_clock(long long* host_out ) {
  return hipMemcpyFromSymbol(host_out, HIP_SYMBOL(gpfit::g_gemm_clock), sizeof(long long) * 2 * 4096 * 2) == hipSuccess ? 0 : -1;
}
#endif
```

### gaussian_processes_amd/csrc/kernels.h

```cpp
#pragma once
#include "common.h"
#include "lbfgs1d.h"

namespace gpfit {

struct Theta {
  double sigma0, eps0x, eps0y, logbeta, logrho, amp;
  double eb, er;
};

template <typename R>
struct GroupPrepT {
  int n_units, n, np;
  const int* pix_host[GEMM_MAXB / 2];
  int* pix[GEMM_MAXB / 2];
  int d[GEMM_MAXB / 2];
  int* info[GEMM_MAXB / 2];
  const R* m[GEMM_MAXB / 2];
  R* mpad[GEMM_MAXB / 2];
};
struct GroupCollectT {
  int n_units;
  const double* scal[GEMM_MAXB / 2];
  const int* info[GEMM_MAXB / 2];
  double* scal_host[GEMM_MAXB / 2];
  int* info_host[GEMM_MAXB / 2];
};
template <typename R>
int launch_group_prepare(const GroupPrepT<R>& g, hipStream_t s);
int launch_group_collect(const GroupCollectT& g, hipStream_t s);

template <typename R>
struct LeafBatchT {
  const R* A[GEMM_MAXB];
  R* L[GEMM_MAXB];
  R* Li[GEMM_MAXB];
  int* info[GEMM_MAXB];
  int64_t lda, ldl, ldi;
  int info_base;
  int n;
};
template <typename R> int launch_chol_leaf_batch(const LeafBatchT<R>& bt, hipStream_t s);

template <typename R>
int launch_localker(const Theta& th, const int* pix, int d, int dp, int n_rows, int n_cols, R* C, int64_t ldc,
                    R* dC, hipStream_t s);
template <typename R>
int launch_gather(const R* X, int64_t ldx, int n, const int* pix, int d, int dp, int np, R* Xt, int64_t ldt, R* Xm,
                  int64_t ldm, hipStream_t s);
template <typename R>
int launch_qvec(const R* Xt, const R* XCt, int64_t ld, int dp, int n, int np, double s0sq, R* Kvec, R* q,
                hipStream_t s);
template <typename R>
int launch_pack_lower(const R* src, int64_t lds, int n, R* dst, int64_t ldd, int np, hipStream_t s);
template <typename R> int launch_symmetrize(R* A, int64_t lda, int n, hipStream_t s);
template <typename R> int launch_logdet(const R* L, int64_t ldl, int n, double* out, hipStream_t s);
template <typename R> int launch_logdet_pair(const R* L0, double* out0, const R* L1, double* out1, int64_t ldl, int n, hipStream_t s);
template <typename R>
int launch_frob_lower(const R* T, int64_t ldt, int np, double* out, double* partial, hipStream_t s);
template <typename R> int launch_trmv_lower(const R* L, int64_t ldl, int np, const R* x, R* y, hipStream_t s);
template <typename R>
int launch_trmv_lower_t(const R* L, int64_t ldl, int np, const R* x, R* z, double* partial, hipStream_t s);
template <typename R> int launch_dot(const R* x, const R* y, int n, double* out, hipStream_t s);

template <typename R>
int launch_moments(const R* Kvec, const R* q, const R* Cos, int64_t ldc, const R* V, int64_t ldv, const R* m,
                   const R* r, int n, double A, double lambda0, R* lam_m, R* lam_var, R* f, R* wl, double* scal,
                   double* part, int* ticket, hipStream_t s);

template <typename R>
int launch_adjoint(const R* W, const R* Cos, int64_t ld, const R* b, const R* q, int n, int np, R* Aout,
                   double* upart, double* vpart, double* sumA_part, hipStream_t s);
template <typename R>
int launch_adjoint_reduce(const double* upart, const double* vpart, const double* sumA_part, int ntile,
                          int ntile_tri, const R* q, const R* wl, int n, int np, R* tvec, double* uq,
                          double* scal_out, hipStream_t s);
template <typename R>
int launch_rowscale_add(R* Y, int64_t ldy, const R* Xm, int64_t ldm, const R* t, int np, int dp, hipStream_t s);
template <typename RI, typename RO>
int launch_reduce_slices(const RI* src, int64_t slice_stride, int nslice, RO* dst, int64_t count, hipStream_t s);
template <typename R>
int launch_metric_contract(const Theta& th, const int* pix, int d, int n_rows, int n_cols, const R* C, int64_t ldc,
                           const R* M, int64_t ldm, double* grad5, double* part ,
                           int* ticket , hipStream_t s);
int launch_frob_finish(const double* partial, int nt, double* out, hipStream_t s);
template <typename R> int launch_add_diag(R* A, int64_t lda, int n, double v, hipStream_t s);
template <typename R> int launch_scale_copy(R* dst, const R* src, int n, double alpha, hipStream_t s);
template <typename R>
int launch_axpby_block(R* dst, int64_t ldd, const R* src, int64_t lds, int rows, int cols, double a, double b,
                       hipStream_t s);

int launch_adjoint_rect(const double* W, int64_t ldw, const double* Cos, int64_t ldc, const double* q1,
                        const double* q2, int n1, int n2, int np1, int np2, double* Aout, int64_t lda, double* upart,
                        double* vpart, double* tile_sum, const double* extra1, double* t1, double* t2, double* uq1,
                        double* uq2, double* scal3, hipStream_t s);

int launch_nd_utility(const double* sigma2, const double* mu, int64_t nstar, const double* r, int nr, double* U,
                      hipStream_t s);

int launch_pad_copy(const double* src, int64_t lds, int rows, int cols, double* dst, int64_t ldd, int prow,
                    int pcol, hipStream_t s);
int launch_symmetrize_avg(double* A, int64_t lda, int n, hipStream_t s);
int launch_dk_sigma0(const double* Cos, int64_t ldc, const double* q1, const double* q2, int n1, int n2,
                     double s0, double* dK, int64_t ldk, hipStream_t s);
int launch_dq(const double* Xt, const double* XDt, int64_t ld, int dp, int n, const double* q, double* dq,
              double* h, hipStream_t s);
int launch_dk_metric(double* H, int64_t ldh, const double* Cos, int64_t ldc, const double* q1, const double* q2,
                     const double* dq1, const double* dq2, int n1, int n2, hipStream_t s);
int launch_fill(double* x, int64_t n, double v, hipStream_t s);

int launch_proj_moments(const double* Bp, const double* Kb, const double* aV, int64_t ld, int nb, const double* mb,
                        const double* Kvec, const double* r, int n, double A, double lambda0, double* lam_m,
                        double* lam_var, double* f, double* gm, double* gv, double* part, double* out3, hipStream_t s);
int launch_proj_ga(const double* Kb, const double* aV, int64_t ld, int nb, int n, int np, const double* gm,
                   const double* gv, const double* mb, double* Ga, hipStream_t s);
int launch_proj_gkb(const double* Bp, int64_t ld, int nb, int n, int np, const double* gv, double* GaKi, hipStream_t s);
int launch_proj_gktb(const double* Ki, const double* P1, const double* P2, int64_t ld, int nb, const double* b, double* G,
                     hipStream_t s);
int launch_proj_trace(const double* A, int64_t lda, int n, double* out, hipStream_t s);
int launch_estep_proj_rows(const double* a, int64_t lda, int nb, const double* mb, const double* f, const double* r,
                           int n, int nrows, double A, double* sv, double* u, hipStream_t s);
int launch_estep_proj_scale(const double* aL, int64_t ldal, int nb, int n, int nrows, const double* sv, const double* u,
                            double* Y, double* aLp , int64_t ld, int npc, double* part, hipStream_t s);
int launch_estep_proj_moments(const double* Z, int64_t ld, int nb, const double* z1, const double* kv0, int n,
                              double* lam_m, double* lam_var, hipStream_t s);

int launch_estep_prep(const double* f, const double* r, const double* m, int n, int np, double A, double* sv,
                      double* rhs, hipStream_t s);
int launch_estep_build(const double* K, int64_t ldk, int n, int np, const double* sv, double* Mb, double* SK,
                       double* Kl, int64_t ld, hipStream_t s);
int launch_symv_lower(const double* A, int64_t lda, int n, const double* x, double* y, hipStream_t s);
int launch_unpack_sym(const double* src, int64_t lds, int n, double* dst, int64_t ldd, hipStream_t s);
int launch_unpack_tri(const double* src, int64_t lds, int n, double* dst, int64_t ldd, hipStream_t s);
int launch_fparam(const double* lam_m, const double* lam_var, const double* r, int n, double A, int closed_form,
                  double lambda0_in, double* f, double* out, hipStream_t s);
int launch_fparam_lbfgs(const double* lam_m, const double* lam_var, const double* r, int n, double logA0,
                        int lambda0_mode, double lambda0_fixed, const Lbfgs1dConfig& cfg, double* f, double* out,
                        hipStream_t s);

}
```

Baseline: 33.96 fits/s.

## Keep top-level Cholesky inverse in 2x2 block form and restructure downstream solves

For large N, the Cholesky call now skips forming the full inverse at the top level (need mask 0) and keeps L21 from the factor. The mean solve, the trace and Frobenius terms, and the two-sided gradient update are all rewritten as 2x2 block operations using the diagonal inverses and L21. This is meant to avoid the costly full triangular inverse GEMMs. In exchange it adds many more kernel launches and new gemv and frob kernels, and the mixed-precision path now also demotes the L21 block.

```diff
diff --git a/gaussian_processes_amd/csrc/elementwise.hip b/gaussian_processes_amd/csrc/elementwise.hip
--- a/gaussian_processes_amd/csrc/elementwise.hip
+++ b/gaussian_processes_amd/csrc/elementwise.hip
@@ -360,6 +360,106 @@
   hipLaunchKernelGGL(trmv_lower_t_kernel<R>, dim3(np / 64, chunks), dim3(256), 0, s, L, ldl, np, x, partial);
   GP_HIP(hipGetLastError());
   return launch_reduce_slices(partial, np, chunks, z, np, s);
+}
+
+template <typename R>
+__global__ void gemv_sub_kernel(const R* __restrict__ M, int64_t ldm, int rows, int cols, const R* __restrict__ x,
+                                const R* __restrict__ y, R* __restrict__ out) {
+  const int lane = threadIdx.x & 63;
+  const int i = blockIdx.x * (blockDim.x >> 6) + (threadIdx.x >> 6);
+  if (i >= rows) return;
+  const R* row = M + (int64_t)i * ldm;
+  double v = 0.0;
+#pragma unroll 8
+  for (int j = lane; j < cols; j += 64) v += (double)row[j] * (double)x[j];
+  v = wave_sum(v);
+  if (lane == 0) out[i] = (R)((double)y[i] - v);
+}
+
+template <typename R>
+int launch_gemv_sub(const R* M, int64_t ldm, int rows, int cols, const R* x, const R* y, R* out, hipStream_t s) {
+  if (rows <= 0) return 0;
+  hipLaunchKernelGGL(gemv_sub_kernel<R>, dim3((rows + 3) / 4), dim3(256), 0, s, M, ldm, rows, cols, x, y, out);
+  GP_HIP(hipGetLastError());
+  return 0;
+}
+
+template <typename R>
+__global__ void gemv_t_kernel(const R* __restrict__ M, int64_t ldm, int rows, int cols, const R* __restrict__ x,
+                              double* __restrict__ partial) {
+  __shared__ double sh[4][64];
+  const int c = threadIdx.x & 63, rl = threadIdx.x >> 6;
+  const int j = blockIdx.x * 64 + c;
+  const int i0 = blockIdx.y * TRMV_ROWS, i1 = min(rows, i0 + TRMV_ROWS);
+  double v = 0.0;
+#pragma unroll 8
+  for (int i = i0 + rl; i < i1; i += 4) v += (double)M[(int64_t)i * ldm + j] * (double)x[i];
+  sh[rl][c] = v;
+  __syncthreads();
+  if (rl == 0) partial[(int64_t)blockIdx.y * cols + j] = sh[0][c] + sh[1][c] + sh[2][c] + sh[3][c];
+}
+
+template <typename R>
+__global__ void sub_slices_kernel(const double* __restrict__ partial, int cols, int nslice, const R* __restrict__ y,
+                                  R* __restrict__ out) {
+  const int j = blockIdx.x * blockDim.x + threadIdx.x;
+  if (j >= cols) return;
+  double v = 0.0;
+  for (int z = 0; z < nslice; ++z) v += partial[(int64_t)z * cols + j];
+  out[j] = (R)((double)y[j] - v);
+}
+
+template <typename R>
+int launch_gemv_t_sub(const R* M, int64_t ldm, int rows, int cols, const R* x, const R* y, R* out, double* partial,
+                      hipStream_t s) {
+  if (rows <= 0 || cols <= 0) return 0;
+  if (cols % 64) {
+    set_error("launch_gemv_t_sub: the column count must be a multiple of 64");
+    return -3;
+  }
+  const int chunks = (rows + TRMV_ROWS - 1) / TRMV_ROWS;
+  hipLaunchKernelGGL(gemv_t_kernel<R>, dim3(cols / 64, chunks), dim3(256), 0, s, M, ldm, rows, cols, x, partial);
+  hipLaunchKernelGGL(sub_slices_kernel<R>, dim3((cols + 255) / 256), dim3(256), 0, s, partial, cols, chunks, y, out);
+  GP_HIP(hipGetLastError());
+  return 0;
+}
+
+template <typename R>
+__global__ void frob_block_kernel(const R* __restrict__ T, int64_t ldt, int tn, double* __restrict__ partial) {
+  __shared__ double sh[17];
+  const int ti = blockIdx.x / tn, tj = blockIdx.x % tn;
+  const R* base = T + (int64_t)ti * TILE * ldt + tj * TILE;
+  double v = 0.0;
+#pragma unroll 8
+  for (int e = threadIdx.x; e < TILE * TILE; e += 256) {
+    const double x = (double)base[(int64_t)(e >> 7) * ldt + (e & 127)];
+    v += x * x;
+  }
+  v = block_sum(v, sh);
+  if (threadIdx.x == 0) partial[blockIdx.x] = v;
+}
+
+template <typename R>
+int launch_frob_tiles(const R* T, int64_t ldt, int rows, int cols, int lower, double* partial, hipStream_t s) {
+  const int tm = rows / TILE, tn = cols / TILE;
+  if (tm <= 0 || tn <= 0) return 0;
+  if (lower) hipLaunchKernelGGL(frob_tile_kernel<R>, dim3(tm * (tm + 1) / 2), dim3(256), 0, s, T, ldt, partial);
+  else hipLaunchKernelGGL(frob_block_kernel<R>, dim3(tm * tn), dim3(256), 0, s, T, ldt, tn, partial);
+  GP_HIP(hipGetLastError());
+  return 0;
+}
+
+__global__ void demote_block_kernel(const double* __restrict__ src, int64_t lds, float* __restrict__ dst, int64_t ldd,
+                                    int cols) {
+  const int c = blockIdx.x * blockDim.x + threadIdx.x;
+  if (c < cols) dst[(int64_t)blockIdx.y * ldd + c] = (float)src[(int64_t)blockIdx.y * lds + c];
+}
+
+int launch_demote_block(const double* src, int64_t lds, float* dst, int64_t ldd, int rows, int cols, hipStream_t s) {
+  if (rows <= 0 || cols <= 0) return 0;
+  hipLaunchKernelGGL(demote_block_kernel, dim3((cols + 255) / 256, rows), dim3(256), 0, s, src, lds, dst, ldd, cols);
+  GP_HIP(hipGetLastError());
+  return 0;
 }
 
 template <typename R>
@@ -1135,6 +1235,9 @@
   template int launch_frob_lower<R>(const R*, int64_t, int, double*, double*, hipStream_t);                         \
   template int launch_trmv_lower<R>(const R*, int64_t, int, const R*, R*, hipStream_t);                             \
   template int launch_trmv_lower_t<R>(const R*, int64_t, int, const R*, R*, double*, hipStream_t);                  \
+  template int launch_gemv_sub<R>(const R*, int64_t, int, int, const R*, const R*, R*, hipStream_t);                \
+  template int launch_gemv_t_sub<R>(const R*, int64_t, int, int, const R*, const R*, R*, double*, hipStream_t);     \
+  template int launch_frob_tiles<R>(const R*, int64_t, int, int, int, double*, hipStream_t);                        \
   template int launch_group_prepare<R>(const GroupPrepT<R>&, hipStream_t);                                          \
   template int launch_dot<R>(const R*, const R*, int, double*, hipStream_t);                                        \
   template int launch_moments<R>(const R*, const R*, const R*, int64_t, const R*, int64_t, const R*, const R*, int, \
diff --git a/gaussian_processes_amd/csrc/fit.hip b/gaussian_processes_amd/csrc/fit.hip
--- a/gaussian_processes_amd/csrc/fit.hip
+++ b/gaussian_processes_amd/csrc/fit.hip
@@ -336,6 +336,34 @@
   void* sk_ws = nullptr;
 };
 template <typename R>
+static int dual_update_list(hipStream_t s, int cnt, const R* const* Ap, const R* const* Bp, R* const* Hp, R* const* Zp, int M,
+                            int N, int K, double alpha, int64_t ld, int b_tri, int walk, void* sk_ws) {
+  bool fused = false;
+  if (fused_epilogues() & 4) {
+    GemmArgsT<R> g = gemm_args<R>(0, 1, M, N, K, alpha, Ap[0], ld, Bp[0], ld, 0.0, Hp[0], ld, 0, 0, b_tri, walk, 0, sk_ws);
+    g.epi = 4; g.aux = Zp[0];
+    static const bool no_batch = getenv("GPFIT_NO_BATCH") != nullptr;
+    if (cnt > 1 && gemm_pick_tile(g) != TILE && !no_batch) { g.nptr = cnt; g.batch = cnt; }
+    fused = gemm_epilogue_ok(g);
+  }
+  if (fused) {
+    bool done = false;
+    GP_TRY(gemm_list<R>(s, cnt, Ap, Bp, Hp, 0, 1, M, N, K, alpha, ld, ld, 0.0, ld, 0, 0, b_tri, walk, 0, sk_ws, 4, Zp, nullptr, &done));
+    if (!done) {
+      set_error("two_sided: the dual-update epilogue was announced but not carried");
+      return -100;
+    }
+    return 0;
+  }
+  for (int i = 0; i < cnt; ++i)
+    GP_HIP(hipMemcpy2DAsync(Hp[i], (size_t)ld * sizeof(R), Zp[i], (size_t)ld * sizeof(R), (size_t)N * sizeof(R), (size_t)M,
+                            hipMemcpyDeviceToDevice, s));
+  GP_TRY(gemm_list<R>(s, cnt, Ap, Bp, Hp, 0, 1, M, N, K, alpha, ld, ld, 1.0, ld, 0, 0, b_tri, walk, 0, sk_ws));
+  for (int i = 0; i < cnt; ++i) GP_TRY(launch_axpby_block<R>(Zp[i], ld, Hp[i], ld, M, N, 1.0, 1.0, s));
+  return 0;
+}
+
+template <typename R>
 static int two_sided_list(int cnt, const TwoSidedBufs<R>* b, const int* r0, int n, hipStream_t s) {
   if (cnt <= 0) return 0;
   const int64_t ld = b[0].ld;
@@ -373,34 +401,13 @@
   }
   GP_TRY(gemm_list<R>(s, cnt, Ap, Bp, Cp, 1, 1, n2, n1, n2, 0.5, ld, ld, 0.0, ld, 0, 0, 0, 0, 0, b[0].sk_ws));
   {
+    R* Hp[GEMM_MAXB];
     R* Zp[GEMM_MAXB];
     for (int i = 0; i < cnt; ++i) {
       const int r1 = r0[i] + n1;
-      Ap[i] = at(b[i].Q, r1, r0[i]); Bp[i] = at(b[i].Li, r0[i], r0[i]); Cp[i] = at(b[i].H, r1, r0[i]); Zp[i] = at(b[i].Z, r1, r0[i]);
-    }
-    bool fused = false;
-    if (fused_epilogues() & 4) {
-      GemmArgsT<R> g = gemm_args<R>(0, 1, n2, n1, n1, 1.0, Ap[0], ld, Bp[0], ld, 0.0, Cp[0], ld, 0, 0, 1, walks()[6], 0, b[0].sk_ws);
-      g.epi = 4; g.aux = Zp[0];
-      static const bool no_batch = getenv("GPFIT_NO_BATCH") != nullptr;
-      if (cnt > 1 && gemm_pick_tile(g) != TILE && !no_batch) { g.nptr = cnt; g.batch = cnt; }
-      fused = gemm_epilogue_ok(g);
-    }
-    if (fused) {
-      bool done = false;
-      GP_TRY(gemm_list<R>(s, cnt, Ap, Bp, Cp, 0, 1, n2, n1, n1, 1.0, ld, ld, 0.0, ld, 0, 0, 1, walks()[6], 0, b[0].sk_ws, 4, Zp, nullptr,
-                          &done));
-      if (!done) {
-        set_error("two_sided: the dual-update epilogue was announced but not carried");
-        return -100;
-      }
-    } else {
-      for (int i = 0; i < cnt; ++i)
-        GP_HIP(hipMemcpy2DAsync(Cp[i], (size_t)ld * sizeof(R), Zp[i], (size_t)ld * sizeof(R), (size_t)n1 * sizeof(R), (size_t)n2,
-                                hipMemcpyDeviceToDevice, s));
-      GP_TRY(gemm_list<R>(s, cnt, Ap, Bp, Cp, 0, 1, n2, n1, n1, 1.0, ld, ld, 1.0, ld, 0, 0, 1, walks()[6], 0, b[0].sk_ws));
-      for (int i = 0; i < cnt; ++i) GP_TRY(launch_axpby_block<R>(Zp[i], ld, Cp[i], ld, n2, n1, 1.0, 1.0, s));
-    }
+      Ap[i] = at(b[i].Q, r1, r0[i]); Bp[i] = at(b[i].Li, r0[i], r0[i]); Hp[i] = at(b[i].H, r1, r0[i]); Zp[i] = at(b[i].Z, r1, r0[i]);
+    }
+    GP_TRY(dual_update_list<R>(s, cnt, Ap, Bp, Hp, Zp, n2, n1, n1, 1.0, ld, 1, walks()[6], b[0].sk_ws));
   }
   static const int w21_walk = getenv("GPFIT_W21_WALK") ? atoi(getenv("GPFIT_W21_WALK")) : 0;
   for (int i = 0; i < cnt; ++i) {
@@ -420,6 +427,41 @@
   }
   GP_TRY(gemm_list<R>(s, cnt, Ap, Bp, Cp, 1, 1, n1, n1, n2, 0.5, ld, ld, 1.0, ld, 1, 0, 0, 0, 0, b[0].sk_ws));
   return 0;
+}
+
+constexpr int TOP_BLOCKS_MIN = 2048, TOP_BLOCKS_MIN_F32 = 5120;
+static bool top_in_blocks(int np, size_t elem_bytes) { return np >= (elem_bytes == 4 ? TOP_BLOCKS_MIN_F32 : TOP_BLOCKS_MIN); }
+
+template <typename R>
+static int two_sided_top(int cnt, const TwoSidedBufs<R>* b, const R* const* Lf, int n, hipStream_t s) {
+  if (cnt <= 0) return 0;
+  const int64_t ld = b[0].ld;
+  auto at = [&](const R* base, int r, int c) { return const_cast<R*>(base) + (int64_t)r * ld + c; };
+  int rr[GEMM_MAXB];
+  const int k = n / TILE;
+  const int n1 = ((k + 1) / 2) * TILE, n2 = n - n1;
+  const R* Ap[GEMM_MAXB];
+  const R* Bp[GEMM_MAXB];
+  R* Cp[GEMM_MAXB];
+  R* Zp[GEMM_MAXB];
+  void* sk = b[0].sk_ws;
+  for (int i = 0; i < cnt; ++i) rr[i] = n1;
+  GP_TRY(two_sided_list<R>(cnt, b, rr, n2, s));
+  for (int i = 0; i < cnt; ++i) GP_TRY(launch_symmetrize(at(b[i].W, n1, n1), ld, n2, s));
+  static const int w21_walk = getenv("GPFIT_W21_WALK") ? atoi(getenv("GPFIT_W21_WALK")) : 0;
+  for (int i = 0; i < cnt; ++i) { Ap[i] = at(b[i].Li, n1, n1); Bp[i] = at(b[i].Q, n1, 0); Cp[i] = at(b[i].Z, n1, 0); }
+  GP_TRY(gemm_list<R>(s, cnt, Ap, Bp, Cp, 1, 1, n2, n1, n2, 0.5, ld, ld, 0.0, ld, 0, 2, 0, w21_walk, 0, sk));
+  for (int i = 0; i < cnt; ++i) { Ap[i] = at(b[i].W, n1, n1); Bp[i] = at(Lf[i], n1, 0); Cp[i] = at(b[i].H, n1, 0); Zp[i] = at(b[i].Z, n1, 0); }
+  GP_TRY(dual_update_list<R>(s, cnt, Ap, Bp, Cp, Zp, n2, n1, n2, -1.0, ld, 0, 0, sk));
+  for (int i = 0; i < cnt; ++i) { Ap[i] = at(b[i].H, n1, 0); Bp[i] = at(b[i].Li, 0, 0); Cp[i] = at(b[i].W, n1, 0); }
+  GP_TRY(gemm_list<R>(s, cnt, Ap, Bp, Cp, 0, 1, n2, n1, n1, 1.0, ld, ld, 0.0, ld, 0, 0, 1, walks()[6], 0, sk));
+  for (int i = 0; i < cnt; ++i) { Ap[i] = at(Lf[i], n1, 0); Bp[i] = at(b[i].Z, n1, 0); Cp[i] = at(b[i].Q, 0, 0); }
+  GP_TRY(gemm_list<R>(s, cnt, Ap, Bp, Cp, 1, 1, n1, n1, n2, -1.0, ld, ld, 1.0, ld, 1, 0, 0, 0, 0, sk));
+  for (int i = 0; i < cnt; ++i) { Ap[i] = at(b[i].Z, n1, 0); Bp[i] = at(Lf[i], n1, 0); }
+  GP_TRY(gemm_list<R>(s, cnt, Ap, Bp, Cp, 1, 1, n1, n1, n2, -1.0, ld, ld, 1.0, ld, 1, 0, 0, 0, 0, sk));
+  for (int i = 0; i < cnt; ++i) GP_TRY(launch_symmetrize(Cp[i], ld, n1, s));
+  for (int i = 0; i < cnt; ++i) rr[i] = 0;
+  return two_sided_list<R>(cnt, b, rr, n1, s);
 }
 
 static double lin_pm1_host(int i, int n) {
@@ -550,11 +592,23 @@
 }
 
 template <typename R>
-static int solve_mean(gpfit_ctx* c, int np, hipStream_t s) {
+static int solve_mean(gpfit_ctx* c, int np, bool blocks, hipStream_t s) {
   const int64_t ld = np;
-  GP_TRY(launch_trmv_lower(ws_as<R>(c->Libuf), ld, np, ws_as<R>(c->mpad), ws_as<R>(c->yv), s));
-  GP_TRY(launch_dot(ws_as<R>(c->yv), ws_as<R>(c->yv), np, c->scal + 6, s));
-  return launch_trmv_lower_t(ws_as<R>(c->Libuf), ld, np, ws_as<R>(c->yv), ws_as<R>(c->bv), c->trmv_part, s);
+  R *m = ws_as<R>(c->mpad), *y = ws_as<R>(c->yv), *b = ws_as<R>(c->bv);
+  if (!blocks) {
+    GP_TRY(launch_trmv_lower(ws_as<R>(c->Libuf), ld, np, m, y, s));
+    GP_TRY(launch_dot(y, y, np, c->scal + 6, s));
+    return launch_trmv_lower_t(ws_as<R>(c->Libuf), ld, np, y, b, c->trmv_part, s);
+  }
+  const int kt = np / TILE, n1 = ((kt + 1) / 2) * TILE, n2 = np - n1;
+  const R *A = ws_as<R>(c->Libuf), *C = A + (int64_t)n1 * ld + n1, *L21 = ws_as<R>(c->Lbuf) + (int64_t)n1 * ld;
+  GP_TRY(launch_trmv_lower(A, ld, n1, m, y, s));
+  GP_TRY(launch_gemv_sub(L21, ld, n2, n1, y, m + n1, b + n1, s));
+  GP_TRY(launch_trmv_lower(C, ld, n2, b + n1, y + n1, s));
+  GP_TRY(launch_dot(y, y, np, c->scal + 6, s));
+  GP_TRY(launch_trmv_lower_t(C, ld, n2, y + n1, b + n1, c->trmv_part, s));
+  GP_TRY(launch_gemv_t_sub(L21, ld, n2, n1, b + n1, y, b, c->trmv_part, s));
+  return launch_trmv_lower_t(A, ld, n1, b, b, c->trmv_part, s);
 }
 
 template <typename R>
@@ -656,20 +710,24 @@
 
 template <typename R>
 struct PostJoin {
-  const R *Li, *LV, *Cos, *bv, *q, *wl, *Xm, *Cmat;
+  const R *Li, *L, *LV, *Cos, *bv, *q, *wl, *Xm, *Cmat;
   R *T, *W, *Z, *H, *A, *Y, *tvec, *Mpart, *Mmat;
 };
 template <typename R>
 static PostJoin<R> post_join_args(gpfit_ctx* c) {
   auto RP = ws_as<R>;
-  return PostJoin<R>{RP(c->Libuf), RP(c->LVbuf), RP(c->Cos), RP(c->bv), RP(c->q), RP(c->wl), RP(c->Xm), RP(c->Cmat),
+  return PostJoin<R>{RP(c->Libuf), RP(c->Lbuf), RP(c->LVbuf), RP(c->Cos), RP(c->bv), RP(c->q), RP(c->wl), RP(c->Xm), RP(c->Cmat),
                      RP(c->Tbuf), RP(c->Wbuf), RP(c->Zbuf), RP(c->Tmp), RP(c->Abuf), RP(c->Ybuf), RP(c->tvec),
                      RP(c->Mpart), RP(c->Mmat)};
 }
-static int demote_for_mixed(gpfit_ctx* c, bool reuse_V, int np, int dp, hipStream_t s, PostJoin<float>* pf) {
+static int demote_for_mixed(gpfit_ctx* c, bool reuse_V, int np, int dp, bool blocks, hipStream_t s, PostJoin<float>* pf) {
   auto F = ws_as<float>;
   const int64_t nn = (int64_t)np * np;
   GP_TRY((launch_reduce_slices<double, float>(c->Libuf, nn, 1, F(c->Kbuf), nn, s)));
+  if (blocks) {
+    const int kt = np / TILE, n1 = ((kt + 1) / 2) * TILE;
+    GP_TRY(launch_demote_block(c->Lbuf + (int64_t)n1 * np, np, F(c->Kbuf) + (int64_t)n1 * np, np, np - n1, n1, s));
+  }
   if (!(reuse_V && c->lv32_valid)) GP_TRY((launch_reduce_slices<double, float>(c->LVbuf, nn, 1, F(c->Vbuf), nn, s)));
   c->lv32_valid = true;
   GP_TRY((launch_reduce_slices<double, float>(c->Cos, nn, 1, F(c->TmpV), nn, s)));
@@ -678,21 +736,100 @@
   GP_TRY((launch_reduce_slices<double, float>(c->wl, np, 1, F(c->dq2), np, s)));
   GP_TRY((launch_reduce_slices<double, float>(c->Xm, (int64_t)np * dp, 1, F(c->Xt2), (int64_t)np * dp, s)));
   GP_TRY((launch_reduce_slices<double, float>(c->Cmat, (int64_t)dp * dp, 1, F(c->dCpad), (int64_t)dp * dp, s)));
-  *pf = PostJoin<float>{F(c->Kbuf), F(c->Vbuf), F(c->TmpV), F(c->q2), F(c->dq1), F(c->dq2), F(c->Xt2), F(c->dCpad),
+  *pf = PostJoin<float>{F(c->Kbuf), F(c->Kbuf), F(c->Vbuf), F(c->TmpV), F(c->q2), F(c->dq1), F(c->dq2), F(c->Xt2), F(c->dCpad),
                         F(c->Tbuf), F(c->Wbuf), F(c->Zbuf), F(c->Tmp), F(c->Abuf), F(c->Ybuf), F(c->tvec),
                         F(c->Mpart), F(c->Mmat)};
   return 0;
 }
+
+template <typename R>
+static int t_in_blocks(int cnt, gpfit_ctx* const* cs, const PostJoin<R>* a, int np, hipStream_t s) {
+  const int64_t ld = np;
+  const R* Ap[GEMM_MAXB];
+  const R* Bp[GEMM_MAXB];
+  R* Cp[GEMM_MAXB];
+  R* Tp[GEMM_MAXB];
+  double* Sp[GEMM_MAXB];
+  const int kt = np / TILE, n1 = ((kt + 1) / 2) * TILE, n2 = np - n1;
+  int ent = 0;
+  auto asks = [&](int M, int Nn, int K, int lower, int a_tri, int b_tri, int walk) {
+    GemmArgsT<R> g1 = gemm_args<R>(0, 1, M, Nn, K, 1.0, a[0].Li, ld, a[0].LV, ld, 0.0, a[0].T, ld, lower, a_tri, b_tri, walk, 0, cs[0]->sk_ws[0]);
+    g1.epi = 2; g1.sumsq = cs[0]->frob_part;
+    return ((fused_epilogues() & 2) && gemm_pick_tile(g1) == TILE) ? gemm_sumsq_entries(g1) : 0;
+  };
+  const bool any_fused = asks(n1, n1, n1, 1, 1, 1, walks()[3]) > 0 || asks(n2, n2, n2, 1, 1, 1, walks()[3]) > 0 ||
+                         asks(n2, n1, n2, 0, 1, 0, walks()[2]) > 0;
+  auto diag_blocks = [&](int cb, const int* rb, int nblk) -> int {
+    const int tb = nblk / TILE;
+    int e = asks(nblk, nblk, nblk, 1, 1, 1, walks()[3]);
+    const bool ask = e > 0;
+    if (!ask) e = tb * (tb + 1) / 2;
+    int m = 0;
+    for (int i = 0; i < cnt; ++i)
+      for (int j = 0; j < cb; ++j, ++m) {
+        const int64_t o = (int64_t)rb[j] * ld + rb[j];
+        Ap[m] = a[i].Li + o; Bp[m] = a[i].LV + o; Tp[m] = a[i].T + o; Sp[m] = cs[i]->frob_part + ent + j * e;
+      }
+    bool normed = false;
+    GP_TRY(gemm_list<R>(s, m, Ap, Bp, Tp, 0, 1, nblk, nblk, nblk, 1.0, ld, ld, 0.0, ld, 1, 1, 1, walks()[3], 0, cs[0]->sk_ws[0],
+                        ask ? 2 : 0, nullptr, Sp, &normed));
+    if (normed != ask) {
+      set_error("post_join: the tile-norm epilogue of a diagonal block of T was announced but not carried");
+      return -100;
+    }
+    if (!normed && any_fused)
+      for (int q = 0; q < m; ++q) GP_TRY(launch_frob_tiles<R>(Tp[q], ld, nblk, nblk, 1, Sp[q], s));
+    ent += cb * e;
+    return 0;
+  };
+  const int r_both[2] = {0, n1};
+  if (n2 == n1 && 2 * cnt <= GEMM_MAXB) GP_TRY(diag_blocks(2, r_both, n1));
+  else {
+    GP_TRY(diag_blocks(1, r_both, n1));
+    GP_TRY(diag_blocks(1, r_both + 1, n2));
+  }
+  {
+    const int64_t o21 = (int64_t)n1 * ld;
+    for (int i = 0; i < cnt; ++i) {
+      GP_HIP(hipMemcpy2DAsync(a[i].Z + o21, (size_t)ld * sizeof(R), a[i].LV + o21, (size_t)ld * sizeof(R), (size_t)n1 * sizeof(R),
+                              (size_t)n2, hipMemcpyDeviceToDevice, s));
+      Ap[i] = a[i].L + o21; Bp[i] = a[i].T; Cp[i] = a[i].Z + o21;
+    }
+    GP_TRY(gemm_list<R>(s, cnt, Ap, Bp, Cp, 0, 1, n2, n1, n1, -1.0, ld, ld, 1.0, ld, 0, 0, 1, walks()[1], 0, cs[0]->sk_ws[0]));
+    int e = asks(n2, n1, n2, 0, 1, 0, walks()[2]);
+    const bool ask = e > 0;
+    if (!ask) e = (n2 / TILE) * (n1 / TILE);
+    for (int i = 0; i < cnt; ++i) {
+      Ap[i] = a[i].Li + o21 + n1; Bp[i] = a[i].Z + o21; Tp[i] = a[i].T + o21; Sp[i] = cs[i]->frob_part + ent;
+    }
+    bool normed = false;
+    GP_TRY(gemm_list<R>(s, cnt, Ap, Bp, Tp, 0, 1, n2, n1, n2, 1.0, ld, ld, 0.0, ld, 0, 1, 0, walks()[2], 0, cs[0]->sk_ws[0],
+                        ask ? 2 : 0, nullptr, Sp, &normed));
+    if (normed != ask) {
+      set_error("post_join: the tile-norm epilogue of T21 was announced but not carried");
+      return -100;
+    }
+    if (!normed && any_fused)
+      for (int i = 0; i < cnt; ++i) GP_TRY(launch_frob_tiles<R>(Tp[i], ld, n2, n1, 0, Sp[i], s));
+    ent += e;
+  }
+  for (int i = 0; i < cnt; ++i) {
+    if (any_fused) GP_TRY(launch_frob_finish(cs[i]->frob_part, ent, cs[i]->scal + 5, s));
+    else GP_TRY(launch_frob_lower(a[i].T, ld, np, cs[i]->scal + 5, cs[i]->frob_part, s));
+  }
+  return 0;
+}
+
 template <typename R, typename PhaseFn>
 static int post_join_list(int cnt, gpfit_ctx* const* cs, const PostJoin<R>* a, const Theta* th, int n, int np, const int* d,
-                          const int* dp, int n_rows, int n_cols, int want_grad, hipStream_t s, PhaseFn&& phase) {
+                          const int* dp, int n_rows, int n_cols, int want_grad, bool blocks, hipStream_t s, PhaseFn&& phase) {
   const int64_t ld = np;
   const R* Ap[GEMM_MAXB];
   const R* Bp[GEMM_MAXB];
   R* Cp[GEMM_MAXB];
   double* Sp[GEMM_MAXB];
   if (cnt <= 0 || cnt > GEMM_MAXB) return cnt == 0 ? 0 : -3;
-  {
+  if (!blocks) {
     for (int i = 0; i < cnt; ++i) { Ap[i] = a[i].Li; Bp[i] = a[i].LV; Cp[i] = a[i].T; Sp[i] = cs[i]->frob_part; }
     bool normed = false;
     int norm_entries = 0;
@@ -702,6 +839,8 @@
       if (normed) GP_TRY(launch_frob_finish(cs[i]->frob_part, norm_entries, cs[i]->scal + 5, s));
       else GP_TRY(launch_frob_lower(a[i].T, ld, np, cs[i]->scal + 5, cs[i]->frob_part, s));
     }
+  } else {
+    GP_TRY(t_in_blocks<R>(cnt, cs, a, np, s));
   }
   phase(4, s);
   if (!want_grad) return 0;
@@ -719,13 +858,18 @@
   {
     static const int ts_min = getenv("GPFIT_TS_MIN") ? atoi(getenv("GPFIT_TS_MIN")) : 4096;
     TwoSidedBufs<R> tb[GEMM_MAXB];
-    int r0[GEMM_MAXB];
+    const R* Lf[GEMM_MAXB];
     for (int i = 0; i < cnt; ++i) {
       tb[i] = TwoSidedBufs<R>{a[i].W, a[i].Li, a[i].T, a[i].Z, a[i].H, ld, ts_min > 0 ? ts_min : (1 << 30)};
       tb[i].sk_ws = cs[0]->sk_ws[0];
-      r0[i] = 0;
-    }
-    GP_TRY(two_sided_list<R>(cnt, tb, r0, np, s));
+      Lf[i] = a[i].L;
+    }
+    if (blocks) GP_TRY(two_sided_top<R>(cnt, tb, Lf, np, s));
+    else {
+      int r0[GEMM_MAXB];
+      for (int i = 0; i < cnt; ++i) r0[i] = 0;
+      GP_TRY(two_sided_list<R>(cnt, tb, r0, np, s));
+    }
   }
   phase(6, s);
   for (int i = 0; i < cnt; ++i)
@@ -776,6 +920,7 @@
   const Theta th = ad.th;
   const double A = std::exp(logA);
   const int64_t ld = np;
+  const bool blocks = top_in_blocks(np, sizeof(R));
   c->cur_n = n; c->cur_np = np; c->cur_d = d; c->cur_dp = dp;
 
   ++g_eval_count;
@@ -822,21 +967,22 @@
     cb.A[1] = RP(c->Vbuf); cb.L[1] = RP(c->LVbuf); cb.Li[1] = RP(c->LiVbuf); cb.Tmp[1] = RP(c->TmpV); cb.info[1] = c->info + 1;
     cb.ld = ld; cb.ws = 0; cb.sk_ws = c->sk_ws[0]; cb.ctx = c; cb.side_min = side_min;
     if (!reuse_V) GP_HIP(hipStreamWaitEvent(s, c->ev_join, 0));
-    GP_TRY(potrf_lockstep<R>(cb, 0, np, 1u, s));
+    if (blocks) GP_TRY(potrf_lockstep<R>(cb, 0, np, 0u, s, 1u));
+    else GP_TRY(potrf_lockstep<R>(cb, 0, np, 1u, s));
     if (!reuse_V) GP_TRY(launch_logdet(RP(c->LVbuf), ld, n, c->scal + 40, s));
     phase(3, s);
   }
   GP_TRY(launch_logdet(RP(c->Lbuf), ld, n, c->scal + 3, s));
-  GP_TRY(solve_mean<R>(c, np, s));
+  GP_TRY(solve_mean<R>(c, np, blocks, s));
 
   phase(2, s);
   if (mixed_grad) {
     PostJoin<float> pf;
-    GP_TRY(demote_for_mixed(c, reuse_V, np, dp, s, &pf));
-    GP_TRY(post_join_list<float>(1, &c, &pf, &th, n, np, &d, &dp, n_rows, n_cols, want_grad, s, phase));
+    GP_TRY(demote_for_mixed(c, reuse_V, np, dp, blocks, s, &pf));
+    GP_TRY(post_join_list<float>(1, &c, &pf, &th, n, np, &d, &dp, n_rows, n_cols, want_grad, blocks, s, phase));
   } else {
     const PostJoin<R> pj = post_join_args<R>(c);
-    GP_TRY(post_join_list<R>(1, &c, &pj, &th, n, np, &d, &dp, n_rows, n_cols, want_grad, s, phase));
+    GP_TRY(post_join_list<R>(1, &c, &pj, &th, n, np, &d, &dp, n_rows, n_cols, want_grad, blocks, s, phase));
   }
 
   if (lam_m_out) GP_HIP(hipMemcpyAsync(lam_m_out, RP(c->lam_m), (size_t)n * sizeof(R), hipMemcpyDeviceToDevice, s));
@@ -888,6 +1034,7 @@
   const int64_t ld = np;
   const bool mixed_grad = (want_grad & 8) != 0 && sizeof(R) == 8 && (want_grad & 1);
   const bool want_reuse = (want_grad & 2) != 0;
+  const bool blocks = top_in_blocks(np, sizeof(R));
   want_grad &= 1;
   const auto t_host0 = std::chrono::steady_clock::now();
 
@@ -942,18 +1089,19 @@
   if (batch_times) (void)hipEventRecord(tev[1], s);
   {
     CholBatchT<R> cb;
-    uint32_t need = 0;
+    uint32_t kchains = 0;
     for (int i = 0; i < na; ++i) {
       gpfit_ctx* c = un[i].c;
       int b = cb.nb++;
       cb.A[b] = RP(c->Kbuf); cb.L[b] = RP(c->Lbuf); cb.Li[b] = RP(c->Libuf); cb.Tmp[b] = RP(c->Tmp); cb.info[b] = c->info + 0;
-      need |= 1u << b;
+      kchains |= 1u << b;
       if (un[i].reuse_V) continue;
       b = cb.nb++;
       cb.A[b] = RP(c->Vbuf); cb.L[b] = RP(c->LVbuf); cb.Li[b] = RP(c->LiVbuf); cb.Tmp[b] = RP(c->TmpV); cb.info[b] = c->info + 1;
     }
     cb.ld = ld; cb.ws = 0; cb.sk_ws = c0->sk_ws[0]; cb.ctx = nullptr; cb.side_min = 0;
-    GP_TRY(potrf_lockstep<R>(cb, 0, np, need, s));
+    if (blocks) GP_TRY(potrf_lockstep<R>(cb, 0, np, 0u, s, kchains));
+    else GP_TRY(potrf_lockstep<R>(cb, 0, np, kchains, s));
   }
   if (batch_times) (void)hipEventRecord(tev[2], s);
   auto no_phase = [](int, hipStream_t) {};
@@ -968,12 +1116,12 @@
     cl[i] = c; thl[i] = q.th; dl[i] = q.d; dpl[i] = q.dp;
     if (!q.reuse_V) GP_TRY(launch_logdet_pair(RP(c->Lbuf), c->scal + 3, RP(c->LVbuf), c->scal + 40, ld, n, s));
     else GP_TRY(launch_logdet(RP(c->Lbuf), ld, n, c->scal + 3, s));
-    GP_TRY(solve_mean<R>(c, np, s));
-    if (mixed_grad) GP_TRY(demote_for_mixed(c, q.reuse_V, np, q.dp, s, &pfl[i]));
+    GP_TRY(solve_mean<R>(c, np, blocks, s));
+    if (mixed_grad) GP_TRY(demote_for_mixed(c, q.reuse_V, np, q.dp, blocks, s, &pfl[i]));
     else pjl[i] = post_join_args<R>(c);
   }
-  if (mixed_grad) GP_TRY(post_join_list<float>(na, cl, pfl, thl, n, np, dl, dpl, n_rows, n_cols, want_grad, s, no_phase));
-  else GP_TRY(post_join_list<R>(na, cl, pjl, thl, n, np, dl, dpl, n_rows, n_cols, want_grad, s, no_phase));
+  if (mixed_grad) GP_TRY(post_join_list<float>(na, cl, pfl, thl, n, np, dl, dpl, n_rows, n_cols, want_grad, blocks, s, no_phase));
+  else GP_TRY(post_join_list<R>(na, cl, pjl, thl, n, np, dl, dpl, n_rows, n_cols, want_grad, blocks, s, no_phase));
   {
     GroupCollectT gc{};
     gc.n_units = na;
diff --git a/gaussian_processes_amd/csrc/gemm.hip b/gaussian_processes_amd/csrc/gemm.hip
--- a/gaussian_processes_amd/csrc/gemm.hip
+++ b/gaussian_processes_amd/csrc/gemm.hip
@@ -118,7 +118,8 @@
       __syncthreads();
       if ((threadIdx.x & 63) == 0) red[threadIdx.x >> 6] = ss;
       __syncthreads();
-      if (threadIdx.x == 0) sumsq[(int64_t)ti * (ti + 1) / 2 + tj] = (red[0] + red[1]) + (red[2] + red[3]);
+      if (threadIdx.x == 0)
+        sumsq[p.out_lower ? (int64_t)ti * (ti + 1) / 2 + tj : (int64_t)ti * tiles_n + tj] = (red[0] + red[1]) + (red[2] + red[3]);
     }
     return;
   }
@@ -266,7 +267,7 @@
   const int T = gemm_pick_tile(a);
   if ((a.M % T) || (a.N % T)) return false;
   if ((a.epi & 1) && (!a.out_lower || a.M != a.N)) return false;
-  if ((a.epi & 2) && (T != TILE || !a.out_lower)) return false;
+  if ((a.epi & 2) && T != TILE) return false;
   if ((a.epi & 4) && a.nptr <= 0 && a.aux == nullptr) return false;
   if (T != TILE || a.a_kmajor || a.half_occ) return false;
   if (!((a.epi == 2 && a.b_kmajor) || (a.epi == 1 && !a.b_kmajor) || (a.epi == 4 && a.b_kmajor))) return false;
@@ -281,7 +282,7 @@
 template <typename R>
 int gemm_sumsq_entries(const GemmArgsT<R>& a) {
   if (!(a.epi & 2) || !gemm_epilogue_ok(a)) return 0;
-  const int t = a.M / TILE, nt = t * (t + 1) / 2;
+  const int t = a.M / TILE, nt = a.out_lower ? t * (t + 1) / 2 : t * (a.N / TILE);
   if (a.nptr > 0 || a.half_occ || a.tile_limit != 0 || a.batch > 1) return nt;
   if ((a.reverse & 8) && gemm_xcd_applies(a)) return nt;
   return gemm_streamk_applies(a) ? 33 * nt : nt;
diff --git a/gaussian_processes_amd/csrc/kernels.h b/gaussian_processes_amd/csrc/kernels.h
--- a/gaussian_processes_amd/csrc/kernels.h
+++ b/gaussian_processes_amd/csrc/kernels.h
@@ -61,6 +61,14 @@
 template <typename R> int launch_trmv_lower(const R* L, int64_t ldl, int np, const R* x, R* y, hipStream_t s);
 template <typename R>
 int launch_trmv_lower_t(const R* L, int64_t ldl, int np, const R* x, R* z, double* partial, hipStream_t s);
+template <typename R>
+int launch_gemv_sub(const R* M, int64_t ldm, int rows, int cols, const R* x, const R* y, R* out, hipStream_t s);
+template <typename R>
+int launch_gemv_t_sub(const R* M, int64_t ldm, int rows, int cols, const R* x, const R* y, R* out, double* partial,
+                      hipStream_t s);
+template <typename R>
+int launch_frob_tiles(const R* T, int64_t ldt, int rows, int cols, int lower, double* partial, hipStream_t s);
+int launch_demote_block(const double* src, int64_t lds, float* dst, int64_t ldd, int rows, int cols, hipStream_t s);
 template <typename R> int launch_dot(const R* x, const R* y, int n, double* out, hipStream_t s);
 
 template <typename R>
```

Measured after the change: 36.17 fits/s (median of 6 runs). 6.5% higher.
